# paulvantieghem/curla

Hardware: AMD Instinct MI355X
Metric: SAC+CURL gradient updates/sec, batch=512 84x84x9 (higher is better)
Workload: dtype f32

## Files before the change

curla_amd/_lib.py:

```python
import ctypes
import os

_HERE = os.path.dirname(os.path.abspath(__file__))
LIB_PATH = os.environ.get("CURLA_LIB_PATH") or os.path.join(_HERE, "libcurla_hip.so")

c_int, c_ll, c_float, c_size_t, vp = ctypes.c_int, ctypes.c_longlong, ctypes.c_float, ctypes.c_size_t, ctypes.c_void_p
c_u64 = ctypes.c_ulonglong
c_double = ctypes.c_double

ABI_VERSION = 8

SIGNATURES = {
    "curla_conv1_fwd": [vp, c_int, vp, vp, vp, vp, vp, vp, c_int, c_int, c_int, c_int, c_int, c_int, c_int, c_float, vp],
    "curla_conv3x3_s1_fwd": [vp, vp, vp, vp, c_int, c_int, c_int, c_int, vp],
    "curla_conv3x3_s1_fwd2": [vp, vp, vp, vp, c_int, vp, vp, vp, vp, c_int, c_int, c_int, c_int, vp],
    "curla_conv3x3_s1_fwd_stack": [c_int, vp, vp, vp, vp, c_int, vp, vp, vp, vp, c_int, c_int, c_int, c_int, vp],
    "curla_conv3x3_s1_stack_granule": [],
    "curla_conv1_fwd2": [vp, vp, vp, vp, vp, vp, vp, c_int, vp, vp, vp, vp, vp, vp, c_int, c_int, c_int, c_int, c_int, c_int,
                         c_int, c_float, vp],
    "curla_conv3x3_s1_dgrad": [vp, vp, vp, vp, c_int, c_int, c_int, c_int, vp],
    "curla_conv3x3_s1_wgrad": [vp, vp, vp, vp, vp, c_int, c_int, c_int, c_int, vp],
    "curla_conv1_wgrad": [vp, c_int, vp, vp, vp, vp, vp, vp, vp, c_int, c_int, c_int, c_int, c_int, c_int, c_int,
                          c_float, vp],
    "curla_conv3x3_s1_wgrad_slabs": [vp, vp, vp, c_int, c_int, c_int, c_int, vp, vp],
    "curla_conv1_wgrad_slabs": [vp, c_int, vp, vp, vp, vp, vp, c_int, c_int, c_int, c_int, c_int, c_int, c_int, c_float, vp,
                                vp],
    "curla_conv3x3_s1_bwd_slabs": [vp, vp, vp, vp, vp, c_int, c_int, c_int, c_int, vp, vp],
    "curla_conv1_dgrad": [vp, vp, vp, c_int, c_int, c_int, c_int, c_int, c_float, vp],
    "curla_wgrad_reduce_multi": [c_int, vp, vp, vp, vp, vp, vp, vp],
    "curla_conv_wgrad_workspace_floats": [c_int],
    "curla_gemm": [vp, c_int, c_int, c_ll, vp, c_int, c_int, c_ll, vp, c_int, c_ll, c_int, c_int, c_int, c_int, c_int,
                   c_ll, c_float, vp, c_ll, c_int, vp, c_int, c_ll, vp],
    "curla_fc_dx": [vp, vp, vp, vp, c_int, c_int, c_int, vp],
    "curla_fc_dw": [vp, vp, vp, c_int, c_int, c_int, vp],
    "curla_fc_bwd": [vp, vp, vp, vp, vp, c_int, c_int, c_int, vp],
    "curla_fc_bwd_ln": [vp, vp, vp, vp, vp, c_int, c_int, c_int, vp, c_int, vp, vp, vp, vp],
    "curla_fc_dw_ln": [vp, vp, vp, c_int, c_int, c_int, vp, c_int, vp, vp, vp, vp],
    "curla_fc_bwd_ln2": [vp, vp, vp, vp, vp, c_int, c_int, c_int, vp, c_int, vp, vp, vp, vp, c_int, c_int, vp, vp],
    "curla_curl_head": [vp, vp, vp, vp, vp, vp, c_int, c_int, vp, vp, vp, vp, vp, vp, vp, vp, vp, vp],
    "curla_gemm_nested": [vp, c_int, c_int, c_ll, c_ll, vp, c_int, c_int, c_ll, c_ll, vp, c_int, c_ll, c_ll, c_int, c_int, c_int,
                          c_int, c_int, c_float, vp, c_ll, c_ll, c_int, vp, c_int, c_ll, c_ll, vp],
    "curla_mlp_out_fwd_nested": [vp, c_ll, c_ll, vp, c_ll, c_ll, vp, c_ll, c_ll, vp, c_ll, c_ll, c_int, c_int, c_int, c_int, c_int,
                                 vp],
    "curla_gemm_multi": [c_int, vp, vp, vp, c_int, c_int, c_int, c_int, c_int, c_int, c_int, c_ll, vp],
    "curla_fc_fwd_multi": [c_int, vp, vp, vp, c_int, c_int, c_int, c_int, c_ll, c_int, vp],
    "curla_splitk_reduce": [vp, c_int, c_ll, c_int, c_int, c_int, vp, c_int, vp, c_int, vp],
    "curla_mlp_out_fwd": [vp, c_ll, vp, c_ll, vp, c_ll, vp, c_ll, c_int, c_int, c_int, c_int, vp],
    "curla_mlp_out_bwd": [vp, c_ll, vp, c_ll, vp, c_ll, vp, c_ll, vp, c_ll, c_int, c_int, c_int, c_int, vp],
    "curla_mlp_out_bwd_loss": [vp, vp, c_ll, vp, c_ll, vp, c_ll, vp, c_ll, c_int, c_int, vp, vp, c_ll, vp],
    "curla_mlp_out_bwd_bias": [vp, c_ll, vp, c_ll, vp, c_ll, vp, c_ll, vp, c_ll, c_int, c_int, c_int, c_int, vp, vp, c_ll,
                               vp],
    "curla_gemm_small_shape": [c_int, c_int, c_int, c_int],
    "curla_gemm_colsum": [vp, c_int, c_int, c_ll, vp, c_int, c_int, c_ll, vp, c_int, c_ll, c_int, c_int, c_int, c_int, vp,
                          c_ll, vp],
    "curla_linear_bwd": [vp, c_ll, vp, c_ll, vp, c_ll, vp, c_ll, vp, c_ll, vp, c_ll, vp, c_ll, c_int, c_int, c_int, c_int, vp],
    "curla_fc_ln_fwd": [vp, c_int, c_ll, c_int, vp, vp, vp, c_int, c_int, c_float, vp, vp, vp, vp, c_int, vp, vp, c_int,
                        vp],
    "curla_critic_td_loss": [vp, vp, c_ll, vp, vp, vp, vp, c_float, c_int, vp, vp, vp, vp],
    "curla_soft_update2": [vp, vp, c_size_t, c_size_t, c_float, c_float, c_float, c_float, vp],
    "curla_adam_step": [vp, vp, vp, vp, c_size_t, c_double, c_double, c_double, c_double, c_ll, vp, vp],
    "curla_adam_step_lerp": [vp, vp, vp, vp, c_size_t, c_double, c_double, c_double, c_double, c_ll, vp, vp, c_size_t,
                             c_float, c_float, c_float, c_float, vp],
    "curla_adam_step_scalar64": [vp, vp, vp, vp, c_size_t, c_double, c_double, c_double, c_double, c_ll, vp, vp, vp, vp, vp,
                                 c_double, c_double, c_double, c_double, c_ll, vp, vp],
    "curla_adam_step2": [vp, vp, vp, vp, vp, vp, c_size_t, c_size_t, c_double, c_double, c_double, c_double, c_ll, c_double,
                         c_double, c_double, c_double, c_ll, vp, vp],
    "curla_f64_pack": [vp, vp, vp],
    "curla_f64_unpack": [vp, c_double, c_double, vp, vp],
    "curla_gather_transition_scalars": [vp, vp, c_int, c_int, vp, vp, vp, vp],
    "curla_sample_stage": [vp, vp, c_ll, vp, c_int, c_int, vp, vp, vp, vp],
    "curla_nstep_compose": [vp, c_ll, vp, vp, c_ll, c_int, c_float, c_int, c_int, vp, vp, vp, vp],
    "curla_sample_stage_nstep": [vp, vp, c_ll, c_ll, vp, vp, c_ll, c_int, c_float, c_int, c_int, vp, vp, vp, vp],
    "curla_host_device_pointer": [vp, vp],
    "curla_ln_bwd": [vp, vp, vp, vp, c_int, c_int, vp, vp, vp, vp, vp],
    "curla_ln_bwd_twin": [vp, vp, c_int, vp, vp, vp, c_int, c_int, vp, vp, vp, vp, vp],
    "curla_ln_bwd_partial": [vp, vp, c_int, vp, vp, vp, c_int, c_int, vp, vp, vp, vp],
    "curla_colsum": [vp, c_int, c_int, c_int, c_ll, vp, c_ll, c_int, vp],
    "curla_colsum3": [vp, c_int, vp, c_int, vp, c_int, c_int, vp, vp, vp, c_ll, c_int, vp],
    "curla_actor_head_fwd": [vp, vp, c_int, c_int, c_float, c_float, vp, vp, vp, vp, vp, vp, c_int, vp],
    "curla_mlp_out_head_fwd": [vp, vp, vp, vp, c_int, c_int, c_int, vp, c_float, c_float, vp, vp, vp, vp, vp, vp, c_int, vp],
    "curla_actor_head_fwd_rng": [vp, vp, c_u64, c_u64, vp, c_int, c_int, c_float, c_float, vp, vp, vp, vp, vp, vp, c_int, vp],
    "curla_mlp_out_head_fwd_rng": [vp, vp, vp, vp, c_int, c_int, c_int, vp, c_u64, c_u64, vp, c_float, c_float, vp, vp, vp,
                                   vp, vp, vp, c_int, vp],
    "curla_fc_ln_fwd_multi": [c_int, vp, c_int, c_ll, c_int, c_int, c_int, c_float, c_int, vp],
    "curla_actor_head_bwd": [vp, vp, c_int, vp, vp, c_float, vp, vp, vp, vp, c_int, c_int, c_float, c_float, vp, vp],
    "curla_policy_head_bwd": [vp, vp, vp, vp, vp, vp, vp, vp, vp, c_int, c_int, c_float, c_float, vp, vp],
    "curla_concat": [vp, vp, c_int, c_int, c_int, vp, vp],
    "curla_split_sum": [vp, c_ll, c_int, c_int, c_int, vp, vp, vp],
    "curla_td_target": [vp, c_ll, vp, vp, vp, vp, c_float, c_int, vp, vp],
    "curla_critic_loss": [vp, c_ll, vp, c_int, vp, vp, vp],
    "curla_actor_loss": [vp, c_ll, vp, vp, c_int, vp, c_float, c_int, vp, vp, vp, vp],
    "curla_curl_ce": [vp, c_int, c_int, vp, vp, vp, vp],
    "curla_mean": [vp, c_int, vp, vp],
    "curla_soft_update": [vp, vp, c_size_t, c_float, c_float, vp],
    "curla_crop_nchw": [vp, vp, vp, vp, c_int, c_int, c_int, c_int, c_int, c_int, vp, vp, vp],
    "curla_store_frame": [vp, vp, c_ll, c_int, c_int, c_int, vp],
    "curla_stage_frames_u8": [vp, vp, c_ll, c_int, c_int, c_int, c_int, c_int, c_int, c_int, c_int, vp],
    "curla_gather_stacks": [vp, vp, c_int, vp, c_int, c_int, c_int, c_int, vp, vp],
    "curla_nhwc_to_nchw": [vp, vp, c_int, c_int, c_int, c_int, vp],
    "curla_color_jiggle": [vp, vp, vp, vp, c_int, c_int, c_int, c_int, vp, vp],
    "curla_noisy_cover": [vp, vp, vp, c_float, c_float, c_float, c_int, c_int, c_int, c_int, c_int, c_int, vp, vp],
    "curla_gather_nhwc": [vp, vp, c_int, c_int, c_int, c_int, vp, vp],
    "curla_noisy_cover_rng": [vp, vp, c_float, c_u64, c_u64, vp, c_float, c_float, c_float, vp, c_int, c_int, c_int, c_int,
                              c_int, c_int, vp, vp, vp],
    "curla_color_jiggle_nchw": [vp, vp, vp, c_int, c_int, c_int, c_int, vp, vp],
    "curla_noisy_cover_nchw": [vp, vp, c_float, c_float, c_float, c_int, c_int, c_int, c_int, c_int, c_int, vp, vp],
    "curla_random_shift_u8": [vp, vp, c_int, vp, vp, c_int, c_int, c_int, c_int, c_int, vp, vp],
    "curla_version": [],
    "curla_abi_version": [],
    "curla_set_option": [ctypes.c_char_p, ctypes.c_char_p],
    "curla_get_option": [ctypes.c_char_p],
}
_RESTYPES = {"curla_conv_wgrad_workspace_floats": c_size_t, "curla_version": ctypes.c_char_p,
             "curla_get_option": ctypes.c_char_p}
_ERRORS = {-1: "CURLA_ERR_ARG (bad pointer/size/alignment)", -2: "CURLA_ERR_LAUNCH (HIP launch failed)",
           -3: "CURLA_ERR_UNSUPPORTED (shape not supported by the gfx950 kernels)"}


class CurlaHipError(RuntimeError):
    pass


_lib = None


def load():
    global _lib
    if _lib is not None:
        return _lib
    if not os.path.exists(LIB_PATH):
        raise CurlaHipError(f"{LIB_PATH} is missing: build it with `python -m curla_amd.build` "
                            "(there is no CPU/PyTorch fallback for the learner path)")
    if LIB_PATH == os.path.join(_HERE, "libcurla_hip.so") and os.environ.get("CURLA_SKIP_SRCHASH", "0") != "1":
        from . import build
        try:
            want = build.source_hash()
        except OSError as e:
            raise CurlaHipError(f"cannot check {LIB_PATH} against its sources ({e}); set CURLA_SKIP_SRCHASH=1 to load "
                                "a library that was built elsewhere") from e
        if build.built_hash() != want:
            raise CurlaHipError(f"{LIB_PATH} was built from other sources than the ones in curla_amd/csrc "
                                f"(stamp {build.built_hash()} != {want}): rebuild it with "
                                "`python -m curla_amd.build` (or CURLA_SKIP_SRCHASH=1 for an externally built library)")
    lib = ctypes.CDLL(LIB_PATH)
    try:
        lib.curla_abi_version.restype = c_int
        got = int(lib.curla_abi_version())
    except AttributeError:
        got = None
    if got != ABI_VERSION:
        raise CurlaHipError(f"{LIB_PATH} has C-ABI version {got}, this binding was written for {ABI_VERSION} "
                            "(include/curla_hip.h CURLA_ABI_VERSION): rebuild the library or use the matching package")
    for name, args in SIGNATURES.items():
        fn = getattr(lib, name)
        fn.argtypes = args
        fn.restype = _RESTYPES.get(name, c_int)
    _lib = lib
    return lib


_trace_hook = None


def set_trace_hook(fn):
    global _trace_hook
    _trace_hook = fn


def call(name, *args):
    if _trace_hook is not None:
        _trace_hook(name, args)
        return
# ... 46 lines not shown
```

curla_amd/csrc/conv.hip:

```cpp
#include <algorithm>
#include <cstdlib>
#include <cstring>
#include <mutex>
#include <type_traits>

#include "common.h"
#include "options.h"

namespace {

constexpr int kLdsPix = 36;

enum { MODE_FWD = 0, MODE_DGRAD = 1 };

__device__ float g_zero_px[32];

#ifdef CURLA_ABLATE
int g_ablate = 0;
#define ABL(bit) (a.dbg & (bit))
#define ABL_HOST g_ablate
#else
#define ABL(bit) 0
#define ABL_HOST 0
#endif

#include "conv_rw.h"

__global__ __launch_bounds__(512, 2) void conv_rw_fwd_kernel(rw::Args A) {
  extern __shared__ __attribute__((aligned(16))) float lds[];
  for (int l = 0; l < A.nlayers; ++l) {
    rw::build_filter<MODE_FWD, 512>(lds, A.p[l][0].w, A.p[l][1].B > 0 ? A.p[l][1].w : nullptr, threadIdx.x);
    __syncthreads();
    rw::run_layer<MODE_FWD, 8>(A.g[l], A.p[l][0], A.p[l][1], lds, blockIdx.x, gridDim.x);
    if (l + 1 < A.nlayers) {
      __builtin_amdgcn_fence(__ATOMIC_RELEASE, "workgroup");
      __syncthreads();
      __builtin_amdgcn_fence(__ATOMIC_ACQUIRE, "workgroup");
    }
  }
}

#include "conv_rw43.h"

__global__ __launch_bounds__(256, 1) __attribute__((amdgpu_waves_per_eu(1, 1))) void conv_rw43_fwd_kernel(rw::Args A) {
  extern __shared__ __attribute__((aligned(16))) float lds[];
  for (int l = 0; l < A.nlayers; ++l) {
    rw43::build_filter<MODE_FWD, 256>(lds, A.p[l][0].w, A.p[l][1].B > 0 ? A.p[l][1].w : nullptr, threadIdx.x);
    __syncthreads();
    rw43::run_layer<MODE_FWD, 4>(A.g[l], A.p[l][0], A.p[l][1], lds, blockIdx.x, gridDim.x);
    if (l + 1 < A.nlayers) {
      __builtin_amdgcn_fence(__ATOMIC_RELEASE, "workgroup");
      __syncthreads();
      __builtin_amdgcn_fence(__ATOMIC_ACQUIRE, "workgroup");
    }
  }
}

__global__ __launch_bounds__(256, 1) __attribute__((amdgpu_waves_per_eu(1, 1))) void conv_rw43_dgrad_kernel(rw::Args A) {
  extern __shared__ __attribute__((aligned(16))) float lds[];
  rw43::build_filter<MODE_DGRAD, 256>(lds, A.p[0][0].w, nullptr, threadIdx.x);
  __syncthreads();
  rw43::run_layer<MODE_DGRAD, 4>(A.g[0], A.p[0][0], A.p[0][1], lds, blockIdx.x, gridDim.x);
}

#include "conv_rwb.h"

#ifdef RWB_CLOCK
__device__ unsigned long long g_rwb_clock[3 * 1024];
#endif

template <int NW>
__device__ __forceinline__ void rwb_fwd_body(const rw::Args& A) {
  extern __shared__ __attribute__((aligned(16))) unsigned short lds_h[];
#if defined(RWB_STAMP) || defined(RWB_CLOCK)
  const unsigned long long kt0 = __builtin_readcyclecounter(), kr0 = __builtin_amdgcn_s_memrealtime();
#endif
  for (int l = 0; l < A.nlayers; ++l) {
#ifdef RWB_STAMP
    const unsigned long long k0 = __builtin_readcyclecounter();
#endif
    rwb::build_filter<MODE_FWD, 64 * NW>(lds_h, A.p[l][0].w, A.p[l][1].B > 0 ? A.p[l][1].w : nullptr, threadIdx.x);
    __syncthreads();
#ifdef RWB_STAMP
    const unsigned long long k1 = __builtin_readcyclecounter();
#endif
    rwb::run_layer<MODE_FWD, NW>(A.g[l], A.p[l][0], A.p[l][1], lds_h, blockIdx.x, gridDim.x);
#ifdef RWB_STAMP
    const unsigned long long k2 = __builtin_readcyclecounter();
#endif
    if (l + 1 < A.nlayers) {
      __builtin_amdgcn_fence(__ATOMIC_RELEASE, "workgroup");
      __syncthreads();
      __builtin_amdgcn_fence(__ATOMIC_ACQUIRE, "workgroup");
    }
#ifdef RWB_STAMP
    const unsigned long long k3 = __builtin_readcyclecounter();
    if (threadIdx.x == 0 && blockIdx.x == 7) {
      rwb::g_rwb_stamp[4] += k1 - k0, rwb::g_rwb_stamp[5] += k2 - k1, rwb::g_rwb_stamp[6] += k3 - k2, rwb::g_rwb_stamp[7] += 1;
    }
#endif
  }
#ifdef RWB_STAMP
  if (threadIdx.x == 0 && blockIdx.x == 7) {
    rwb::g_rwb_stamp[15] += __builtin_readcyclecounter() - kt0;
    rwb::g_rwb_stamp[14] += __builtin_amdgcn_s_memrealtime() - kr0;
  }
#endif
#ifdef RWB_CLOCK
  if (threadIdx.x == 0 && blockIdx.x < 1024) {
    g_rwb_clock[3 * blockIdx.x + 0] += __builtin_readcyclecounter() - kt0;
    g_rwb_clock[3 * blockIdx.x + 1] += __builtin_amdgcn_s_memrealtime() - kr0;
    g_rwb_clock[3 * blockIdx.x + 2] += 1;
  }
#endif
}

__global__ __launch_bounds__(512, 1) void conv_rwb_fwd_kernel(rw::Args A) { rwb_fwd_body<8>(A); }

__global__ __launch_bounds__(512, 1) void conv_rwb_dgrad_kernel(rw::Args A) {
  extern __shared__ __attribute__((aligned(16))) unsigned short lds_h[];
  rwb::build_filter<MODE_DGRAD, 512>(lds_h, A.p[0][0].w, nullptr, threadIdx.x);
  __syncthreads();
  rwb::run_layer<MODE_DGRAD, 8>(A.g[0], A.p[0][0], A.p[0][1], lds_h, blockIdx.x, gridDim.x);
}

__global__ __launch_bounds__(256, 2) void conv_rw_dgrad_kernel(rw::Args A) {
  extern __shared__ __attribute__((aligned(16))) float lds[];
  rw::build_filter<MODE_DGRAD, 256>(lds, A.p[0][0].w, nullptr, threadIdx.x);
  __syncthreads();
  rw::run_layer<MODE_DGRAD, 4>(A.g[0], A.p[0][0], A.p[0][1], lds, blockIdx.x, gridDim.x);
}

#include "conv1_rw.h"

template <int C>
__global__ __launch_bounds__(512, 2) void conv1_rw_fwd_kernel(rw::Conv1Args a) {
  rw::conv1_body<C, 8>(a, blockIdx.x, gridDim.x);
}

template <int C>
__global__ __launch_bounds__(512, 2) void wgrad1_rw_kernel(rw::Wgrad1Args a) {
  rw::wgrad1_body<C, 8>(a, blockIdx.x, gridDim.x);
}

#include "conv1_u8_rw.h"

constexpr int kC1U8Threads = 512, kC1U8PerCU = 2;

template <int C>
__global__ __launch_bounds__(kC1U8Threads, kC1U8PerCU) void conv1_u8_rw_fwd_kernel(rw::Conv1U8Args a) {
  __shared__ __attribute__((aligned(16))) float lds_img[2 * rw::conv1_u8_image_floats<C>()];
  rw::conv1_u8_stage_weights<C, kC1U8Threads>(lds_img, a.p[0].w, a.p[0].bias, a.scale, threadIdx.x);
  if (a.p[1].B > 0)
    rw::conv1_u8_stage_weights<C, kC1U8Threads>(lds_img + rw::conv1_u8_image_floats<C>(), a.p[1].w, a.p[1].bias, a.scale,
                                                threadIdx.x);
  __syncthreads();
  if ((a.Ws * C) % 4 == 0)
    rw::conv1_u8_body<C, kC1U8Threads / 64, true>(a, lds_img, blockIdx.x, gridDim.x);
  else
    rw::conv1_u8_body<C, kC1U8Threads / 64, false>(a, lds_img, blockIdx.x, gridDim.x);
}

constexpr int kC1U8bThreads = 256, kC1U8bPerCU = 3;
template <int C>
__global__ __launch_bounds__(kC1U8bThreads, kC1U8bPerCU) void conv1_u8_rwb_fwd_kernel(rw::Conv1U8Args a) {
  __shared__ __attribute__((aligned(16))) unsigned char lds_imgb[2 * rw::kConv1U8B3ImageBytes];
  rw::conv1_u8b_stage_weights<C, kC1U8bThreads>(lds_imgb, a.p[0].w, a.p[0].bias, a.scale, threadIdx.x);
  if (a.p[1].B > 0)
    rw::conv1_u8b_stage_weights<C, kC1U8bThreads>(lds_imgb + rw::kConv1U8B3ImageBytes, a.p[1].w, a.p[1].bias, a.scale,
                                                  threadIdx.x);
  __syncthreads();
  if ((a.Ws * C) % 4 == 0)
    rw::conv1_u8b_body<C, kC1U8bThreads / 64, true>(a, lds_imgb, blockIdx.x, gridDim.x);
  else
    rw::conv1_u8b_body<C, kC1U8bThreads / 64, false>(a, lds_imgb, blockIdx.x, gridDim.x);
}

#include "conv1_band.h"

constexpr int kPartialS1 = 32 * 288 + 32;

#include "conv_rw_wgrad.h"
#include "conv_rw_wgrad2.h"

__device__ __forceinline__ void wgrad_any(const rw::WgradArgs& wa, const int bid, const int nblk) {
  if (wa.two_d)
    rw::wgrad2_body<4>(wa, bid, nblk);
  else
    rw::wgrad_body<4>(wa, bid, nblk);
}

__global__ __launch_bounds__(256, 2) void wgrad_rw_kernel(rw::WgradArgs wa) {
  wgrad_any(wa, blockIdx.x, gridDim.x);
}

__global__ __launch_bounds__(256, 2) void bwd_rw2_kernel(rw::WgradArgs wa, rw::Args da, int nw) {
  if ((int)blockIdx.x < nw) {
    wgrad_any(wa, blockIdx.x, nw);
  } else {
    extern __shared__ __attribute__((aligned(16))) float lds[];
    rw::build_filter<MODE_DGRAD, 256>(lds, da.p[0][0].w, nullptr, threadIdx.x);
    __syncthreads();
    rw::run_layer<MODE_DGRAD, 4>(da.g[0], da.p[0][0], da.p[0][1], lds, (int)blockIdx.x - nw, (int)gridDim.x - nw);
  }
}

__global__ __launch_bounds__(256, 2) void bwd_rwb2_kernel(rw::WgradArgs wa, rw::Args da, int nw) {
  if ((int)blockIdx.x < nw) {
    wgrad_any(wa, blockIdx.x, nw);
  } else {
    extern __shared__ __attribute__((aligned(16))) unsigned short lds_hb[];
    rwb::build_filter<MODE_DGRAD, 256>(lds_hb, da.p[0][0].w, nullptr, threadIdx.x);
    __syncthreads();
    rwb::run_layer<MODE_DGRAD, 4>(da.g[0], da.p[0][0], da.p[0][1], lds_hb, (int)blockIdx.x - nw, (int)gridDim.x - nw);
  }
}

#include "conv1_wgrad.h"

#include "conv_wgrad_reduce.h"

constexpr int kMaxLds = 160 * 1024;
static_assert(2 * rwb::kWBytes <= kMaxLds, "the two problems' split filters of conv_rwb_fwd_kernel must fit one CU's LDS");
template <typename K>
int set_lds(K kernel, size_t bytes) {
  if (bytes > (size_t)kMaxLds) return CURLA_ERR_UNSUPPORTED;
  return curla_set_dyn_lds(reinterpret_cast<const void*>(kernel), kMaxLds);
}

template <typename... Params, typename... Args>
int launch(void (*kernel)(Params...), int grid, int threads, size_t lds, hipStream_t st, const Args&... args) {
  if (lds) {
    const int rc = set_lds(kernel, lds);
    if (rc != CURLA_OK) return rc;
  }
  hipLaunchKernelGGL(kernel, dim3(grid), dim3(threads), lds, st, args...);
  return curla_launch_status();
}

template <int... Cs, typename F>
int dispatch_c(int C, F&& f) {
  int rc = CURLA_ERR_UNSUPPORTED;
  (void)(... || (C == Cs ? (rc = f(std::integral_constant<int, Cs>{}), true) : false));
  return rc;
}

enum { kSrcF32Nchw = 0, kSrcU8Ring = 1, kSrcF32Nhwc = 2 };
template <typename F>
int dispatch_src(int src_kind, F&& f) {
  if (src_kind == kSrcU8Ring) return f(std::integral_constant<int, SRC_U8>{});
  if (src_kind == kSrcF32Nhwc) return f(std::integral_constant<int, SRC_NHWC>{});
  return f(std::integral_constant<int, SRC_F32>{});
}


enum class S1Form { F23, F43, B3 };
S1Form select_s1_form() {
  const int opt = curla_opt(kOptS1Fwd);
  return opt == kS1FwdF23 ? S1Form::F23 : opt == kS1FwdF43 ? S1Form::F43 : S1Form::B3;
}

enum class BwdShape { SideBySide, TwoAndTwo };
BwdShape select_bwd_shape(S1Form dgrad, int B, int Ho, int Wo) {
  const int opt = curla_opt(kOptBwdSplit);
  const bool side = opt == kBwdSplitAuto ? dgrad == S1Form::B3 || (long long)B * Ho * Wo <= (1LL << 20) : opt == kBwdSplitOn;
  return side ? BwdShape::SideBySide : BwdShape::TwoAndTwo;
}

enum class S1WgradForm { X, XY };
S1WgradForm select_s1_wgrad_form() { return curla_opt(kOptS1Wgrad) == kS1WgradX ? S1WgradForm::X : S1WgradForm::XY; }

int u8_row_bytes(int Wc, int C) { return ((Wc * C + 15) & ~15) + 16; }
int f32_row_floats(int Wc, int C) { return ((Wc * C + 3) & ~3) + 4; }
int u8_band_rows(int Ho, int RSb, size_t budget) {
  int th = Ho;
  while (th > 1 && (size_t)(2 * th + 1) * RSb > budget) --th;
  return th;
}

enum class Conv1U8Form { Rwb, Rw, Hybrid, Band };
constexpr size_t kConv1U8BandBudget = 76 * 1024;
Conv1U8Form select_conv1_u8_form(int C, int Hs, int Ws, int Wc, int Btotal, int Ho, int Wo) {
  const int opt = curla_opt(kOptConv1U8);
  const bool walk_asked = opt == kConv1U8Auto || opt == kConv1U8Rw || opt == kConv1U8Rwb;
  const bool walk_fits =
      (long long)Hs * Ws * C < (1LL << 30) && (long long)Btotal * Ho * ((Wo + 15) / 16 + 1) < (1LL << 28);
  if (walk_asked && walk_fits) return opt != kConv1U8Rw && 3 * C <= 32 ? Conv1U8Form::Rwb : Conv1U8Form::Rw;
  const bool one_band = u8_band_rows(Ho, u8_row_bytes(Wc, C), kConv1U8BandBudget) == Ho;
  return one_band && Wc * C <= 64 * 16 && opt != kConv1U8Band ? Conv1U8Form::Hybrid : Conv1U8Form::Band;
}

enum class Conv1F32Form { Rw, Band };
Conv1F32Form select_conv1_f32_form(int src_kind, int C, int Hc, int Wc) {
  const bool rw = src_kind == kSrcF32Nhwc && curla_opt(kOptConv1F32) == kConv1F32Rw && (long long)Hc * Wc * C * 4 < (1LL << 30);
  return rw ? Conv1F32Form::Rw : Conv1F32Form::Band;
}

enum class Wgrad1U8Form { B16, F32, F32FourWave };
constexpr size_t kWgrad1U8BandBudget = 76 * 1024, kWgrad1U8BandBudget4 = 38 * 1024;
Wgrad1U8Form select_wgrad1_u8_form(int C, int Wc, int Wo) {
  if ((ABL_HOST & 1024) && (size_t)(2 * 4 + 1) * u8_row_bytes(Wc, C) <= kWgrad1U8BandBudget4) return Wgrad1U8Form::F32FourWave;
  return curla_opt(kOptWgrad1U8) != kWgrad1U8F32 && Wo >= 8 && 3 * C <= 32 ? Wgrad1U8Form::B16 : Wgrad1U8Form::F32;
}

bool rw_supported(int Hi, int Wi) { return (long long)(Hi + 2) * (Wi + 2) * 128 < (1LL << 30); }

rw::Geom s1_plan(S1Form f, int Hi, int Wi, int Ho, int Wo) {
  return f == S1Form::B3 ? rwb::plan(Hi, Wi, Ho, Wo) : f == S1Form::F43 ? rw43::plan(Hi, Wi, Ho, Wo) : rw::plan(Hi, Wi, Ho, Wo);
}
size_t s1_filter_bytes(S1Form f) {
  return f == S1Form::B3 ? rwb::kWBytes : (f == S1Form::F43 ? rw43::kWFloats : rw::kWFloats) * sizeof(float);
}

int launch_rw_fwd(int nlayers, const float* in, const float* const* w, const float* const* bias, float* const* out, int B,
                  const float* in2, const float* const* w2, const float* const* bias2, float* const* out2, int B2, int Hi,
                  int Wi, bool owned, hipStream_t st) {
  const S1Form form = select_s1_form();
  rw::Args A;
  A.nlayers = nlayers;
  for (int l = 0; l < rw::kMaxLayers; ++l) {
    const bool on = l < nlayers;
    const int hi = Hi - 2 * l, wi = Wi - 2 * l;
    A.g[l] = on ? s1_plan(form, hi, wi, hi - 2, wi - 2) : rw::Geom{};
    A.p[l][0] = on ? rw::Problem{l == 0 ? in : out[l - 1], w[l], bias[l], out[l], B} : rw::Problem{};
    A.p[l][1] = (on && B2 > 0) ? rw::Problem{l == 0 ? in2 : out2[l - 1], w2[l], bias2[l], out2[l], B2} : rw::Problem{};
    if (on && (hi < 3 || wi < 3)) return CURLA_ERR_UNSUPPORTED;
  }
  if (!rw_supported(Hi, Wi)) return CURLA_ERR_UNSUPPORTED;
  const int cus = curla_cu_count();
  const int grid = owned ? cus : std::min(B > B2 ? B : B2, cus);
  const size_t lds = (size_t)(B2 > 0 ? 2 : 1) * s1_filter_bytes(form);
  switch (form) {
    case S1Form::B3: return launch(conv_rwb_fwd_kernel, grid, 512, lds, st, A);
    case S1Form::F43: return launch(conv_rw43_fwd_kernel, grid, 256, lds, st, A);
    default: return launch(conv_rw_fwd_kernel, grid, 512, lds, st, A);
  }
}

rw::Args rw_dgrad_args(S1Form form, const float* g, const float* w, const float* act_below, float* gin, int B, int Ho,
                       int Wo) {
  rw::Args A;
  A.nlayers = 1;
  for (int l = 0; l < rw::kMaxLayers; ++l) A.g[l] = rw::Geom{}, A.p[l][0] = rw::Problem{}, A.p[l][1] = rw::Problem{};
  A.g[0] = s1_plan(form, Ho, Wo, Ho + 2, Wo + 2);
  A.p[0][0] = rw::Problem{g, w, act_below, gin, B};
  return A;
}

int launch_dgrad(S1Form form, const float* g, const float* w, const float* act_below, float* gin, int B, int Ho, int Wo,
                 hipStream_t st) {
  const rw::Args A = rw_dgrad_args(form, g, w, act_below, gin, B, Ho, Wo);
  const int cus = curla_cu_count();
  const size_t lds = s1_filter_bytes(form);
  switch (form) {
    case S1Form::B3: return launch(conv_rwb_dgrad_kernel, std::min(B, cus), 512, lds, st, A);
    case S1Form::F43: return launch(conv_rw43_dgrad_kernel, std::min(B, cus), 256, lds, st, A);
    default: return launch(conv_rw_dgrad_kernel, std::min(B, 2 * cus), 256, lds, st, A);
  }
}

int launch_conv_s1(int mode, const float* in, const float* w, const float* aux, float* out, int B, int Hs, int Ws,
                   hipStream_t st, const float* in2 = nullptr, const float* w2 = nullptr, const float* aux2 = nullptr,
                   float* out2 = nullptr, int B2 = 0) {
  if (!rw_supported(Hs, Ws)) return CURLA_ERR_UNSUPPORTED;
  if (mode == MODE_FWD) return launch_rw_fwd(1, in, &w, &aux, &out, B, in2, &w2, &aux2, &out2, B2, Hs, Ws, false, st);
  return launch_dgrad(select_s1_form(), in, w, aux, out, B, Hs, Ws, st);
}

rw::WgradArgs wgrad_args(const float* in, const float* g, float* workspace, int B, int Hi, int Wi, int Ho, int Wo) {
  const bool two_d = select_s1_wgrad_form() == S1WgradForm::XY;
  return rw::WgradArgs{in, g, workspace, B, Hi, Wi, Ho, Wo, two_d ? rw::plan4p(Hi, Wi, Ho, Wo) : rw::plan4(Hi, Wi, Ho, Wo),
                       two_d ? 1 : 0};
}

int plan_band_conv1(int Ho, int Wo, int Wc, int C, int g_px_per_row, size_t lds_budget) {
  const int RS = f32_row_floats(Wc, C);
// ... 151 lines not shown
                               float* const* out, int B, const float* in2, const float* const* w2,
                               const float* const* bias2, float* const* out2, int B2, int Hi, int Wi, int channels,
                               void* stream) {
  CURLA_REQUIRE(nlayers > 0 && nlayers <= rw::kMaxLayers && in && w && bias && out && B > 0 && Hi >= 3 && Wi >= 3);
  CURLA_REQUIRE(B2 == 0 || (in2 && w2 && bias2 && out2));
  if (channels != 32) return CURLA_ERR_UNSUPPORTED;
  const int G1 = curla_cu_count();
  if (B % G1 != 0 || B2 % G1 != 0) return CURLA_ERR_UNSUPPORTED;
  CURLA_REQUIRE(aligned16(in) && (!B2 || aligned16(in2)));
  for (int l = 0; l < nlayers; ++l) {
    CURLA_REQUIRE(w[l] && bias[l] && out[l] && aligned16(w[l]) && aligned16(bias[l]) && aligned16(out[l]));
    CURLA_REQUIRE(!B2 || (w2[l] && bias2[l] && out2[l] && aligned16(w2[l]) && aligned16(bias2[l]) && aligned16(out2[l])));
  }
  if (Hi - 2 * nlayers < 1 || Wi - 2 * nlayers < 1) return CURLA_ERR_UNSUPPORTED;
  return launch_rw_fwd(nlayers, in, w, bias, out, B, in2, w2, bias2, out2, B2, Hi, Wi, true,
                       static_cast<hipStream_t>(stream));
}

int curla_conv3x3_s1_stack_granule(void) { return curla_cu_count(); }

int curla_conv3x3_s1_dgrad(const float* g, const float* w, const float* act_below, float* gin, int B, int Ho, int Wo,
                           int channels, void* stream) {
  CURLA_REQUIRE(g && w && act_below && gin && B > 0 && Ho >= 1 && Wo >= 1);
  if (channels != 32) return gen_dgrad(g, w, act_below, gin, B, Ho, Wo, channels, static_cast<hipStream_t>(stream));
  CURLA_REQUIRE(aligned16(g) && aligned16(gin) && aligned16(act_below) && aligned16(w));
  return launch_conv_s1(MODE_DGRAD, g, w, act_below, gin, B, Ho, Wo, static_cast<hipStream_t>(stream));
}

static int conv1_common_check(const void* src, int src_kind, int B, int C, int Hs, int Ws, int Hc, int Wc) {
  CURLA_REQUIRE(src && B > 0 && Hc >= 3 && Wc >= 3 && src_kind >= 0 && src_kind <= 2);
  if (C != 9 && C != 12 && C != 6 && C != 3) return CURLA_ERR_UNSUPPORTED;
  if (src_kind == kSrcU8Ring) {
    CURLA_REQUIRE(Hs >= Hc && Ws >= Wc);
    CURLA_REQUIRE((reinterpret_cast<uintptr_t>(src) & 3) == 0);
  }
  return CURLA_OK;
}

struct Conv1Second {
  const int64_t* idx;
  const int32_t* h1;
  const int32_t* w1;
  const float* w;
  const float* bias;
  float* out;
  int B;
};

static int launch_conv1_u8_rw(Conv1U8Form form, const Conv1Args& a, hipStream_t st) {
  rw::Conv1U8Args ra;
  ra.src = static_cast<const uint8_t*>(a.src);
  ra.p[0] = rw::Conv1U8Problem{a.idx, a.h1, a.w1, a.w, a.bias, a.out, a.B};
  ra.p[1] = rw::Conv1U8Problem{a.idx2, a.h1_2, a.w1_2, a.w2, a.bias2, a.out2, a.B2};
  ra.Hs = a.Hs, ra.Ws = a.Ws, ra.Ho = a.Ho, ra.Wo = a.Wo, ra.scale = a.scale;
  ra.g.Hi = a.Hc, ra.g.Wi = a.Wc, ra.g.Ho = a.Ho, ra.g.Wo = a.Wo;
  rw::plan_units(ra.g, a.Ho, a.Wo, 16);
  const long long pool = (long long)(a.B + a.B2) * ra.g.steps;
  const bool b16 = form == Conv1U8Form::Rwb;
  const int threads = b16 ? kC1U8bThreads : kC1U8Threads;
  const int cap = (b16 ? kC1U8bPerCU : kC1U8PerCU) * curla_cu_count();
  const int share = 8 * (threads / 64);
  const int want = (int)((pool + share - 1) / share);
  const int grid = want < cap ? (want < 1 ? 1 : want) : cap;
  if (b16)
    return dispatch_c<9, 6, 3>(a.C, [&](auto cc) { return launch(conv1_u8_rwb_fwd_kernel<cc()>, grid, threads, 0, st, ra); });
  return dispatch_c<9, 12, 6, 3>(a.C, [&](auto cc) { return launch(conv1_u8_rw_fwd_kernel<cc()>, grid, threads, 0, st, ra); });
}

static int launch_conv1_u8_band(Conv1U8Form form, Conv1Args& a, hipStream_t st) {
  const size_t lds = plan_conv1_u8_band(a);
  const int grid = (a.B + a.B2) * a.nbands;
  if (form == Conv1U8Form::Hybrid) {
    rw::Geom G;
    G.Hi = a.Hc, G.Wi = a.Wc, G.Ho = a.Ho, G.Wo = a.Wo;
    rw::plan_units(G, a.Ho, a.Wo, 16);
    return dispatch_c<9, 12, 6, 3>(a.C, [&](auto cc) { return launch(conv1_u8_walk_kernel<cc()>, grid, 512, lds, st, a, G); });
  }
  return dispatch_c<9, 12, 6, 3>(a.C, [&](auto cc) { return launch(conv1_fwd_u8_kernel<cc()>, grid, 512, lds, st, a); });
}

static int launch_conv1_rw(const Conv1Args& a, hipStream_t st) {
  rw::Conv1Args ra;
  ra.src = static_cast<const float*>(a.src), ra.w = a.w, ra.bias = a.bias, ra.out = a.out;
  ra.B = a.B, ra.Hc = a.Hc, ra.Wc = a.Wc, ra.Ho = a.Ho, ra.Wo = a.Wo, ra.scale = a.scale;
  ra.g.Hi = a.Hc, ra.g.Wi = a.Wc, ra.g.Ho = a.Ho, ra.g.Wo = a.Wo;
  rw::plan_units(ra.g, a.Ho, a.Wo, 16);
  const int grid = std::min(a.B, curla_cu_count());
  return dispatch_c<12, 9, 6, 3>(a.C, [&](auto cc) { return launch(conv1_rw_fwd_kernel<cc()>, grid, 512, 0, st, ra); });
}

static int launch_conv1_band(int src_kind, Conv1Args& a, hipStream_t st) {
  a.th = plan_band_conv1(a.Ho, a.Wo, a.Wc, a.C, 0, 76 * 1024);
  a.nbands = (a.Ho + a.th - 1) / a.th;
  const size_t lds = std::max<size_t>(((size_t)(2 * a.th + 1) * f32_row_floats(a.Wc, a.C) + 8) * sizeof(float),
                              (size_t)32 * a.C * 9 * sizeof(float));
  const int grid = std::min(a.B * a.nbands, 2 * curla_cu_count());
  return dispatch_c<9, 12, 6, 3>(a.C, [&](auto cc) {
    return dispatch_src(src_kind, [&](auto src) { return launch(conv1_fwd_kernel<src(), cc()>, grid, 512, lds, st, a); });
  });
}

static int conv1_fwd_impl(const void* src, int src_kind, const int64_t* idx, const int32_t* h1, const int32_t* w1,
                          const float* w, const float* bias, float* out, int B, int C, int Hs, int Ws, int Hc, int Wc,
                          int channels, float scale, void* stream, const Conv1Second* second) {
  CURLA_REQUIRE(w && bias && out);
  int rc = conv1_common_check(src, src_kind, B, C, Hs, Ws, Hc, Wc);
  if (rc != CURLA_OK) return rc;
  hipStream_t st = static_cast<hipStream_t>(stream);
  if (second && src_kind != kSrcU8Ring) return CURLA_ERR_UNSUPPORTED;
  if (channels != 32) {
    rc = gen_fwd1(gen_src(src, src_kind, idx, h1, w1, C, Hs, Ws, Hc, Wc, scale), w, bias, out, B, channels, st);
    if (rc == CURLA_OK && second)
      rc = gen_fwd1(gen_src(src, src_kind, second->idx, second->h1, second->w1, C, Hs, Ws, Hc, Wc, scale), second->w,
                    second->bias, second->out, second->B, channels, st);
    return rc;
  }
  Conv1Args a;
  a.src = src, a.idx = idx, a.h1 = h1, a.w1 = w1, a.w = w, a.bias = bias, a.out = out;
  a.B = B, a.C = C, a.Hs = Hs, a.Ws = Ws, a.Hc = Hc, a.Wc = Wc;
  a.Ho = (Hc - 3) / 2 + 1, a.Wo = (Wc - 3) / 2 + 1;
  a.scale = scale;
  a.dbg = ABL_HOST;
  a.idx2 = second ? second->idx : nullptr, a.h1_2 = second ? second->h1 : nullptr, a.w1_2 = second ? second->w1 : nullptr;
  a.w2 = second ? second->w : nullptr, a.bias2 = second ? second->bias : nullptr, a.out2 = second ? second->out : nullptr;
  a.B2 = second ? second->B : 0;
  if (src_kind == kSrcU8Ring) {
    switch (const Conv1U8Form form = select_conv1_u8_form(C, Hs, Ws, Wc, B + a.B2, a.Ho, a.Wo)) {
      case Conv1U8Form::Rwb:
      case Conv1U8Form::Rw: return launch_conv1_u8_rw(form, a, st);
      case Conv1U8Form::Hybrid:
      case Conv1U8Form::Band:
        if (!(ABL_HOST & 128)) return launch_conv1_u8_band(form, a, st);
        break;
    }
  } else if (select_conv1_f32_form(src_kind, C, Hc, Wc) == Conv1F32Form::Rw) {
    return launch_conv1_rw(a, st);
  }
  return launch_conv1_band(src_kind, a, st);
}

int curla_conv1_fwd(const void* src, int src_kind, const int64_t* idx, const int32_t* h1, const int32_t* w1,
                    const float* w, const float* bias, float* out, int B, int C, int Hs, int Ws, int Hc, int Wc,
                    int channels, float scale, void* stream) {
  return conv1_fwd_impl(src, src_kind, idx, h1, w1, w, bias, out, B, C, Hs, Ws, Hc, Wc, channels, scale, stream, nullptr);
}

int curla_conv1_fwd2(const uint8_t* ring, const int64_t* idx, const int32_t* h1, const int32_t* w1, const float* w,
                     const float* bias, float* out, int B, const int64_t* idx2, const int32_t* h1_2,
                     const int32_t* w1_2, const float* w2, const float* bias2, float* out2, int B2, int C, int Hs, int Ws,
                     int Hc, int Wc, int channels, float scale, void* stream) {
  CURLA_REQUIRE(w2 && bias2 && out2 && B2 > 0);
  Conv1Second sec{idx2, h1_2, w1_2, w2, bias2, out2, B2};
  return conv1_fwd_impl(ring, kSrcU8Ring, idx, h1, w1, w, bias, out, B, C, Hs, Ws, Hc, Wc, channels, scale, stream, &sec);
}

size_t curla_conv_wgrad_workspace_floats(int cin) {
  return (size_t)4 * curla_cu_count() * ((size_t)32 * cin * 9 + 32);
}

static int launch_wgrad_s1(const float* in, const float* g, float* workspace, int B, int Hi, int Wi, int channels,
                           hipStream_t st, int* nslabs) {
  CURLA_REQUIRE(in && g && workspace && B > 0 && Hi >= 3 && Wi >= 3);
  if (channels != 32) return gen_wgrad_s1(in, g, workspace, B, Hi, Wi, channels, st, nslabs);
  if (!rw_supported(Hi, Wi)) return CURLA_ERR_UNSUPPORTED;
  CURLA_REQUIRE(aligned16(in) && aligned16(g));
  const rw::WgradArgs ra = wgrad_args(in, g, workspace, B, Hi, Wi, Hi - 2, Wi - 2);
  *nslabs = std::min(B, 2 * curla_cu_count());
  return launch(wgrad_rw_kernel, *nslabs, 256, kPartialS1 * sizeof(float), st, ra);
}

static int launch_wgrad_reduce(const float* workspace, int nslabs, int nw, int channels, float* dw, float* db, hipStream_t st) {
  return launch(wgrad_reduce_kernel, (nw + channels + 31) / 32, 1024, 0, st, workspace, nslabs, nw, channels, dw, db);
}

int curla_conv3x3_s1_wgrad(const float* in, const float* g, float* dw, float* db, float* workspace, int B, int Hi,
                           int Wi, int channels, void* stream) {
  CURLA_REQUIRE(dw && db);
  hipStream_t st = static_cast<hipStream_t>(stream);
  int nslabs = 0;
  const int rc = launch_wgrad_s1(in, g, workspace, B, Hi, Wi, channels, st, &nslabs);
  if (rc != CURLA_OK) return rc;
  return launch_wgrad_reduce(workspace, nslabs, channels * channels * 9, channels, dw, db, st);
}

int curla_conv3x3_s1_wgrad_slabs(const float* in, const float* g, float* workspace, int B, int Hi, int Wi, int channels,
                                 int* nslabs, void* stream) {
  CURLA_REQUIRE(nslabs);
  return launch_wgrad_s1(in, g, workspace, B, Hi, Wi, channels, static_cast<hipStream_t>(stream), nslabs);
}

int curla_conv3x3_s1_bwd_slabs(const float* in, const float* g, const float* w, float* gin, float* workspace, int B, int Hi,
                               int Wi, int channels, int* nslabs, void* stream) {
  CURLA_REQUIRE(in && g && w && gin && workspace && nslabs && B > 0 && Hi >= 3 && Wi >= 3);
  hipStream_t st = static_cast<hipStream_t>(stream);
  if (channels != 32) {
    const int rc = gen_wgrad_s1(in, g, workspace, B, Hi, Wi, channels, st, nslabs);
    return rc != CURLA_OK ? rc : gen_dgrad(g, w, in, gin, B, Hi - 2, Wi - 2, channels, st);
  }
  CURLA_REQUIRE(aligned16(in) && aligned16(g) && aligned16(w) && aligned16(gin));
  const int Ho = Hi - 2, Wo = Wi - 2;
  if (!rw_supported(Hi, Wi)) return CURLA_ERR_UNSUPPORTED;
  const S1Form form = select_s1_form();
  if (form == S1Form::F43) {
    const int rc = launch_wgrad_s1(in, g, workspace, B, Hi, Wi, channels, st, nslabs);
    return rc != CURLA_OK ? rc : launch_dgrad(form, g, w, in, gin, B, Ho, Wo, st);
  }
  const int per_cu = select_bwd_shape(form, B, Ho, Wo) == BwdShape::SideBySide ? 1 : 2;
  const int n = std::min(B, per_cu * curla_cu_count());
  const rw::WgradArgs wr = wgrad_args(in, g, workspace, B, Hi, Wi, Ho, Wo);
  const rw::Args dr = rw_dgrad_args(form, g, w, in, gin, B, Ho, Wo);
  const size_t lds = std::max<size_t>(s1_filter_bytes(form), kPartialS1 * sizeof(float));
  *nslabs = n;
  return launch(form == S1Form::B3 ? bwd_rwb2_kernel : bwd_rw2_kernel, 2 * n, 256, lds, st, wr, dr, n);
}

int curla_wgrad_reduce_multi(int njobs, const float* const* slabs, const int* nslabs, const int* nw, const int* nb,
                             float* const* dw, float* const* db, void* stream) {
  CURLA_REQUIRE(njobs > 0 && njobs <= kMaxReduceJobs && slabs && nslabs && nw && dw && db);
  ReduceJobs J;
  int blocks = 0;
  for (int j = 0; j < njobs; ++j) {
    CURLA_REQUIRE(slabs[j] && dw[j] && db[j] && nslabs[j] > 0 && nw[j] > 0);
    J.partial[j] = slabs[j], J.dw[j] = dw[j], J.db[j] = db[j], J.nslabs[j] = nslabs[j], J.nw[j] = nw[j];
    J.nb[j] = nb ? nb[j] : 32;
    CURLA_REQUIRE(J.nb[j] > 0);
    J.first_block[j] = blocks;
    blocks += (nw[j] + J.nb[j] + 31) / 32;
  }
  J.first_block[njobs] = blocks;
  J.njobs = njobs;
  return launch(wgrad_reduce_multi_kernel, blocks, 1024, 0, static_cast<hipStream_t>(stream), J);
}

static int launch_wgrad1(const void* src, int src_kind, const int64_t* idx, const int32_t* h1, const int32_t* w1,
                         const float* g, float* workspace, int B, int C, int Hs, int Ws, int Hc, int Wc, int channels,
                         float scale, void* stream, int* nslabs) {
  CURLA_REQUIRE(g && workspace);
  const int rc = conv1_common_check(src, src_kind, B, C, Hs, Ws, Hc, Wc);
  if (rc != CURLA_OK) return rc;
  hipStream_t st = static_cast<hipStream_t>(stream);
  if (channels != 32)
    return gen_wgrad1(gen_src(src, src_kind, idx, h1, w1, C, Hs, Ws, Hc, Wc, scale), g, workspace, B, channels, st, nslabs);
  CURLA_REQUIRE(aligned16(g));
  Wgrad1Args a;
  a.src = src, a.idx = idx, a.h1 = h1, a.w1 = w1, a.g = g, a.partial = workspace;
  a.B = B, a.C = C, a.Hs = Hs, a.Ws = Ws, a.Hc = Hc, a.Wc = Wc;
  a.Ho = (Hc - 3) / 2 + 1, a.Wo = (Wc - 3) / 2 + 1;
  a.scale = scale;
  a.lds_bytes = 0;
  a.dbg = ABL_HOST;
  const size_t slab_bytes = (size_t)(32 * C * 9 + 32) * sizeof(float);
  int& grid = *nslabs;
  if (src_kind == kSrcU8Ring && !(ABL_HOST & 256)) {
    const Wgrad1U8Form form = select_wgrad1_u8_form(C, Wc, a.Wo);
    const size_t lds = plan_wgrad1_u8(a, form);
    grid = std::min(B * a.nbands, (form == Wgrad1U8Form::F32FourWave ? 4 : 2) * curla_cu_count());
    switch (form) {
      case Wgrad1U8Form::B16:
        return dispatch_c<9, 6, 3>(C, [&](auto cc) { return launch(wgrad1_u8b_kernel<cc(), 8>, grid, 512, lds, st, a); });
      case Wgrad1U8Form::F32FourWave:
        return dispatch_c<9, 12, 6, 3>(C, [&](auto cc) { return launch(wgrad1_u8_kernel<cc(), 4>, grid, 256, lds, st, a); });
      default:
        return dispatch_c<9, 12, 6, 3>(C, [&](auto cc) { return launch(wgrad1_u8_kernel<cc(), 8>, grid, 512, lds, st, a); });
    }
  }
  if (src_kind != kSrcU8Ring && select_conv1_f32_form(src_kind, C, Hc, Wc) == Conv1F32Form::Rw) {
    rw::Wgrad1Args ra;
    ra.src = static_cast<const float*>(src), ra.g = g, ra.partial = workspace;
    ra.B = B, ra.Hc = Hc, ra.Wc = Wc, ra.Ho = a.Ho, ra.Wo = a.Wo, ra.scale = scale;
    ra.gg.Hi = Hc, ra.gg.Wi = Wc, ra.gg.Ho = a.Ho, ra.gg.Wo = a.Wo;
    rw::plan_units(ra.gg, a.Ho, a.Wo, 4);
    grid = std::min(B, curla_cu_count());
    return dispatch_c<12, 9, 6, 3>(C, [&](auto cc) { return launch(wgrad1_rw_kernel<cc()>, grid, 512, slab_bytes, st, ra); });
  }
  a.th = plan_band_conv1(a.Ho, a.Wo, Wc, C, 0, 150 * 1024);
  a.nbands = (a.Ho + a.th - 1) / a.th;
  const size_t lds = std::max<size_t>(((size_t)(2 * a.th + 1) * f32_row_floats(Wc, C) + 8) * sizeof(float), slab_bytes);
  grid = std::min(B * a.nbands, curla_cu_count());
  return dispatch_c<9, 12, 6, 3>(C, [&](auto cc) {
    return dispatch_src(src_kind, [&](auto s) { return launch(wgrad1_kernel<s(), cc()>, grid, 512, lds, st, a); });
  });
}

int curla_conv1_wgrad(const void* src, int src_kind, const int64_t* idx, const int32_t* h1, const int32_t* w1,
                      const float* g, float* dw, float* db, float* workspace, int B, int C, int Hs, int Ws, int Hc,
                      int Wc, int channels, float scale, void* stream) {
  CURLA_REQUIRE(dw && db);
  int nslabs = 0;
  const int rc = launch_wgrad1(src, src_kind, idx, h1, w1, g, workspace, B, C, Hs, Ws, Hc, Wc, channels, scale, stream, &nslabs);
  if (rc != CURLA_OK) return rc;
  return launch_wgrad_reduce(workspace, nslabs, channels * C * 9, channels, dw, db, static_cast<hipStream_t>(stream));
}

int curla_conv1_wgrad_slabs(const void* src, int src_kind, const int64_t* idx, const int32_t* h1, const int32_t* w1,
                            const float* g, float* workspace, int B, int C, int Hs, int Ws, int Hc, int Wc, int channels,
                            float scale, int* nslabs, void* stream) {
  CURLA_REQUIRE(nslabs);
  return launch_wgrad1(src, src_kind, idx, h1, w1, g, workspace, B, C, Hs, Ws, Hc, Wc, channels, scale, stream, nslabs);
}

}

#include "conv1_dgrad.h"
```

curla_amd/csrc/conv1_u8_rw.h:

```cpp
#pragma once

namespace rw {

struct Conv1U8Problem {
  const int64_t* idx;
  const int32_t* h1;
  const int32_t* w1;
  const float* w;
  const float* bias;
  float* out;
  int B;
};

struct Conv1U8Args {
  const uint8_t* src;
  Conv1U8Problem p[2];
  int Hs, Ws, Ho, Wo;
  float scale;
  Geom g;
};

template <class T>
__device__ __forceinline__ T const_load(const T* p, int i) {
  return ((const T __attribute__((address_space(4)))*)(unsigned long long)p)[i];
// ... 100 lines not shown
    const long long slot = P.idx ? const_load(P.idx, b) : b;
    const int origin = ((P.h1 ? const_load(P.h1, b) : 0) * a.Ws + (P.w1 ? const_load(P.w1, b) : 0)) * C;
    const uint8_t* crop = a.src + (size_t)slot * frame + origin;
    const int mis = AL ? (int)(reinterpret_cast<uintptr_t>(crop) & 3) : 0;
    const __amdgpu_buffer_rsrc_t rin = uniform_rsrc(crop - mis, frame - origin + 8 + mis);
    const __amdgpu_buffer_rsrc_t rout = uniform_rsrc(P.out + (size_t)b * a.Ho * a.Wo * 32, a.Ho * out_row);
    {
      int x, y0;
      bool lane_on;
      if (k < G.nfull) {
        x = 16 * k + li, y0 = 0, lane_on = true;
      } else {
        const int u = (k - G.nfull) * 16 + li;
        const int col = u / G.nseg, sg = u - col * G.nseg;
        lane_on = col < G.brem;
        x = 16 * G.nfull + col, y0 = sg * G.nr;
      }
      const int Y = y0 + sb;
      const unsigned run = (unsigned)((2 * Y * a.Ws + 2 * x) * C + E * kq + mis);
      const unsigned vin = lane_on ? (AL ? run & ~3u : run) : 0x80000000u;
      const unsigned sh = run & 3u;
      unsigned vo = lane_on ? (unsigned)((Y * a.Wo + x) * 128 + kq * 16) : 0x80000000u;

      struct Row {
        float v[E];
      };
      using Raw = RawBytes<NL>;
      auto load_row = [&](Raw& R, int r) {
        load_raw<NL>(R, rin, vin, __builtin_amdgcn_readfirstlane((unsigned)(r * in_row)));
      };
      auto convert = [&](Row& F, const Raw& R) {
        RawBytes<NW_> Wd;
#pragma unroll
        for (int j = 0; j < NW_; ++j)
          Wd.d[j] = AL ? __builtin_amdgcn_alignbyte(j + 1 < NL ? R.d[j + 1 < NL ? j + 1 : j] : 0u, R.d[j], sh) : R.d[j];
#pragma unroll
        for (int e = 0; e < E; ++e) F.v[e] = byte_f32<NW_>(Wd, e);
      };
      auto mma_row = [&](f32x4 (&acc)[2], const Row& F, const int dy) {
#pragma unroll
        for (int e = 0; e < E; ++e)
#pragma unroll
          for (int mt = 0; mt < 2; ++mt) acc[mt] = mfma16(wr[dy][e][mt], F.v[e], acc[mt]);
      };
      struct Pair {
        Raw a, b;
      };
      auto step = [&](const Row& r0, Row& r1, Row& r2, const Pair& cur, Pair& nxt, const int t) {
        load_row(nxt.a, 2 * t + 2 * kDepth + 1);
        load_row(nxt.b, 2 * t + 2 * kDepth + 2);
        __builtin_amdgcn_sched_barrier(0);
        f32x4 acc[2] = {bias4[0], bias4[1]};
        mma_row(acc, r0, 0);
        __builtin_amdgcn_sched_barrier(0);
        convert(r1, cur.a);
        convert(r2, cur.b);
        __builtin_amdgcn_sched_barrier(0);
        mma_row(acc, r1, 1);
        mma_row(acc, r2, 2);
#pragma unroll
        for (int mt = 0; mt < 2; ++mt) {
          f32x4 v = acc[mt];
#pragma unroll
          for (int r = 0; r < 4; ++r) v[r] = relu_bits(v[r]);
          __builtin_amdgcn_raw_buffer_store_b128(__builtin_bit_cast(__attribute__((ext_vector_type(4))) unsigned, v), rout,
                                                 vo + mt * 64u, 0, CURLA_ACT_STORE_POLICY);
        }
        vo += out_row;
      };

      Row S0, S1, S2, S3, S4;
      Pair P0, P1, P2;
      {
        Raw R0;
        load_row(R0, 0), load_row(P0.a, 1), load_row(P0.b, 2), load_row(P1.a, 3), load_row(P1.b, 4);
        convert(S0, R0);
      }
      for (int t = 0;;) {
        step(S0, S1, S2, P0, P2, t);
        if (++t >= n) break;
        step(S2, S3, S4, P1, P0, t);
        if (++t >= n) break;
        step(S4, S0, S1, P2, P1, t);
        if (++t >= n) break;
        step(S1, S2, S3, P0, P2, t);
        if (++t >= n) break;
        step(S3, S4, S0, P1, P0, t);
        if (++t >= n) break;
        step(S0, S1, S2, P2, P1, t);
        if (++t >= n) break;
        step(S2, S3, S4, P0, P2, t);
        if (++t >= n) break;
        step(S4, S0, S1, P1, P0, t);
        if (++t >= n) break;
        step(S1, S2, S3, P2, P1, t);
        if (++t >= n) break;
        step(S3, S4, S0, P0, P2, t);
        if (++t >= n) break;
        step(S0, S1, S2, P1, P0, t);
        if (++t >= n) break;
        step(S2, S3, S4, P2, P1, t);
        if (++t >= n) break;
        step(S4, S0, S1, P0, P2, t);
        if (++t >= n) break;
        step(S1, S2, S3, P1, P0, t);
        if (++t >= n) break;
        step(S3, S4, S0, P2, P1, t);
        if (++t >= n) break;
      }
    }
  }
}

struct U8Frag {
  unsigned d[4];
};

constexpr int kConv1U8B3ImageBytes = 3 * 2 * 3 * 64 * 16 + 32 * 4;

template <int C, int NT>
__device__ __forceinline__ void conv1_u8b_stage_weights(unsigned char* img, const float* __restrict__ w,
                                                        const float* __restrict__ bias, float scale, int tid) {
  static_assert(3 * C <= 32, "one k-step per input row");
  typedef __bf16 bf2 __attribute__((ext_vector_type(2)));
  auto pk = [](float x0, float x1) {
    const f32x2 v = {x0, x1};
    return __builtin_bit_cast(unsigned, __builtin_convertvector(v, bf2));
  };
  for (int item = tid; item < 3 * 2 * 64; item += NT) {
    const int slot = item & 63, dm = item >> 6, dy = dm >> 1, mt = dm & 1;
    const int li = slot & 15, kq = slot >> 4, co = 16 * mt + li;
    unsigned h[4], m[4], l[4];
#pragma unroll
    for (int q = 0; q < 4; ++q) {
      float x[2];
#pragma unroll
      for (int e = 0; e < 2; ++e) {
        const int rr = 8 * kq + 2 * q + e, dx = rr / C, c = rr - dx * C;
        x[e] = rr < 3 * C ? w[(co * C + c) * 9 + dy * 3 + dx] * scale : 0.f;
      }
      h[q] = pk(x[0], x[1]);
      const float r0 = x[0] - __builtin_bit_cast(float, h[q] << 16), r1 = x[1] - __builtin_bit_cast(float, h[q] & 0xFFFF0000u);
      m[q] = pk(r0, r1);
      const float s0 = r0 - __builtin_bit_cast(float, m[q] << 16), s1 = r1 - __builtin_bit_cast(float, m[q] & 0xFFFF0000u);
      l[q] = pk(s0, s1);
    }
    typedef unsigned u4 __attribute__((ext_vector_type(4)));
    u4* p = reinterpret_cast<u4*>(img) + (dm * 3) * 64 + slot;
    p[0] = u4{h[0], h[1], h[2], h[3]}, p[64] = u4{m[0], m[1], m[2], m[3]}, p[128] = u4{l[0], l[1], l[2], l[3]};
  }
  if (tid < 32) reinterpret_cast<float*>(img + 3 * 2 * 3 * 64 * 16)[tid] = bias[tid];
}

template <int C, int NW, bool AL>
__device__ __forceinline__ void conv1_u8b_body(const Conv1U8Args& a, const unsigned char* lds_img, const int bid,
                                               const int nblk) {
  constexpr int E = 8;
  constexpr int NW_ = 2;
  constexpr int NL = AL ? 3 : NW_;
  typedef short bf16x8 __attribute__((ext_vector_type(8)));
  typedef unsigned u4 __attribute__((ext_vector_type(4)));
  const int lane = threadIdx.x & 63;
  const int wave = __builtin_amdgcn_readfirstlane(threadIdx.x >> 6);
  const int li = lane & 15, kq = lane >> 4;
  const Geom& G = a.g;

  const int B0 = a.p[0].B;
  const int pool = (B0 + a.p[1].B) * G.steps;
  const int per = pool / nblk, rem = pool - per * nblk;
  const int g0 = bid * per + (bid < rem ? bid : rem), len = per + (bid < rem ? 1 : 0);
  const int lo = g0 + len * wave / NW, hi = g0 + len * (wave + 1) / NW;
  const int in_row = a.Ws * C, out_row = a.Wo * 128;
  const int frame = a.Hs * in_row;

  u4 wf[3][2][3];
  f32x4 bias4[2];
  int have = -1;

  for (int g = lo; g < hi;) {
    const int u = g / G.steps;
    const int r = g - u * G.steps;
    int k, sb, n_strip;
    if (r < G.nfull * G.Ho) {
      k = r / G.Ho, sb = r - k * G.Ho, n_strip = G.Ho;
    } else {
      const int q = (r - G.nfull * G.Ho) / G.nr;
      k = G.nfull + q, sb = r - G.nfull * G.Ho - q * G.nr, n_strip = G.nr;
    }
    const int n = hi - g < n_strip - sb ? hi - g : n_strip - sb;
    g += n;
    const int prob = u >= B0 ? 1 : 0;
    const int b = u - (prob ? B0 : 0);
    const Conv1U8Problem& P = a.p[prob];
    if (prob != have) {
      have = prob;
      const unsigned char* im = lds_img + prob * kConv1U8B3ImageBytes;
      const u4* wl = reinterpret_cast<const u4*>(im) + lane;
#pragma unroll
      for (int dy = 0; dy < 3; ++dy)
#pragma unroll
        for (int mt = 0; mt < 2; ++mt)
#pragma unroll
          for (int p = 0; p < 3; ++p) wf[dy][mt][p] = wl[((dy * 2 + mt) * 3 + p) * 64];
      const float* bl = reinterpret_cast<const float*>(im + 3 * 2 * 3 * 64 * 16);
#pragma unroll
      for (int mt = 0; mt < 2; ++mt) bias4[mt] = *reinterpret_cast<const f32x4*>(bl + mt * 16 + 4 * kq);
    }
    const long long slot = P.idx ? const_load(P.idx, b) : b;
    const int origin = ((P.h1 ? const_load(P.h1, b) : 0) * a.Ws + (P.w1 ? const_load(P.w1, b) : 0)) * C;
    const uint8_t* crop = a.src + (size_t)slot * frame + origin;
    const int mis = AL ? (int)(reinterpret_cast<uintptr_t>(crop) & 3) : 0;
    const __amdgpu_buffer_rsrc_t rin = uniform_rsrc(crop - mis, frame - origin + 16 + mis);
    const __amdgpu_buffer_rsrc_t rout = uniform_rsrc(P.out + (size_t)b * a.Ho * a.Wo * 32, a.Ho * out_row);
    {
      int x, y0;
      bool lane_on;
      if (k < G.nfull) {
        x = 16 * k + li, y0 = 0, lane_on = true;
      } else {
        const int uu = (k - G.nfull) * 16 + li;
        const int col = uu / G.nseg, sg = uu - col * G.nseg;
        lane_on = col < G.brem;
        x = 16 * G.nfull + col, y0 = sg * G.nr;
      }
      const int Y = y0 + sb;
      const unsigned run = (unsigned)((2 * Y * a.Ws + 2 * x) * C + E * kq + mis);
      const unsigned vin = lane_on ? (AL ? run & ~3u : run) : 0x80000000u;
      const unsigned sh = run & 3u;
      unsigned vo = lane_on ? (unsigned)((Y * a.Wo + x) * 128 + kq * 16) : 0x80000000u;

      using Raw = RawBytes<NL>;
      auto load_row = [&](Raw& R, int rr) {
        load_raw<NL>(R, rin, vin, __builtin_amdgcn_readfirstlane((unsigned)(rr * in_row)));
      };
      auto convert = [&](u4& F, const Raw& R) {
        RawBytes<NW_> Wd;
#pragma unroll
        for (int j = 0; j < NW_; ++j)
          Wd.d[j] = AL ? __builtin_amdgcn_alignbyte(R.d[j + 1], R.d[j], sh) : R.d[j];
#pragma unroll
        for (int q = 0; q < 4; ++q) {
          const float f0 = byte_f32<NW_>(Wd, 2 * q), f1 = byte_f32<NW_>(Wd, 2 * q + 1);
          F[q] = (__builtin_bit_cast(unsigned, f0) >> 16) | (__builtin_bit_cast(unsigned, f1) & 0xFFFF0000u);
        }
      };
      auto mma_row = [&](f32x4 (&acc)[2], const u4& F, const int dy) {
        const bf16x8 xb = __builtin_bit_cast(bf16x8, F);
#pragma unroll
        for (int p = 2; p >= 0; --p)
#pragma unroll
          for (int mt = 0; mt < 2; ++mt)
            acc[mt] = __builtin_amdgcn_mfma_f32_16x16x32_bf16(__builtin_bit_cast(bf16x8, wf[dy][mt][p]), xb, acc[mt], 0, 0, 0);
      };
      struct Pair {
        Raw a, b;
      };
      auto step = [&](const u4& r0, u4& r1, u4& r2, const Pair& cur, Pair& nxt, const int t) {
        load_row(nxt.a, 2 * t + 2 * kDepth + 1);
        load_row(nxt.b, 2 * t + 2 * kDepth + 2);
        __builtin_amdgcn_sched_barrier(0);
        f32x4 acc[2] = {bias4[0], bias4[1]};
        mma_row(acc, r0, 0);
        convert(r1, cur.a);
        convert(r2, cur.b);
        mma_row(acc, r1, 1);
        mma_row(acc, r2, 2);
#pragma unroll
        for (int mt = 0; mt < 2; ++mt) {
          f32x4 v = acc[mt];
#pragma unroll
          for (int rr = 0; rr < 4; ++rr) v[rr] = relu_bits(v[rr]);
          __builtin_amdgcn_raw_buffer_store_b128(__builtin_bit_cast(u4, v), rout, vo + mt * 64u, 0, CURLA_ACT_STORE_POLICY);
        }
        vo += out_row;
      };

      u4 S0, S1, S2, S3, S4;
      Pair P0, P1, P2;
      {
        Raw R0;
        load_row(R0, 0), load_row(P0.a, 1), load_row(P0.b, 2), load_row(P1.a, 3), load_row(P1.b, 4);
        convert(S0, R0);
      }
      for (int t = 0;;) {
        step(S0, S1, S2, P0, P2, t);
        if (++t >= n) break;
        step(S2, S3, S4, P1, P0, t);
        if (++t >= n) break;
        step(S4, S0, S1, P2, P1, t);
        if (++t >= n) break;
        step(S1, S2, S3, P0, P2, t);
        if (++t >= n) break;
        step(S3, S4, S0, P1, P0, t);
        if (++t >= n) break;
        step(S0, S1, S2, P2, P1, t);
        if (++t >= n) break;
        step(S2, S3, S4, P0, P2, t);
        if (++t >= n) break;
        step(S4, S0, S1, P1, P0, t);
        if (++t >= n) break;
        step(S1, S2, S3, P2, P1, t);
        if (++t >= n) break;
        step(S3, S4, S0, P0, P2, t);
        if (++t >= n) break;
        step(S0, S1, S2, P1, P0, t);
        if (++t >= n) break;
        step(S2, S3, S4, P2, P1, t);
        if (++t >= n) break;
        step(S4, S0, S1, P0, P2, t);
        if (++t >= n) break;
        step(S1, S2, S3, P1, P0, t);
        if (++t >= n) break;
        step(S3, S4, S0, P2, P1, t);
        if (++t >= n) break;
      }
    }
  }
}

}
```

curla_amd/csrc/conv_rwb.h:

```cpp
#pragma once

namespace rwb {

using rw::Args;
using rw::Geom;
using rw::Problem;
using rw::uniform_rsrc;

typedef short bf16x8 __attribute__((ext_vector_type(8)));
typedef unsigned u32x4 __attribute__((ext_vector_type(4)));
typedef __bf16 bf16x2_t __attribute__((ext_vector_type(2)));

constexpr int kWBytes = 3 * 4 * 2 * 3 * 64 * 16;

inline Geom plan(int Hi, int Wi, int Ho, int Wo) { return rw::plan(Hi, Wi, Ho, Wo); }

struct B3 {
  u32x4 h, m, l;
};

__device__ __forceinline__ unsigned cvt_pk_bf16(float x0, float x1) {
  const f32x2 v = {x0, x1};
  return __builtin_bit_cast(unsigned, __builtin_convertvector(v, bf16x2_t));
}

__device__ __forceinline__ B3 split8(const float (&v)[8]) {
  B3 o;
#if defined(RWB_ABL) && (RWB_ABL & 1)
#pragma unroll
  for (int p = 0; p < 4; ++p) o.h[p] = __builtin_bit_cast(unsigned, v[2 * p]), o.m[p] = __builtin_bit_cast(unsigned, v[2 * p + 1]);
  o.l = o.h;
  return o;
#endif
#pragma unroll
  for (int p = 0; p < 4; ++p) {
    const float x0 = v[2 * p], x1 = v[2 * p + 1];
    const unsigned h = cvt_pk_bf16(x0, x1);
    const float r0 = x0 - __builtin_bit_cast(float, h << 16), r1 = x1 - __builtin_bit_cast(float, h & 0xFFFF0000u);
    const unsigned m = cvt_pk_bf16(r0, r1);
    const float s0 = r0 - __builtin_bit_cast(float, m << 16), s1 = r1 - __builtin_bit_cast(float, m & 0xFFFF0000u);
    o.h[p] = h, o.m[p] = m, o.l[p] = cvt_pk_bf16(s0, s1);
  }
  return o;
}

__device__ __forceinline__ f32x4 mfma_bf16(const u32x4 a, const u32x4 b, const f32x4 c) {
  return __builtin_amdgcn_mfma_f32_16x16x32_bf16(__builtin_bit_cast(bf16x8, a), __builtin_bit_cast(bf16x8, b), c, 0, 0, 0);
}

template <int MODE, int NT>
__device__ __forceinline__ void build_filter(unsigned short* lds_w, const float* __restrict__ w0,
                                             const float* __restrict__ w1, int tid) {
  const int nitems = (w1 ? 2 : 1) * 6 * 64;
  for (int item = tid; item < nitems; item += NT) {
    const int slot = item & 63, dm = (item >> 6) % 6, prob = item / 384;
    const int li = slot & 15, kq = slot >> 4, dy = dm >> 1, mt = dm & 1;
    const float* __restrict__ w = prob ? w1 : w0;
    const int co = 16 * mt + li;
    float u[8][4];
#pragma unroll
    for (int j = 0; j < 8; ++j) {
      const int ci = 8 * kq + j;
      const float* t = MODE == MODE_FWD ? w + (co * 32 + ci) * 9 + dy * 3 : w + (ci * 32 + co) * 9 + (2 - dy) * 3;
      if (MODE == MODE_FWD)
        rw::filter_transform(t[0], t[1], t[2], u[j]);
      else
        rw::filter_transform(t[2], t[1], t[0], u[j]);
    }
    u32x4* img = reinterpret_cast<u32x4*>(lds_w + prob * (kWBytes / 2));
#pragma unroll
    for (int pos = 0; pos < 4; ++pos) {
      float v[8];
#pragma unroll
      for (int j = 0; j < 8; ++j) v[j] = u[j][pos];
      const B3 x = split8(v);
      u32x4* p = img + ((((dy * 4 + pos) * 2 + mt) * 3)) * 64 + slot;
      p[0] = x.h, p[64] = x.m, p[128] = x.l;
    }
  }
}

#ifdef RWB_STAMP
__device__ unsigned long long g_rwb_stamp[16];
#endif

struct Acc {
  f32x4 m[2][4];
};

template <int MODE, int NW>
__device__ __forceinline__ void run_layer(const Geom& G, const Problem& P0, const Problem& P1, const unsigned short* lds_w,
                                          int bid, int nblk) {
  const int lane = threadIdx.x & 63;
  const int wave = __builtin_amdgcn_readfirstlane(threadIdx.x >> 6);
  const int li = lane & 15, kq = lane >> 4;
  const int pad = MODE == MODE_FWD ? 0 : 2;
  const int cnt0 = bid < P0.B ? (P0.B - bid + nblk - 1) / nblk : 0;
  const int cnt1 = bid < P1.B ? (P1.B - bid + nblk - 1) / nblk : 0;
  const int nstrips = G.nfull + G.ntr;
  const int T = (cnt0 + cnt1) * G.steps;
  const int lo = (int)((long)wave * T / NW), hi = (int)((long)(wave + 1) * T / NW);
  const int in_row = G.Wi * 128, out_row = G.Wo * 128;

  int before = 0;
  for (int si = 0; si < cnt0 + cnt1; ++si) {
    const bool second = si >= cnt0;
    const Problem& P = second ? P1 : P0;
    const int b = bid + (second ? si - cnt0 : si) * nblk;
    const u32x4* lw = reinterpret_cast<const u32x4*>(lds_w + (second ? kWBytes / 2 : 0)) + lane;
    for (int k = 0; k < nstrips; ++k) {
      const int n_strip = k < G.nfull ? G.Ho : G.nr;
      const int a0 = lo > before ? lo : before;
      const int a1 = hi < before + n_strip ? hi : before + n_strip;
      const int sb = a0 - before, n = a1 - a0;
      before += n_strip;
      if (n <= 0) continue;

      int j, y0;
      bool lane_on;
      if (k < G.nfull) {
        j = 16 * k + li, y0 = 0, lane_on = true;
      } else {
        const int u = (k - G.nfull) * 16 + li;
        const int col = u / G.nseg, sg = u - col * G.nseg;
        lane_on = col < G.brem;
        j = 16 * G.nfull + col, y0 = sg * G.nr;
      }
      const int Y = y0 + sb;
      const int x0 = 2 * j;
      const __amdgpu_buffer_rsrc_t rin = uniform_rsrc(P.in + (size_t)b * G.Hi * G.Wi * 32, G.Hi * in_row);
      const __amdgpu_buffer_rsrc_t rout = uniform_rsrc(P.out + (size_t)b * G.Ho * G.Wo * 32, G.Ho * out_row);
      const __amdgpu_buffer_rsrc_t raux = uniform_rsrc(MODE == MODE_DGRAD ? P.aux + (size_t)b * G.Ho * G.Wo * 32 : P.aux,
                                                       MODE == MODE_DGRAD ? G.Ho * out_row : 128);
      unsigned voff[4];
#pragma unroll
      for (int c = 0; c < 4; ++c) {
        const int col = x0 + c - pad;
        const bool ok = lane_on && (unsigned)col < (unsigned)G.Wi;
        voff[c] = ok ? (unsigned)(((Y - pad) * G.Wi + col) * 128 + kq * 32) : 0x80000000u;
      }
      unsigned oa = lane_on ? (unsigned)((Y * G.Wo + x0) * 128 + kq * 16) : 0x80000000u;
      unsigned ob = (lane_on && x0 + 1 < G.Wo) ? oa + 128u : 0x80000000u;

      f32x4 bias[2] = {{0, 0, 0, 0}, {0, 0, 0, 0}};
      if (MODE == MODE_FWD) {
        bias[0] = *reinterpret_cast<const f32x4*>(P.aux + 4 * kq);
        bias[1] = *reinterpret_cast<const f32x4*>(P.aux + 16 + 4 * kq);
      }

      f32x4 raw[4][2];
      auto load_row = [&]() {
#pragma unroll
        for (int c = 0; c < 4; ++c) {
          raw[c][0] = __builtin_bit_cast(f32x4, __builtin_amdgcn_raw_buffer_load_b128(rin, voff[c], 0, 0));
          raw[c][1] = __builtin_bit_cast(f32x4, __builtin_amdgcn_raw_buffer_load_b128(rin, voff[c] + 16u, 0, 0));
        }
      };
      struct W3 {
        u32x4 h, m, l;
      };
      auto wread = [&](const int g) {
        const int pos = g / 6, dy = 2 - (g / 2) % 3, mt = g & 1;
        const u32x4* p = lw + ((((dy * 4 + pos) * 2 + mt) * 3)) * 64;
        W3 w;
#if defined(RWB_ABL) && (RWB_ABL & 2)
        w.h = p[0], w.m = w.h, w.l = w.h;
        return w;
#endif
        w.h = p[0], w.m = p[64], w.l = p[128];
        return w;
      };

      Acc S0, S1, S2;
      f32x4 mk[2][2];

      auto mul6 = [&](f32x4 acc, const W3& w, const B3& x) {
#if !(defined(RWB_ABL) && (RWB_ABL & 4))
        acc = mfma_bf16(w.l, x.h, acc);
        acc = mfma_bf16(w.h, x.l, acc);
        acc = mfma_bf16(w.m, x.m, acc);
#endif
        acc = mfma_bf16(w.m, x.h, acc);
        acc = mfma_bf16(w.h, x.m, acc);
        acc = mfma_bf16(w.h, x.h, acc);
        return acc;
      };
      auto finish = [&](const Acc& S) {
#pragma unroll
        for (int mt = 0; mt < 2; ++mt) {
          f32x4 ya = S.m[mt][0] + S.m[mt][1] + S.m[mt][2];
          f32x4 yb = S.m[mt][1] - S.m[mt][2] - S.m[mt][3];
          if (MODE == MODE_FWD) {
#pragma unroll
            for (int r = 0; r < 4; ++r) ya[r] = fmaxf(ya[r], 0.f), yb[r] = fmaxf(yb[r], 0.f);
          } else {
#pragma unroll
            for (int r = 0; r < 4; ++r) ya[r] = mk[0][mt][r] > 0.f ? ya[r] : 0.f, yb[r] = mk[1][mt][r] > 0.f ? yb[r] : 0.f;
          }
          __builtin_amdgcn_raw_buffer_store_b128(__builtin_bit_cast(u32x4, ya), rout, oa + mt * 64u, 0, CURLA_ACT_STORE_POLICY);
          __builtin_amdgcn_raw_buffer_store_b128(__builtin_bit_cast(u32x4, yb), rout, ob + mt * 64u, 0, CURLA_ACT_STORE_POLICY);
        }
        oa += out_row, ob += out_row;
      };

      W3 Wa, Wb;
      auto step = [&](Acc& Sdy2, Acc& Sdy1, Acc& Sdy0, const int t) {
#ifdef RWB_STAMP
        const unsigned long long c0 = __builtin_readcyclecounter();
#endif
        B3 X[4];
        {
          float v[4][8];
#pragma unroll
          for (int c8 = 0; c8 < 8; ++c8) {
            const float d0 = raw[0][c8 >> 2][c8 & 3], d1 = raw[1][c8 >> 2][c8 & 3], d2 = raw[2][c8 >> 2][c8 & 3],
                        d3 = raw[3][c8 >> 2][c8 & 3];
            v[0][c8] = d0 - d2, v[1][c8] = d1 + d2, v[2][c8] = d2 - d1, v[3][c8] = d1 - d3;
          }
#pragma unroll
          for (int pos = 0; pos < 4; ++pos) X[pos] = split8(v[pos]);
        }
        if (t < n + 1) {
#pragma unroll
          for (int c = 0; c < 4; ++c) voff[c] += in_row;
          load_row();
        }
        const bool do2 = t >= 2, do1 = t >= 1 && t <= n, do0 = t < n;
        if (MODE == MODE_DGRAD && do2) {
#pragma unroll
          for (int mt = 0; mt < 2; ++mt) {
            mk[0][mt] = __builtin_bit_cast(f32x4, __builtin_amdgcn_raw_buffer_load_b128(raux, oa + mt * 64u, 0, 0));
            mk[1][mt] = __builtin_bit_cast(f32x4, __builtin_amdgcn_raw_buffer_load_b128(raux, ob + mt * 64u, 0, 0));
          }
        }
#ifdef RWB_STAMP
        const unsigned long long c1 = __builtin_readcyclecounter();
#endif
#pragma unroll
        for (int g = 0; g < 24; ++g) {
          const int pos = g / 6, which = (g / 2) % 3, mt = g & 1;
          W3& cur = (g & 1) ? Wb : Wa;
          W3& nxt = (g & 1) ? Wa : Wb;
          nxt = wread(g == 23 ? 0 : g + 1);
          __builtin_amdgcn_sched_barrier(0);
          if (which == 0) {
            if (do2) Sdy2.m[mt][pos] = mul6(Sdy2.m[mt][pos], cur, X[pos]);
          } else if (which == 1) {
            if (do1) Sdy1.m[mt][pos] = mul6(Sdy1.m[mt][pos], cur, X[pos]);
          } else {
            const f32x4 z = {0, 0, 0, 0};
            if (do0) Sdy0.m[mt][pos] = mul6(pos == 1 ? bias[mt] : z, cur, X[pos]);
          }
          __builtin_amdgcn_sched_barrier(0);
        }
#ifdef RWB_STAMP
        const unsigned long long c2 = __builtin_readcyclecounter();
#endif
        if (do2) finish(Sdy2);
#ifdef RWB_STAMP
        const unsigned long long c3 = __builtin_readcyclecounter();
        if (threadIdx.x == 0 && blockIdx.x == 7 && t >= 2 && t < n) {
          g_rwb_stamp[0] += c1 - c0, g_rwb_stamp[1] += c2 - c1, g_rwb_stamp[2] += c3 - c2, g_rwb_stamp[3] += 1;
        }
        if (threadIdx.x == 0 && blockIdx.x == 7 && !(t >= 2 && t < n)) {
          const int e = t < 2 ? t : (t == n ? 2 : 3);
          g_rwb_stamp[11 + e] += c3 - c0;
        }
#endif
      };

#ifdef RWB_STAMP
      const unsigned long long p1 = __builtin_readcyclecounter();
#endif
      load_row();
      Wa = wread(0);
      for (int t = 0;;) {
        step(S1, S2, S0, t);
        if (++t > n + 1) break;
        step(S2, S0, S1, t);
        if (++t > n + 1) break;
        step(S0, S1, S2, t);
        if (++t > n + 1) break;
      }
#ifdef RWB_STAMP
      if (threadIdx.x == 0 && blockIdx.x == 7) {
        g_rwb_stamp[8] += __builtin_readcyclecounter() - p1, g_rwb_stamp[9] += 1, g_rwb_stamp[10] += n;
      }
#endif

    }
  }
}

}
```

curla_amd/csrc/options.h:

```cpp
#pragma once

enum CurlaOpt {
  kOptConv1U8 = 0,
  kOptConv1F32,
  kOptS1Fwd,
  kOptBwdSplit,
  kOptGemmTile,
  kOptLinearBwd,
  kOptGemmMfma,
  kOptS1Wgrad,
  kOptWgrad1U8,
  kOptCount
};

enum Conv1U8Opt { kConv1U8Auto, kConv1U8Hybrid, kConv1U8Band, kConv1U8Rw, kConv1U8Rwb, kConv1U8Values };
enum Conv1F32Opt { kConv1F32Rw, kConv1F32Band, kConv1F32Values };
enum S1FwdOpt { kS1FwdAuto, kS1FwdF23, kS1FwdF43, kS1FwdB3, kS1FwdValues };
enum BwdSplitOpt { kBwdSplitAuto, kBwdSplitOff, kBwdSplitOn, kBwdSplitValues };
enum GemmTileOpt { kGemmTileAuto, kGemmTile6464, kGemmTile6432, kGemmTile3232, kGemmTile12864, kGemmTileValues };
enum LinearBwdOpt { kLinearBwdPair, kLinearBwdSplit, kLinearBwdValues };
enum GemmMfmaOpt { kGemmMfmaAuto, kGemmMfmaF32, kGemmMfmaB3, kGemmMfmaValues };
enum S1WgradOpt { kS1WgradAuto, kS1WgradX, kS1WgradXY, kS1WgradValues };
enum Wgrad1U8Opt { kWgrad1U8Auto, kWgrad1U8F32, kWgrad1U8B16, kWgrad1U8Values };

int curla_opt(int id);
```

curla_amd/csrc/options.hip:

```cpp
#include "options.h"

#include <atomic>
#include <cctype>
#include <cstdlib>
#include <cstring>
#include <mutex>

#include "../../include/curla_hip.h"

namespace {

struct OptDef {
  const char* name;
  const char* values[6];
  const char* alias[6];
};

constexpr OptDef kDefs[kOptCount] = {
    {"conv1_u8", {"auto", "hybrid", "band", "rw", "rwb", nullptr}, {nullptr, nullptr, nullptr, nullptr, nullptr, nullptr}},
    {"conv1_f32", {"rw", "band", nullptr}, {nullptr, nullptr, nullptr}},
    {"s1_fwd", {"auto", "f23", "f43", "b3", nullptr}, {nullptr, nullptr, nullptr, "bf16x3", nullptr}},
    {"bwd_split", {"auto", "0", "1", nullptr}, {nullptr, "off", "on", nullptr}},
    {"gemm_tile", {"auto", "6464", "6432", "3232", "12864", nullptr}, {nullptr, "64x64", "64x32", "32x32", "128x64", nullptr}},
    {"linear_bwd", {"pair", "split", nullptr}, {nullptr, nullptr, nullptr}},
    {"gemm_mfma", {"auto", "f32", "b3", nullptr}, {nullptr, nullptr, "bf16x3", nullptr}},
    {"s1_wgrad", {"auto", "x", "xy", nullptr}, {nullptr, "1d", "2d", nullptr}},
    {"wgrad1_u8", {"auto", "f32", "b16", nullptr}, {nullptr, nullptr, "bf16", nullptr}},
};

constexpr int kValueCount[kOptCount] = {kConv1U8Values, kConv1F32Values, kS1FwdValues, kBwdSplitValues, kGemmTileValues,
                                        kLinearBwdValues, kGemmMfmaValues, kS1WgradValues, kWgrad1U8Values};
constexpr bool value_counts_match() {
  for (int id = 0; id < kOptCount; ++id)
    if (!kDefs[id].values[kValueCount[id] - 1] || kDefs[id].values[kValueCount[id]]) return false;
  return true;
}
static_assert(value_counts_match(), "options.h names a different number of values than kDefs lists for some option");

std::atomic<int> g_value[kOptCount];
std::once_flag g_once;

int parse(const OptDef& d, const char* text) {
  for (int i = 0; i < 6 && d.values[i]; ++i)
    if (!strcmp(text, d.values[i]) || (d.alias[i] && !strcmp(text, d.alias[i]))) return i;
  return -1;
}

void init_from_env() {
  for (int id = 0; id < kOptCount; ++id) {
    char env[64] = "CURLA_";
    size_t n = strlen(env);
    for (const char* p = kDefs[id].name; *p && n + 1 < sizeof(env); ++p) env[n++] = (char)toupper((unsigned char)*p);
    env[n] = 0;
    const char* e = getenv(env);
    const int v = e ? parse(kDefs[id], e) : 0;
    g_value[id].store(v < 0 ? 0 : v, std::memory_order_relaxed);
  }
}

int find(const char* name) {
  if (!name) return -1;
  for (int id = 0; id < kOptCount; ++id)
    if (!strcmp(name, kDefs[id].name)) return id;
  return -1;
}

}

int curla_opt(int id) {
  std::call_once(g_once, init_from_env);
  return g_value[id].load(std::memory_order_relaxed);
}

extern "C" {

int curla_set_option(const char* name, const char* value) {
  std::call_once(g_once, init_from_env);
  const int id = find(name);
  if (id < 0 || !value) return CURLA_ERR_ARG;
  const int v = parse(kDefs[id], value);
  if (v < 0) return CURLA_ERR_ARG;
  g_value[id].store(v, std::memory_order_relaxed);
  return CURLA_OK;
}

const char* curla_get_option(const char* name) {
  std::call_once(g_once, init_from_env);
  const int id = find(name);
  return id < 0 ? nullptr : kDefs[id].values[g_value[id].load(std::memory_order_relaxed)];
}

}
```

curla_amd/curl_sac.py:

```python
import os
import warnings

import numpy as np
import torch
import torch.nn as nn

from . import autograd, ops
from .augmentations import RandomCrop
from .encoder import CNNEncoder
from .ops import ObsRef
from .optim import FlatAdam

LOG_FREQ = 25_000


def weight_init(m):
    if isinstance(m, nn.Linear):
        nn.init.orthogonal_(m.weight.data)
        if m.bias is not None:
            m.bias.data.zero_()
        return
    if isinstance(m, (nn.Conv2d, nn.ConvTranspose2d)):
        kh, kw = m.weight.shape[2:]
        assert kh == kw, "square kernels only"
# ... 623 lines not shown
                raise ValueError("empty batch of observations: " + want)
            shape = (len(x),) + tuple(np.shape(x[0]))
            if any(tuple(np.shape(f)) != shape[1:] for f in x):
                raise ValueError("observations of different shapes in one batch: " + want)
            if not all(isinstance(f, np.ndarray) and f.dtype == np.uint8 for f in x):
                x = np.stack([np.asarray(f.cpu() if torch.is_tensor(f) else f) for f in x])
        if len(shape) != 4 or shape[0] < 1 or shape[1] != C or shape[2:] not in windows:
            raise ValueError("observation batch of shape %s: %s" % (shape, want))
        if noise is not None and not (torch.is_tensor(noise) and tuple(noise.shape) == (shape[0], A)):
            raise ValueError("noise of shape %s: expected an (N, A) = (%d, %d) tensor"
                             % (tuple(getattr(noise, "shape", ())), shape[0], A))
        from . import _lib
        if self.device.type != "cuda" and _lib._trace_hook is None:
            raise RuntimeError("CurlSacAgent.select_actions / sample_actions need a CUDA/HIP device: the acting path "
                               "has no CPU fallback")
        return x, shape, windows[shape[2:]]

    def _stage_obs_batch(self, x, shape, window):
        N, C, H, W = shape
        top, left = window
        h, w = self.image_shape
        if torch.is_tensor(x) and x.dtype == torch.uint8 and not x.is_cuda:
            x = x.numpy()
        on_device = torch.is_tensor(x) and x.dtype == torch.uint8
        if not (on_device or isinstance(x, list) or (isinstance(x, np.ndarray) and x.dtype == np.uint8)):
            if torch.is_tensor(x):
                return x[:, :, top:top + h, left:left + w].to(self.device, torch.float32).contiguous()
            return torch.FloatTensor(np.ascontiguousarray(x[:, :, top:top + h, left:left + w])).to(self.device)
        cuda = self.device.type == "cuda"
        st = self._act_batch_stage.get((C, H, W))
        if st is None or st["cap"] < N:
            ring = torch.zeros(N * h * w * C + 32, dtype=torch.uint8, device=self.device)
            st = self._act_batch_stage[(C, H, W)] = dict(cap=N, ring=ring, src=None, pins=None, turn=0)
        n_src = N * C * H * W
        if on_device:
            src = x.to(self.device).contiguous()
        else:
            if st["src"] is None:
                cap = st["cap"] * C * H * W
                st["src"] = torch.empty(cap, dtype=torch.uint8, device=self.device)
                pins = [torch.empty(cap, dtype=torch.uint8, pin_memory=cuda) for _ in range(self._ACT_PINS)]
                st["pins"] = [(p, p.numpy(), torch.cuda.Event() if cuda else None) for p in pins]
            k = st["turn"]
            st["turn"] = (k + 1) % len(st["pins"])
            pin, pin_np, event = st["pins"][k]
            if cuda:
                event.synchronize()
            host = pin_np[:n_src].reshape(N, C, H, W)
            if isinstance(x, list):
                np.stack(x, out=host)
            else:
                np.copyto(host, x)
            src = st["src"][:n_src].view(N, C, H, W)
            src.copy_(pin[:n_src].view(N, C, H, W), non_blocking=True)
            if cuda:
                event.record()
        frames = st["ring"][:N * h * w * C].view(N, h, w, C)
        ops.stage_frames(src, frames, 0, top, left)
        return ops.ObsRef.from_ring(frames, None, None, None, N, (h, w))

    def select_actions(self, obs, as_tensor=False):
        x, shape, window = self._act_batch_args(obs, None)
        with torch.no_grad():
            mu, _, _, _ = self.actor(self._stage_obs_batch(x, shape, window), compute_pi=False, compute_log_pi=False)
        return mu if as_tensor else mu.cpu().numpy()

    def sample_actions(self, obs, noise=None, as_tensor=False):
        x, shape, window = self._act_batch_args(obs, noise)
        if noise is not None:
            noise = noise.detach().to(self.device, torch.float32).contiguous()
        with torch.no_grad():
            _, pi, _, _ = self.actor(self._stage_obs_batch(x, shape, window), compute_log_pi=False, noise=noise)
        return pi if as_tensor else pi.cpu().numpy()

    def _encoder_backward(self, ws, obs_ref, dz, xhat, rstd, enc, conv_grads=True, dense_done=None, twin_ld=None,
                          ln_token=None):
        B, F, K, L = obs_ref.B, enc.feature_dim, enc.flat_dim, enc.num_layers
        acts = ws.acts_main
        dy, dy2 = (dz, None) if twin_ld is None else (dz[0], dz[1])
        streams = ops.fc_bwd_streams(F, K)
        ln = ln_token if ln_token is not None else ops.ln_bwd(
            dy, xhat, rstd, enc.ln.weight, B, F, ws.dfc, dgamma=enc.ln.weight.grad, dbeta=enc.ln.bias.grad,
            dbias_in=enc.fc.bias.grad, dy2=dy2, ld=twin_ld, defer=ws.ln_partial if streams else None)
        h = acts[-1]
        cur = L % 2
        g = ws.gviews[cur][L - 1]
        if streams and conv_grads:
            ops.fc_bwd(ws.dfc, enc.fc.weight, h, g, enc.fc.weight.grad, B, F, K, ln=ln)
        elif streams:
            ops.fc_dw(ws.dfc, h, enc.fc.weight.grad, B, F, K, ln=ln)
        else:
            ops.linear_dw(ws.dfc, 0, h, 0, enc.fc.weight.grad, 0, B, F, K)
        if dense_done is not None:
            dense_done()
        if not conv_grads:
            return
        if not streams:
            ops.linear_dx(ws.dfc, 0, enc.fc.weight, 0, g, 0, B, F, K, mask=h)
        jobs = []
        for layer in range(L, 1, -1):
            conv = enc.convs[layer - 1]
            cur ^= 1
            gin = ws.gviews[cur][layer - 2]
            n = ops.conv_s1_bwd_slabs(acts[layer - 2], g, conv.weight, gin, ws.wg_ws[layer - 1])
            jobs.append((ws.wg_ws[layer - 1], n, conv.weight.grad, conv.bias.grad))
            g = gin
        n = ops.conv1_wgrad_slabs(obs_ref, g, ws.wg_ws[0], enc.num_filters)
        jobs.append((ws.wg_ws[0], n, enc.convs[0].weight.grad, enc.convs[0].bias.grad))
        for i in range(0, len(jobs), 8):
            ops.wgrad_reduce_multi(jobs[i:i + 8])

    def _records(self, step):
        return self.log_param_hist_imgs and step % LOG_FREQ == 0

    def _noise(self, ws, noise):
        if noise is not None:
            ws.noise.copy_(noise)
            return ws.noise, None
        if self._graph_cap is not None:
            cap = self._graph_cap
            addr = cap["rng"][cap["n_noise"]]
            cap["n_noise"] += 1
            return ws.noise, (0, 0, addr)
        if ws.noise.is_cuda and not self._noise_launch:
            try:
                gen = torch.cuda.default_generators[ws.noise.device.index if ws.noise.device.index is not None
                                                    else torch.cuda.current_device()]
                off = gen.get_offset()
                gen.set_offset(off + 4 * ((ws.noise.numel() + 3) // 4))
                return ws.noise, (gen.initial_seed(), off // 4)
            except (AttributeError, RuntimeError) as e:
                self._noise_launch = True
                warnings.warn(f"curla_amd: the torch generator exposes no Philox offset ({e!r}); policy noise falls "
                              "back to a separate normal_() launch per phase", RuntimeWarning, stacklevel=2)
        ws.noise.normal_()
        return ws.noise, None

    _noise_launch = False

    def update_critic(self, obs, action, reward, next_obs, not_done, L, step, noise=None):
        self._restore_grad_views()
        o, no = _as_ref(obs), _as_ref(next_obs)
        B, A, H = o.B, self.action_dim, self.hidden_dim
        enc, F = self.critic.encoder, self.critic.encoder.feature_dim
        ws = self._ws(B)
        self._anchor_cache = self._pos_cache = None
        self._pos_fc_done = False
        action, reward, not_done = action.contiguous(), reward.contiguous(), not_done.contiguous()

        pair = getattr(o, "pair", None)
        merged = pair is not None and pair[1] is no and pair[0].B == 2 * B
        tenc = self.critic_target.encoder
        if merged:
            enc.conv_forward2(pair[0], ws.acts_pair, tenc, no, ws.acts_tmp)
            h_next = ws.acts_pair[-1][B:]
        else:
            enc.conv_forward(no, ws.acts_tmp)
            h_next = ws.acts_tmp[-1]
        if merged:
            CNNEncoder.fc_partial_multi([(self.actor.encoder, h_next), (tenc, ws.acts_tmp[-1]), (enc, ws.acts_main[-1])])
        else:
            self.actor.encoder.fc_partial(h_next)
        four = merged and self._twin_outer is not None
        rec = self._records(step)
        if four:
            CNNEncoder.ln_from_partial_multi(B, [
                (self.actor.encoder, ws.z_a, {}), (tenc, ws.z_t, dict(xa=ws.xa2[0])),
                (enc, ws.z_c, dict(xhat=ws.xhat_c, rstd=ws.rstd_c, fc_out=ws.fc_out if rec else None, xa=ws.xa,
                                   act=action))], A)
        else:
            self.actor.encoder.ln_from_partial(B, ws.z_a)
        nz, rng = self._noise(ws, noise)
        _mlp_fwd(ws.z_a, 0, _Mlp(self.actor.trunk), 1, B, F, H, 2 * A, ws.a_h1, ws.a_h2, ws.a_out,
                 head=(nz, self.actor.log_std_min, self.actor.log_std_max,
                       dict(pi=None if four else ws.pi, log_pi=ws.log_pi, xa=ws.xa2[0] if four else None, rng=rng)))
        if four:
            _mlp_fwd(ws.xa2, 0, self.critic_target.twin(), 2, B, F + A, H, 1, ws.q_h1_2, ws.q_h2_2, ws.q2,
                     outer=(2, self._twin_outer))
        else:
            if not merged:
                tenc.conv_forward(no, ws.acts_tmp)
                tenc.fc_partial(ws.acts_tmp[-1])
            tenc.ln_from_partial(B, ws.z_t, xa=ws.xa, act=ws.pi)
            _mlp_fwd(ws.xa, 0, self.critic_target.twin(), 2, B, F + A, H, 1, ws.q_h1, ws.q_h2, ws.tq)
            if not merged:
                enc.conv_forward(o, ws.acts_main)
                enc.fc_partial(ws.acts_main[-1])
            enc.ln_from_partial(B, ws.z_c, xhat=ws.xhat_c, rstd=ws.rstd_c, fc_out=ws.fc_out if rec else None,
                                xa=ws.xa, act=action)
            _mlp_fwd(ws.xa, 0, self.critic.twin(), 2, B, F + A, H, 1, ws.q_h1, ws.q_h2, ws.q)
        if rec:
            self.critic.outputs['q1'], self.critic.outputs['q2'] = ws.q[0].clone(), ws.q[1].clone()
            enc.record_from(o, ws.acts_main, ws.fc_out, ws.z_c)
        td = (dict(kind=1, twin_stride=B, q=ws.q, target_q_twin=ws.tq, log_pi=ws.log_pi, reward=reward,
                   not_done=not_done, log_alpha=self.log_alpha, discount=self.discount, target_q=ws.target_q,
                   scalars=ws.scalars[0:1], dq=ws.dq),
              lambda: ops.critic_td_loss(ws.q, ws.tq, B, ws.log_pi, reward, not_done, self.log_alpha, self.discount, B,
                                         ws.target_q, ws.scalars[0:1], ws.dq))
        _mlp_bwd(ws.xa, 0, self.critic.twin(), self.critic.twin(grads=True), 2, B, F + A, H, 1, ws.q_h1, ws.q_h2, ws.dq,
                 ws.q_dh2, ws.q_dh1, ws.dxa, loss=td)
        if step % self.log_interval == 0:
            L.log('train_critic/loss', ws.scalars[0], step)
        lay = self._lay
        e0, total = lay["enc"][0], lay["total"]
        if self._dp_active and self._dp_overlap:
            cut = self._grad_offset(enc.fc.weight, self._critic_gflat)
            self._encoder_backward(ws, o, ws.dxa, ws.xhat_c, ws.rstd_c, enc, conv_grads=not self.detach_encoder,
                                   dense_done=lambda: self._allreduce(self._critic_gflat[cut:total], async_op=True),
                                   twin_ld=F + A)
            self._allreduce(self._critic_gflat[e0:cut], async_op=True)
            self._allreduce_wait()
        else:
            self._encoder_backward(ws, o, ws.dxa, ws.xhat_c, ws.rstd_c, enc, conv_grads=not self.detach_encoder,
                                   twin_ld=F + A)
            self._allreduce(self._critic_gflat[e0:total])
        if self.detach_encoder:
            saved = [(p, p.grad) for m in enc.convs for p in (m.weight, m.bias)]
            for p, _ in saved:
                p.grad = None
            self.critic_optimizer.step()
            for p, g in saved:
                p.grad = g
        else:
            fused = False
            if self._soft_update_hint:
                (e0, e1), (_, q1) = lay["enc"], lay["q"]
                fused = FlatAdam.step_with_lerp(self.critic_optimizer, self._target_flat, e0, q1, e1 - e0,
                                                self.encoder_tau, self.critic_tau)
                self._soft_update_done = fused
            if not fused:
                self.critic_optimizer.step()
        if self.log_param_hist_imgs:
            self.critic.log(L, step)

    def update_actor_and_alpha(self, obs, L, step, noise=None):
        self._restore_grad_views()
        o = _as_ref(obs)
        B, A, H = o.B, self.action_dim, self.hidden_dim
        enc, aenc, F = self.critic.encoder, self.actor.encoder, self.critic.encoder.feature_dim
        ws = self._ws(B)

        pos = self._pos_hint
        self._pos_hint = None
        if pos is not None:
            enc.conv_forward2(o, ws.acts_main, self.critic_target.encoder, pos, ws.acts_tmp)
            self._pos_cache = pos
        else:
            enc.conv_forward(o, ws.acts_main)
        h = ws.acts_main[-1]
        fcs = [(aenc, h), (enc, h)]
        if pos is not None:
            fcs.append((self.critic_target.encoder, ws.acts_tmp[-1]))
            self._pos_fc_done = True
        CNNEncoder.fc_partial_multi(fcs)
        lns = [(aenc, ws.z_a, dict(xhat=ws.xhat_a, rstd=ws.rstd_a)),
               (enc, ws.z_c, dict(xhat=ws.xhat_c, rstd=ws.rstd_c, xa=ws.xa))]
        if pos is not None:
            lns.append((self.critic_target.encoder, ws.z_pos, {}))
        CNNEncoder.ln_from_partial_multi(B, lns, A)
        self._anchor_cache = obs

        trunk = _Mlp(self.actor.trunk)
        nz, rng = self._noise(ws, noise)
        lo, hi = self.actor.log_std_min, self.actor.log_std_max
        _mlp_fwd(ws.z_a, 0, trunk, 1, B, F, H, 2 * A, ws.a_h1, ws.a_h2, ws.a_out,
                 head=(nz, lo, hi, dict(mu=ws.mu, pi=ws.pi, log_pi=ws.log_pi, log_std=ws.log_std, tanh_ls=ws.tanh_ls,
                                        xa=ws.xa, rng=rng)))
        if self._records(step):
            self.actor.outputs['mu'], self.actor.outputs['std'] = ws.a_out[:, :A].clone(), ws.log_std.exp()
        _mlp_fwd(ws.xa, 0, self.critic.twin(), 2, B, F + A, H, 1, ws.q_h1, ws.q_h2, ws.q)
        al = (dict(kind=2, A=A, twin_stride=B, q=ws.q, log_pi=ws.log_pi, log_std=ws.log_std, log_alpha=self.log_alpha,
                   target_entropy=float(self.target_entropy), scalars=ws.scalars[1:5], dq=ws.dq,
                   dlog_alpha=self.log_alpha.grad),
              lambda: ops.actor_loss(ws.q, B, ws.log_pi, ws.log_std, A, self.log_alpha, float(self.target_entropy), B,
                                     ws.scalars[1:5], ws.dq, self.log_alpha.grad))
        _mlp_bwd(ws.xa, 0, self.critic.twin(), None, 2, B, F + A, H, 1, ws.q_h1, ws.q_h2, ws.dq, ws.q_dh2, ws.q_dh1,
                 ws.dxa, loss=al)
        if step % self.log_interval == 0:
            L.log('train_actor/loss', ws.scalars[1], step)
            L.log('train_actor/target_entropy', self.target_entropy, step)
            L.log('train_actor/entropy', ws.scalars[3], step)
        ops.actor_head_bwd(None, self.log_alpha, 1.0 / B, nz, ws.pi, ws.log_std, ws.tanh_ls, B, A, lo, hi, ws.a_dout,
                           twin_dxa=ws.dxa, F=F)
        _mlp_bwd(ws.z_a, 0, trunk, _Mlp(self.actor.trunk, grads=True), 1, B, F, H, 2 * A, ws.a_h1, ws.a_h2, ws.a_dout,
                 ws.a_dh2, ws.a_dh1, ws.dz)
        streams = ops.fc_bwd_streams(F, enc.flat_dim)
        ln = ops.ln_bwd(ws.dz, ws.xhat_a, ws.rstd_a, aenc.ln.weight, B, F, ws.dfc, dgamma=aenc.ln.weight.grad,
                        dbeta=aenc.ln.bias.grad, dbias_in=aenc.fc.bias.grad, defer=ws.ln_partial if streams else None)
        if streams:
            ops.fc_dw(ws.dfc, h, aenc.fc.weight.grad, B, F, enc.flat_dim, ln=ln)
        else:
            ops.linear_dw(ws.dfc, 0, h, 0, aenc.fc.weight.grad, 0, B, F, enc.flat_dim)

        rider = (self.log_alpha.grad, self._la_words)
        if self._dp_active and self._dp_overlap:
            self._allreduce(self._actor_gbucket, async_op=True, f64_rider=rider)
            if self._defer_actor_step and not self.log_param_hist_imgs:
                self._actor_step_pending = True
            else:
                self._allreduce_wait()
        else:
            self._allreduce(self._actor_gbucket, f64_rider=rider)
        if not self._actor_step_pending:
            self._actor_steps()
        if self.log_param_hist_imgs:
            self.actor.log(L, step)
        if step % self.log_interval == 0:
            L.log('train_alpha/loss', ws.scalars[2], step)
            L.log('train_alpha/value', ws.scalars[4], step)

    _defer_actor_step = False
    _actor_step_pending = False

    def _actor_steps(self):
        if isinstance(self.actor_optimizer, FlatAdam):
            FlatAdam.step_with_scalar(self.actor_optimizer, self.log_alpha_optimizer)
        else:
            self.actor_optimizer.step()
            self.log_alpha_optimizer.step()

    def _finish_actor_step(self):
        if self._actor_step_pending:
            self._actor_step_pending = False
            self._allreduce_wait()
            self._actor_steps()

    def update_cpc(self, obs_anchor, obs_pos, cpc_kwargs, L, step):
        self._restore_grad_views()
        oa, op_ = _as_ref(obs_anchor), _as_ref(obs_pos)
        B = oa.B
        enc, tenc, F = self.critic.encoder, self.critic_target.encoder, self.critic.encoder.feature_dim
        ws = self._ws(B)
        need_anchor = self._anchor_cache is None or self._anchor_cache is not obs_anchor
        need_pos = self._pos_cache is None or self._pos_cache is not obs_pos
        pos_fc_done = self._pos_fc_done and not need_pos
        self._anchor_cache = self._pos_cache = None
        self._pos_fc_done = False
        if need_anchor and need_pos:
            enc.conv_forward2(oa, ws.acts_main, tenc, op_, ws.acts_tmp)
        elif need_anchor:
            enc.conv_forward(oa, ws.acts_main)
        elif need_pos:
            tenc.conv_forward(op_, ws.acts_tmp)
        if need_anchor:
            CNNEncoder.fc_partial_multi([(enc, ws.acts_main[-1]), (tenc, ws.acts_tmp[-1])])
            CNNEncoder.ln_from_partial_multi(B, [(enc, ws.z_c, dict(xhat=ws.xhat_c, rstd=ws.rstd_c)),
                                                 (tenc, ws.z_pos, {})])
        elif not pos_fc_done:
            tenc.fc_partial(ws.acts_tmp[-1])
            tenc.ln_from_partial(B, ws.z_pos)

        W = self.CURL.W
        ops.linear_fwd(ws.z_pos, 0, W, 0, None, 0, ws.WzT, 0, B, F, F)
        logged = step % self.log_interval == 0
        token = None
        if ops.curl_head_supported(B, F) and ops.fc_bwd_streams(F, enc.flat_dim) and not self._curl_unfused:
            token = ops.curl_head(ws.z_c, ws.z_pos, ws.WzT, ws.xhat_c, ws.rstd_c, enc.ln.weight, B, F, ws.row_loss, ws.dfc,
                                  ws.ln_partial, ws.w_partial, enc.ln.weight.grad, enc.ln.bias.grad, enc.fc.bias.grad,
                                  W.grad, loss=ws.scalars[5:6] if logged else None, logits=ws.logits, dz=ws.dz)
        else:
            ops.linear_fwd(ws.z_c, 0, ws.WzT, 0, None, 0, ws.logits, 0, B, B, F)
            ops.curl_ce(ws.logits, B, B, ws.row_loss, ws.scalars[5:6] if logged else None, ws.dlogits)
            ops.linear_dx(ws.dlogits, 0, ws.WzT, 0, ws.dz, 0, B, B, F)
            ops.linear_dw(ws.dlogits, 0, ws.z_c, 0, ws.dWzT, 0, B, B, F)
            ops.linear_dw(ws.dWzT, 0, ws.z_pos, 0, W.grad, 0, B, F, F)
        e1 = self._lay["enc"][1]
        if self._dp_active and self._dp_overlap:
            cut = self._grad_offset(enc.fc.weight, self._critic_gflat)
            self._encoder_backward(ws, oa, ws.dz, ws.xhat_c, ws.rstd_c, enc, ln_token=token,
                                   dense_done=lambda: self._allreduce(self._critic_gflat[cut:e1], async_op=True))
            self._allreduce(self._critic_gflat[0:cut], async_op=True)
            self._allreduce_wait()
        else:
            self._encoder_backward(ws, oa, ws.dz, ws.xhat_c, ws.rstd_c, enc, ln_token=token)
            self._allreduce(self._critic_gflat[0:e1])
        if isinstance(self.encoder_optimizer, FlatAdam):
            FlatAdam.step_pair(self.encoder_optimizer, self.cpc_optimizer)
        else:
            self.encoder_optimizer.step()
            self.cpc_optimizer.step()
        if step % self.log_interval == 0:
            L.log('train/curl_loss', ws.scalars[5], step)

    def soft_update_targets(self):
        lay = self._lay
        (e0, e1), (q0, q1) = lay["enc"], lay["q"]
        assert e1 == q0
        ops.soft_update2(self._critic_flat[e0:q1], self._target_flat[e0:q1], e1 - e0, self.encoder_tau, self.critic_tau)

    def update(self, replay_buffer, L, step, only_cpc=False, noise=None):
        self._restore_grad_views()
        self._check_n_step(replay_buffer)
        if noise is None and self._graphs is not None and self._graph_usable(replay_buffer, step, only_cpc):
            return self._update_graphed(replay_buffer, L, step)
        self._update_eager(replay_buffer, L, step, only_cpc, noise)

    def _check_n_step(self, replay_buffer):
        if getattr(replay_buffer, "n_step", 1) > 1 and replay_buffer.discount != self.discount:
            raise ValueError("replay_buffer.discount = %r (n_step = %d) differs from the agent's discount = %r"
                             % (replay_buffer.discount, replay_buffer.n_step, self.discount))

    def _update_eager(self, replay_buffer, L, step, only_cpc=False, noise=None):
        if hasattr(replay_buffer, "sample_cpc_refs"):
            sample = replay_buffer.sample_cpc_refs()
        else:
            sample = replay_buffer.sample_cpc()

        if self._dp_active and self._dp_check_every > 0 and step % self._dp_check_every == 0:
            self.check_replicas()
        self._update_phases(sample, L, step, only_cpc, noise)

    def _update_phases(self, sample, L, step, only_cpc=False, noise=None):
        obs, action, reward, next_obs, not_done, cpc_kwargs = sample
        noise_c, noise_a = noise if noise is not None else (None, None)
        if step % self.log_interval == 0:
            ws = self._ws(action.shape[0])
            ops.mean(reward.contiguous(), reward.numel(), ws.scalars[6:7])
            L.log('train/batch_reward', ws.scalars[6], step)

        do_cpc = (not self.pixel_sac) and step % self.cpc_update_freq == 0
        if not only_cpc:
            soft = step % self.critic_target_update_freq == 0
            self._soft_update_hint, self._soft_update_done = soft, False
            try:
                self.update_critic(obs, action, reward, next_obs, not_done, L, step, noise=noise_c)
            finally:
                self._soft_update_hint = False
            if soft and not self._soft_update_done:
                self.soft_update_targets()
            if step % self.actor_update_freq == 0:
                if do_cpc and isinstance(cpc_kwargs.get("obs_pos"), ObsRef):
                    self._pos_hint = cpc_kwargs["obs_pos"]
                self._defer_actor_step = do_cpc
                try:
                    self.update_actor_and_alpha(obs, L, step, noise=noise_a)
                finally:
                    self._pos_hint = None
                    self._defer_actor_step = False

        if do_cpc:
            obs_anchor, obs_pos = cpc_kwargs["obs_anchor"], cpc_kwargs["obs_pos"]
            self.update_cpc(obs_anchor, obs_pos, cpc_kwargs, L, step)
        self._finish_actor_step()

    def enable_update_graphs(self, replay_buffer, warm=1, depth=2):
        if self.device.type != "cuda":
            raise RuntimeError("update graphs need the HIP device")
        if not getattr(replay_buffer, "graph_supported", lambda: False)():
            raise ValueError("enable_update_graphs: this replay buffer / augmentation is not graph-replayable "
                             "(covered: RandomCrop, RandomShift or identity, plain storage with both rings in one "
                             "allocation or dedup_frames storage; ColorJiggle / NoisyCover "
                             "only on a ReplayBuffer constructed with staged_aug=True; pinned index slots, i.e. not "
                             "CURLA_STAGE_COPY=1)")
        opts = (self.critic_optimizer, self.actor_optimizer, self.encoder_optimizer, self.cpc_optimizer)
        if not all(isinstance(o, FlatAdam) and "step" not in vars(o) for o in opts) or \
                type(self.log_alpha_optimizer) is not torch.optim.Adam or self._noise_launch:
            raise ValueError("enable_update_graphs needs the FlatAdam optimizers and the in-kernel policy noise")
        self._graphs = {}
        self._graph_rb = replay_buffer
        self._graph_warm = int(warm)
        self._graph_depth = max(1, int(depth))
        self._graph_seen = {}
        self._graph_key_at_capture = None

    def disable_update_graphs(self):
        self._graphs = None

    def _graph_kind(self, step):
        return (step % self.actor_update_freq == 0, step % self.critic_target_update_freq == 0,
                (not self.pixel_sac) and step % self.cpc_update_freq == 0)

    def _graph_usable(self, replay_buffer, step, only_cpc):
        return (replay_buffer is self._graph_rb and not only_cpc and not (self._dp_active and not self._dp_avg)
                and not self._records(step) and step % self.log_interval != 0 and self.training)

    def _graph_live(self, opt):
        if opt is self.critic_optimizer and self.detach_encoder:
            convs = {id(p) for m in self.critic.encoder.convs for p in (m.weight, m.bias)}
            return [p for p in opt._plist if id(p) not in convs]
        return None

    def _graph_key(self):
        opts = (self.critic_optimizer, self.actor_optimizer, self.encoder_optimizer, self.cpc_optimizer,
                self.log_alpha_optimizer)
        hyper = tuple((float(g["betas"][0]), float(g["betas"][1]), float(g["eps"]), float(g.get("weight_decay", 0)))
                      for o in opts for g in o.param_groups)
        return (float(self.discount), float(self.critic_tau), float(self.encoder_tau), bool(self.detach_encoder),
                bool(self.pixel_sac), float(self.target_entropy), float(self.actor.log_std_min),
                float(self.actor.log_std_max), self.actor_update_freq, self.critic_target_update_freq,
                self.cpc_update_freq, self._dp_active, self._dp_overlap, id(self._dp_group) if self._dp_active else 0,
                hyper, self._graph_rb_key())

    def _graph_rb_key(self):
        rb = getattr(self, "_graph_rb", None)
        n = getattr(rb, "n_step", 1)
        return (n, float(rb.discount)) if n > 1 else (1, None)
# ... 190 lines not shown
```

curla_amd/encoder.py:

```python
import os

import torch
import torch.nn as nn

from . import autograd, ops


def tie_weights(src, trg):
    if type(src) is not type(trg):
        raise AssertionError("tie_weights needs two layers of the same type")
    trg.weight, trg.bias = src.weight, src.bias


def conv_out_hw(h, w, num_layers):
    h, w = (h - 3) // 2 + 1, (w - 3) // 2 + 1
    for _ in range(num_layers - 1):
        h, w = h - 2, w - 2
    return h, w


class _FcLinear(nn.Linear):

    nhwc = None

    def to_reference_layout(self, w):
        if self.nhwc is None:
            return w
        c, h, ww = self.nhwc
        return w.reshape(-1, h, ww, c).permute(0, 3, 1, 2).reshape(w.shape[0], -1)

    def from_reference_layout(self, w):
        if self.nhwc is None:
            return w
        c, h, ww = self.nhwc
        return w.reshape(-1, c, h, ww).permute(0, 2, 3, 1).reshape(w.shape[0], -1)

    def _save_to_state_dict(self, destination, prefix, keep_vars):
        super()._save_to_state_dict(destination, prefix, keep_vars)
        if self.nhwc is not None:
            destination[prefix + "weight"] = self.to_reference_layout(destination[prefix + "weight"].detach()).contiguous()

    def _load_from_state_dict(self, state_dict, prefix, *args, **kwargs):
        key = prefix + "weight"
        if self.nhwc is not None and key in state_dict:
            state_dict = dict(state_dict)
            state_dict[key] = self.from_reference_layout(state_dict[key]).contiguous()
        super()._load_from_state_dict(state_dict, prefix, *args, **kwargs)


class EncoderWorkspace:

    def __init__(self, enc, B, device):
        self.B = B
        self.acts = [torch.empty((B, h, w, enc.num_filters), device=device, dtype=torch.float32)
                     for (h, w) in enc.layer_hw[1:]]


class CNNEncoder(nn.Module):

    def __init__(self, obs_shape, feature_dim, num_layers=4, num_filters=32, output_logits=False):
        super().__init__()
        assert len(obs_shape) == 3
        c, h, w = obs_shape
        oh, ow = conv_out_hw(h, w, num_layers)
        if h < 3 or w < 3 or oh < 1 or ow < 1:
            raise NotImplementedError("Encoder does not support input shape")
        self.obs_shape = tuple(obs_shape)
        self.feature_dim = feature_dim
        self.num_layers = num_layers
        self.num_filters = num_filters
        self.convs = nn.ModuleList([nn.Conv2d(c, num_filters, 3, stride=2)])
        for _ in range(num_layers - 1):
            self.convs.append(nn.Conv2d(num_filters, num_filters, 3, stride=1))
        hw = [(h, w), ((h - 3) // 2 + 1, (w - 3) // 2 + 1)]
        for _ in range(num_layers - 1):
            hw.append((hw[-1][0] - 2, hw[-1][1] - 2))
        self.layer_hw = hw
        self.out_dim = hw[-1]
        self.flat_dim = num_filters * hw[-1][0] * hw[-1][1]
        self.fc = _FcLinear(self.flat_dim, feature_dim)
        self.ln = nn.LayerNorm(feature_dim)
        self.outputs = dict()
        self.output_logits = output_logits
        self.record_outputs = False
        self._ws = {}
        self._partial = {}
        self._nsplit = {}

    def workspace(self, B, tag="infer"):
        key = (B, tag)
        if key not in self._ws:
            self._ws[key] = EncoderWorkspace(self, B, self.fc.weight.device)
        return self._ws[key]

    def conv_params(self):
        return [(m.weight, m.bias) for m in self.convs]

    def ksplit(self, B):
        mt = (B + 63) // 64
        ks = max(1, min(32, 512 // mt))
        return min(ks, max(1, self.flat_dim // 256))

    def partial(self, B):
        if B not in self._partial:
            ns = max(self.ksplit(B), ops.FC_FWD_MAX_SPLIT if self._streams(B) else 1)
            self._partial[B] = torch.empty((ns, B, self.feature_dim), device=self.fc.weight.device, dtype=torch.float32)
        return self._partial[B]

    def _streams(self, B):
        return os.environ.get("CURLA_FC_FWD") != "gemm" and ops.fc_fwd_supported(B, self.feature_dim, self.flat_dim)

    def nsplit(self, B):
        return self._nsplit.get(B, self.ksplit(B))

    def conv_forward(self, obs_ref, acts, conv_params=None):
        cp = conv_params or self.conv_params()
        L = self.num_layers
        ops.conv1_fwd(obs_ref, cp[0][0], cp[0][1], acts[0])
        if L > 2 and ops.conv_s1_fwd_stack(acts[0], [cp[i][0] for i in range(1, L)], [cp[i][1] for i in range(1, L)],
                                           acts[1:L]):
            return acts[-1]
        for i in range(1, L):
            ops.conv_s1_fwd(acts[i - 1], cp[i][0], cp[i][1], acts[i])
        return acts[-1]

    def conv_forward2(self, obs_ref, acts, other, other_ref, other_acts):
        cp, cp2 = self.conv_params(), other.conv_params()
        if self.num_layers != other.num_layers or acts[0].shape[1:] != other_acts[0].shape[1:]:
            self.conv_forward(obs_ref, acts)
            other.conv_forward(other_ref, other_acts)
            return
        if ops.conv1_pairable(obs_ref, other_ref):
            ops.conv1_fwd2(obs_ref, cp[0][0], cp[0][1], acts[0], other_ref, cp2[0][0], cp2[0][1], other_acts[0])
        else:
            ops.conv1_fwd(obs_ref, cp[0][0], cp[0][1], acts[0])
            ops.conv1_fwd(other_ref, cp2[0][0], cp2[0][1], other_acts[0])
        L = self.num_layers
        if L > 1 and ops.conv_s1_fwd_stack(acts[0], [cp[i][0] for i in range(1, L)], [cp[i][1] for i in range(1, L)],
                                           acts[1:L], other_acts[0], [cp2[i][0] for i in range(1, L)],
                                           [cp2[i][1] for i in range(1, L)], other_acts[1:L]):
            return
        for i in range(1, L):
            ops.conv_s1_fwd2(acts[i - 1], cp[i][0], cp[i][1], acts[i], other_acts[i - 1], cp2[i][0], cp2[i][1],
                             other_acts[i])

    def head_forward(self, h, z, fc_out=None, xhat=None, rstd=None, xa=None, act=None):
        self.fc_partial(h)
        return self.ln_from_partial(h.shape[0], z, fc_out=fc_out, xhat=xhat, rstd=rstd, xa=xa, act=act)

    def fc_partial(self, h):
        B = h.shape[0]
        if self.fc.nhwc is None:
            raise RuntimeError("encoder weights are not in kernel layout; call CNNEncoder.to_kernel_layout() "
                               "(CurlSacAgent does) before running the HIP path")
        F, K = self.feature_dim, self.flat_dim
        if self._streams(B):
            ns = self._nsplit[B] = ops.fc_fwd_nsplit(1, B, K)
            ops.fc_fwd_multi([h], [self.fc.weight], [self.partial(B)], B, F, K, ns, B * F)
            return
        self._nsplit[B] = self.ksplit(B)
        ops.gemm(h, 0, K, 0, self.fc.weight, 0, K, 0, self.partial(B), F, 0, B, F, K, 1, ksplit=self.ksplit(B),
                 split_stride=B * F)

    @staticmethod
    def fc_partial_multi(pairs):
        enc0, h0 = pairs[0]
        B, F, K = h0.shape[0], enc0.feature_dim, enc0.flat_dim
        same = all(e.feature_dim == F and e.flat_dim == K and h.shape[0] == B and e.fc.nhwc is not None for e, h in pairs)
        if not same or len(pairs) > 4 or len(pairs) < 2:
            for e, h in pairs:
                e.fc_partial(h)
            return
        if enc0._streams(B):
            ns = ops.fc_fwd_nsplit(len(pairs), B, K)
            for e, _ in pairs:
                e._nsplit[B] = ns
            ops.fc_fwd_multi([h for _, h in pairs], [e.fc.weight for e, _ in pairs], [e.partial(B) for e, _ in pairs], B, F,
                             K, ns, B * F)
            return
        for e, _ in pairs:
            e._nsplit[B] = enc0.ksplit(B)
        ops.gemm_multi([h for _, h in pairs], [e.fc.weight for e, _ in pairs], [e.partial(B) for e, _ in pairs], B, F, K,
                       ksplit=enc0.ksplit(B), split_stride=B * F)

    def ln_from_partial(self, B, z, fc_out=None, xhat=None, rstd=None, xa=None, act=None):
        F = self.feature_dim
        ops.fc_ln_fwd(self.partial(B), self.nsplit(B), B * F, F, self.fc.bias, self.ln.weight, self.ln.bias, B, F, z,
                      fc_out=fc_out, xhat=xhat, rstd=rstd, eps=self.ln.eps, tanh_out=0 if self.output_logits else 1,
                      xa=xa, act=act)
        return z

    @staticmethod
    def ln_from_partial_multi(B, jobs, A=0):
        enc0 = jobs[0][0]
        F = enc0.feature_dim
        assert all(e.feature_dim == F and e.nsplit(B) == enc0.nsplit(B) and e.ln.eps == enc0.ln.eps for e, _, _ in jobs)
        ops.fc_ln_fwd_multi([dict(partial=e.partial(B), bias=e.fc.bias, gamma=e.ln.weight, beta=e.ln.bias, y=z,
                                  tanh_out=0 if e.output_logits else 1, **kw) for e, z, kw in jobs],
                            enc0.nsplit(B), B * F, F, B, F, enc0.ln.eps, A)

    def to_kernel_layout(self):
        if self.fc.nhwc is None:
            nhwc = (self.num_filters,) + tuple(self.out_dim)
            with torch.no_grad():
                self.fc.nhwc = nhwc
                self.fc.weight.data.copy_(self.fc.from_reference_layout(self.fc.weight.data.clone()))
        return self

    def _forward_conv_nhwc(self, obs):
        ref = obs if isinstance(obs, ops.ObsRef) else ops.ObsRef.from_tensor(obs.contiguous().float())
        ws = self.workspace(ref.B)
        self.conv_forward(ref, ws.acts)
        if self.record_outputs:
            self._record(ws.acts)
        return ref, ws.acts[-1]

    def _record(self, acts):
        for i, a in enumerate(acts):
            out = torch.empty((a.shape[0], a.shape[3], a.shape[1], a.shape[2]), device=a.device, dtype=a.dtype)
            ops.nhwc_to_nchw(a, out)
            self.outputs["conv%s" % (i + 1)] = out

    def _wants_graph(self, obs, convs=True):
        ps = self.parameters() if convs else (self.fc.weight, self.fc.bias, self.ln.weight, self.ln.bias)
        return autograd.wants_graph(obs, *ps)

    def forward_conv(self, obs):
        if autograd.wants_graph(obs, *[t for m in self.convs for t in (m.weight, m.bias)]):
            return autograd.forward_conv(self, obs)
        ref, h = self._forward_conv_nhwc(obs)
        out = torch.empty((h.shape[0], h.shape[3], h.shape[1], h.shape[2]), device=h.device, dtype=h.dtype)
        ops.nhwc_to_nchw(h, out)
        return out.view(ref.B, -1)

    def forward(self, obs, detach=False):
        if self._wants_graph(obs, convs=not detach):
            return autograd.encoder_forward(self, obs, detach)
        ref, h = self._forward_conv_nhwc(obs)
        h = h.view(ref.B, -1)
        z = torch.empty((h.shape[0], self.feature_dim), device=h.device, dtype=torch.float32)
        fc_out = torch.empty_like(z) if self.record_outputs else None
        self.head_forward(h, z, fc_out=fc_out)
        if self.record_outputs:
            self.outputs["fc"] = fc_out
            self.outputs["ln" if self.output_logits else "tanh"] = z
        return z

    def copy_conv_weights_from(self, source):
        for mine, theirs in zip(self.convs, source.convs):
            tie_weights(src=theirs, trg=mine)

    def record_from(self, obs_ref, acts, fc_out, z):
        if obs_ref.is_u8 == 1:
            x = torch.empty((obs_ref.B, obs_ref.C, obs_ref.Hc, obs_ref.Wc), device=z.device, dtype=torch.float32)
            ops.crop_nchw(obs_ref.src, obs_ref.idx, obs_ref.h1, obs_ref.w1, obs_ref.B, (obs_ref.Hc, obs_ref.Wc), out_f32=x)
        elif obs_ref.is_u8 == 2:
            x = torch.empty((obs_ref.B, obs_ref.C, obs_ref.Hc, obs_ref.Wc), device=z.device, dtype=torch.float32)
            ops.nhwc_to_nchw(obs_ref.src, x)
        else:
            x = obs_ref.src.clone()
        self.outputs['obs'] = x.div_(255.0)
        for i, a in enumerate(acts):
            out = torch.empty((a.shape[0], a.shape[3], a.shape[1], a.shape[2]), device=a.device, dtype=a.dtype)
            ops.nhwc_to_nchw(a, out)
            self.outputs['conv%s' % (i + 1)] = out
        self.outputs['fc'] = fc_out.clone()
        self.outputs['ln' if self.output_logits else 'tanh'] = z.clone()

    def log(self, L, step, log_freq):
        if step % log_freq:
            return
        for name, value in self.outputs.items():
            L.log_histogram('train_encoder/%s_hist' % name, value, step)
            if value.dim() > 2:
                L.log_image('train_encoder/%s_img' % name, value[0], step)
        for n, conv in enumerate(self.convs, start=1):
            L.log_param('train_encoder/conv%s' % n, conv, step)
        L.log_param('train_encoder/fc', self.fc, step)
        L.log_param('train_encoder/ln', self.ln, step)


PixelEncoder = CNNEncoder
```

curla_amd/ops.py:

```python
import ctypes

import torch

from . import _lib
from ._lib import call, ptr, stream

F32 = torch.float32


def _dev(t, dtype=F32):
    if not ((t.is_cuda or _lib._trace_hook is not None) and t.dtype == dtype and t.is_contiguous()):
        raise _lib.CurlaHipError(f"expected a contiguous {dtype} CUDA tensor, got {t.dtype} {t.device} "
                                 f"contiguous={t.is_contiguous()}")
    return t


class ObsRef:

    __slots__ = ("src", "is_u8", "idx", "h1", "w1", "B", "C", "Hs", "Ws", "Hc", "Wc", "guard", "pair")

    def __init__(self):
        self.guard = None
        self.pair = None

    @staticmethod
    def from_ring(frames, idx, h1, w1, B, crop_hw, guard=None):
        o = ObsRef()
        _dev(frames, torch.uint8)
        o.src, o.is_u8, o.idx, o.h1, o.w1, o.B = frames, 1, idx, h1, w1, B
        _, o.Hs, o.Ws, o.C = frames.shape
        o.Hc, o.Wc = crop_hw
        o.guard = guard
        return o

    def check(self):
        g = self.guard
        if g is not None and g[0][g[1]] != g[2]:
            raise _lib.CurlaHipError("stale minibatch handle: the replay buffer has drawn further samples since and "
                                     "recycled this one's device index block (ReplayBuffer.N_SAMPLE_SLOTS handles "
                                     "are valid at a time)")
        return self

    @staticmethod
    def from_nhwc(x):
        o = ObsRef()
        _dev(x)
        o.src, o.is_u8, o.idx, o.h1, o.w1 = x, 2, None, None, None
        o.B, o.Hc, o.Wc, o.C = x.shape
        o.Hs, o.Ws = o.Hc, o.Wc
        return o

    @staticmethod
    def from_tensor(x):
        o = ObsRef()
        _dev(x)
        o.src, o.is_u8, o.idx, o.h1, o.w1 = x, 0, None, None, None
        o.B, o.C, o.Hc, o.Wc = x.shape
        o.Hs, o.Ws = o.Hc, o.Wc
        return o


def conv1_fwd(obs: ObsRef, w, b, out, scale=1.0 / 255.0):
    obs.check()
    call("curla_conv1_fwd", ptr(obs.src), obs.is_u8, ptr(obs.idx), ptr(obs.h1), ptr(obs.w1), ptr(w), ptr(b), ptr(out),
         obs.B, obs.C, obs.Hs, obs.Ws, obs.Hc, obs.Wc, w.shape[0], scale, stream())


def conv1_wgrad(obs: ObsRef, g, dw, db, ws, scale=1.0 / 255.0):
    obs.check()
    call("curla_conv1_wgrad", ptr(obs.src), obs.is_u8, ptr(obs.idx), ptr(obs.h1), ptr(obs.w1), ptr(g), ptr(dw), ptr(db),
         ptr(ws), obs.B, obs.C, obs.Hs, obs.Ws, obs.Hc, obs.Wc, dw.shape[0], scale, stream())


def conv_s1_fwd(x, w, b, out):
    B, H, W, C = x.shape
    call("curla_conv3x3_s1_fwd", ptr(x), ptr(w), ptr(b), ptr(out), B, H, W, C, stream())


def conv_s1_fwd2(x, w, b, out, x2, w2, b2, out2):
    B, H, W, C = x.shape
    assert x2.shape[1:] == x.shape[1:]
    call("curla_conv3x3_s1_fwd2", ptr(x), ptr(w), ptr(b), ptr(out), B, ptr(x2), ptr(w2), ptr(b2), ptr(out2), x2.shape[0],
         H, W, C, stream())


def conv_s1_fwd_stack(x, ws, bs, outs, x2=None, ws2=None, bs2=None, outs2=None):
    import ctypes
    B, H, W, C = x.shape
    n = len(ws)
    B2 = 0 if x2 is None else x2.shape[0]
    G = stack_granule()
    if n > 6 or B % G or B2 % G or C != 32:
        return False
    P = ctypes.c_void_p * n
    arr = lambda ts: P(*[ptr(t) for t in ts])
    a_w, a_b, a_o = arr(ws), arr(bs), arr(outs)
    if B2:
        assert x2.shape[1:] == x.shape[1:]
        a_w2, a_b2, a_o2 = arr(ws2), arr(bs2), arr(outs2)
        p2 = (ptr(x2), ctypes.addressof(a_w2), ctypes.addressof(a_b2), ctypes.addressof(a_o2))
    else:
        p2 = (None, None, None, None)
    call("curla_conv3x3_s1_fwd_stack", n, ptr(x), ctypes.addressof(a_w), ctypes.addressof(a_b), ctypes.addressof(a_o), B,
         p2[0], p2[1], p2[2], p2[3], B2, H, W, C, stream())
    return True


_PER_DEVICE = {}


def _device_cached(what, compute):
    key = (what, torch.cuda.current_device())
    if key not in _PER_DEVICE:
        _PER_DEVICE[key] = compute()
    return _PER_DEVICE[key]


def stack_granule():
    if _lib._trace_hook is not None:
        return 256
    return _device_cached("stack_granule", lambda: int(_lib.load().curla_conv3x3_s1_stack_granule()))


def cu_count():
    if _lib._trace_hook is not None:
        return 256
    return _device_cached("cus", lambda: torch.cuda.get_device_properties(torch.cuda.current_device()).multi_processor_count)


def conv1_pairable(o1: "ObsRef", o2: "ObsRef"):
    return (o1.is_u8 == 1 and o2.is_u8 == 1 and o1.src.data_ptr() == o2.src.data_ptr() and o1.src.shape == o2.src.shape
            and (o1.Hc, o1.Wc) == (o2.Hc, o2.Wc))


def conv1_fwd2(o1: "ObsRef", w, b, out, o2: "ObsRef", w2, b2, out2, scale=1.0 / 255.0):
    o1.check(), o2.check()
    call("curla_conv1_fwd2", ptr(o1.src), ptr(o1.idx), ptr(o1.h1), ptr(o1.w1), ptr(w), ptr(b), ptr(out), o1.B, ptr(o2.idx),
         ptr(o2.h1), ptr(o2.w1), ptr(w2), ptr(b2), ptr(out2), o2.B, o1.C, o1.Hs, o1.Ws, o1.Hc, o1.Wc, w.shape[0], scale,
         stream())


def conv_s1_dgrad(g, w, act_below, gin):
    B, H, W, C = g.shape
    call("curla_conv3x3_s1_dgrad", ptr(g), ptr(w), ptr(act_below), ptr(gin), B, H, W, C, stream())


def conv_s1_wgrad(x, g, dw, db, ws):
    B, H, W, C = x.shape
    call("curla_conv3x3_s1_wgrad", ptr(x), ptr(g), ptr(dw), ptr(db), ptr(ws), B, H, W, C, stream())


def conv_s1_wgrad_slabs(x, g, ws):
    import ctypes
    B, H, W, C = x.shape
    n = ctypes.c_int(1)
    call("curla_conv3x3_s1_wgrad_slabs", ptr(x), ptr(g), ptr(ws), B, H, W, C, ctypes.addressof(n), stream())
    return n.value


def conv_s1_bwd_slabs(x, g, w, gin, ws):
    import ctypes
    B, H, W, C = x.shape
    n = ctypes.c_int(1)
    call("curla_conv3x3_s1_bwd_slabs", ptr(x), ptr(g), ptr(w), ptr(gin), ptr(ws), B, H, W, C, ctypes.addressof(n),
         stream())
    return n.value


def conv1_wgrad_slabs(obs: ObsRef, g, ws, channels, scale=1.0 / 255.0):
    import ctypes
    obs.check()
    n = ctypes.c_int(1)
    call("curla_conv1_wgrad_slabs", ptr(obs.src), obs.is_u8, ptr(obs.idx), ptr(obs.h1), ptr(obs.w1), ptr(g), ptr(ws),
         obs.B, obs.C, obs.Hs, obs.Ws, obs.Hc, obs.Wc, channels, scale, ctypes.addressof(n), stream())
    return n.value


def conv1_dgrad(g, w, dobs, scale=1.0 / 255.0):
    B, C, H, W = dobs.shape
    _dev(g), _dev(dobs)
    call("curla_conv1_dgrad", ptr(g), ptr(w), ptr(dobs), B, C, H, W, w.shape[0], scale, stream())


def wgrad_reduce_multi(jobs):
    import ctypes
    n = len(jobs)
    P, I = ctypes.c_void_p * n, ctypes.c_int * n
    slabs = P(*[ptr(j[0]) for j in jobs])
    ns = I(*[int(j[1]) for j in jobs])
    nw = I(*[int(j[2].numel()) for j in jobs])
    nb = I(*[int(j[3].numel()) for j in jobs])
    dw = P(*[ptr(j[2]) for j in jobs])
    db = P(*[ptr(j[3]) for j in jobs])
    call("curla_wgrad_reduce_multi", n, ctypes.addressof(slabs), ctypes.addressof(ns), ctypes.addressof(nw),
         ctypes.addressof(nb), ctypes.addressof(dw), ctypes.addressof(db), stream())


def wgrad_workspace_floats(cin):
    if _lib._trace_hook is not None:
        return 512 * (32 * cin * 9 + 32)
    return int(_lib.load().curla_conv_wgrad_workspace_floats(cin))


def gemm(A, a_kmajor, lda, sA, Bm, b_kmajor, ldb, sB, C, ldc, sC, M, N, K, nbatch=1, ksplit=1, split_stride=0,
         alpha=1.0, bias=None, sBias=0, relu=0, mask=None, ldmask=0, sMask=0):
    call("curla_gemm", ptr(A), a_kmajor, lda, sA, ptr(Bm), b_kmajor, ldb, sB, ptr(C), ldc, sC, M, N, K, nbatch, ksplit,
         split_stride, alpha, ptr(bias), sBias, relu, ptr(mask), ldmask, sMask, stream())


def gemm_multi(As, Bs, Cs, M, N, K, ksplit=1, split_stride=0):
    import ctypes
    n = len(As)
    P = ctypes.c_void_p * n
    a, b, c = P(*[ptr(t) for t in As]), P(*[ptr(t) for t in Bs]), P(*[ptr(t) for t in Cs])
    call("curla_gemm_multi", n, ctypes.addressof(a), ctypes.addressof(b), ctypes.addressof(c), K, K, N, M, N, K, ksplit,
         split_stride, stream())


FC_FWD_MAX_SPLIT = 64


def fc_fwd_supported(B, F_, K):
    return 50 <= F_ <= 64 and F_ % 2 == 0 and B % 128 == 0 and K % 32 == 0 and B * K * 4 < 2 ** 31 and F_ * K * 4 < 2 ** 31

# ... 431 lines not shown
```

include/curla_hip.h:

```cpp
#ifndef CURLA_HIP_H
#define CURLA_HIP_H

#include <stddef.h>
#include <stdint.h>

#ifdef __cplusplus
extern "C" {
#endif

#define CURLA_OK 0
#define CURLA_ERR_ARG (-1)
#define CURLA_ERR_LAUNCH (-2)
#define CURLA_ERR_UNSUPPORTED (-3)

const char* curla_version(void);

#define CURLA_ABI_VERSION 8
int curla_abi_version(void);

int curla_set_option(const char* name, const char* value);
const char* curla_get_option(const char* name);


int curla_conv1_fwd(const void* src, int src_kind, const int64_t* idx, const int32_t* h1, const int32_t* w1,
                    const float* w, const float* bias, float* out, int B, int C, int Hs, int Ws, int Hc, int Wc,
                    int channels, float scale, void* stream);
int curla_conv1_fwd2(const uint8_t* ring, const int64_t* idx, const int32_t* h1, const int32_t* w1, const float* w,
                     const float* bias, float* out, int B, const int64_t* idx2, const int32_t* h1_2,
                     const int32_t* w1_2, const float* w2, const float* bias2, float* out2, int B2, int C, int Hs, int Ws,
                     int Hc, int Wc, int channels, float scale, void* stream);

int curla_conv3x3_s1_fwd(const float* in, const float* w, const float* bias, float* out, int B, int Hi, int Wi,
                         int channels, void* stream);
int curla_conv3x3_s1_fwd2(const float* in, const float* w, const float* bias, float* out, int B, const float* in2,
                          const float* w2, const float* bias2, float* out2, int B2, int Hi, int Wi, int channels,
                          void* stream);
int curla_conv3x3_s1_fwd_stack(int nlayers, const float* in, const float* const* w, const float* const* bias,
                               float* const* out, int B, const float* in2, const float* const* w2,
                               const float* const* bias2, float* const* out2, int B2, int Hi, int Wi, int channels,
                               void* stream);
int curla_conv3x3_s1_stack_granule(void);

int curla_conv3x3_s1_dgrad(const float* g, const float* w, const float* act_below, float* gin, int B, int Ho, int Wo,
                           int channels, void* stream);
int curla_conv3x3_s1_wgrad(const float* in, const float* g, float* dw, float* db, float* workspace, int B, int Hi,
                           int Wi, int channels, void* stream);
int curla_conv1_wgrad(const void* src, int src_kind, const int64_t* idx, const int32_t* h1, const int32_t* w1,
                      const float* g, float* dw, float* db, float* workspace, int B, int C, int Hs, int Ws, int Hc,
                      int Wc, int channels, float scale, void* stream);
int curla_conv3x3_s1_wgrad_slabs(const float* in, const float* g, float* workspace, int B, int Hi, int Wi, int channels,
                                 int* nslabs, void* stream);
int curla_conv1_wgrad_slabs(const void* src, int src_kind, const int64_t* idx, const int32_t* h1, const int32_t* w1,
                            const float* g, float* workspace, int B, int C, int Hs, int Ws, int Hc, int Wc, int channels,
                            float scale, int* nslabs, void* stream);
int curla_conv3x3_s1_bwd_slabs(const float* in, const float* g, const float* w, float* gin, float* workspace, int B, int Hi,
                               int Wi, int channels, int* nslabs, void* stream);
int curla_conv1_dgrad(const float* g, const float* w, float* dobs, int B, int C, int H, int W, int channels,
                      float scale, void* stream);
int curla_wgrad_reduce_multi(int njobs, const float* const* slabs, const int* nslabs, const int* nw, const int* nb,
                             float* const* dw, float* const* db, void* stream);
size_t curla_conv_wgrad_workspace_floats(int cin);

int curla_gemm(const float* A, int a_kmajor, int lda, long long strideA, const float* B, int b_kmajor, int ldb,
               long long strideB, float* C, int ldc, long long strideC, int M, int N, int K, int nbatch, int ksplit,
               long long split_stride, float alpha, const float* bias, long long strideBias, int relu,
               const float* mask, int ldmask, long long strideMask, void* stream);
int curla_gemm_small_shape(int M, int N, int K, int nbatch);
int curla_gemm_colsum(const float* A, int a_kmajor, int lda, long long strideA, const float* B, int b_kmajor, int ldb,
                      long long strideB, float* C, int ldc, long long strideC, int M, int N, int K, int nbatch,
                      float* colsum, long long strideColsum, void* stream);
int curla_linear_bwd(const float* dy, long long stride_dy, const float* x, long long stride_x, const float* W,
                     long long stride_W, const float* mask, long long stride_mask, float* dW, long long stride_dW,
                     float* db, long long stride_db, float* dx, long long stride_dx, int B, int N, int K, int nbatch,
                     void* stream);
int curla_gemm_nested(const float* A, int a_kmajor, int lda, long long strideA, long long strideA2, const float* B,
                      int b_kmajor, int ldb, long long strideB, long long strideB2, float* C, int ldc, long long strideC,
                      long long strideC2, int M, int N, int K, int nbatch, int nbatch2, float alpha, const float* bias,
                      long long strideBias, long long strideBias2, int relu, const float* mask, int ldmask,
                      long long strideMask, long long strideMask2, void* stream);
int curla_gemm_multi(int nprob, const float* const* A, const float* const* B, float* const* C, int lda, int ldb, int ldc,
                     int M, int N, int K, int ksplit, long long split_stride, void* stream);
int curla_fc_fwd_multi(int nprob, const float* const* x, const float* const* W, float* const* partial, int B, int F, int K,
                       int nsplit, long long split_stride, int x_blocked, void* stream);
int curla_splitk_reduce(const float* partial, int nsplit, long long split_stride, int M, int N, int ldp, float* C,
                        int ldc, const float* bias, int relu, void* stream);
int curla_fc_dx(const float* dz, const float* W, const float* mask, float* dx, int B, int F, int K, void* stream);
int curla_fc_dw(const float* dz, const float* x, float* dW, int B, int F, int K, void* stream);
int curla_fc_bwd(const float* dz, const float* W, const float* x, float* dx, float* dW, int B, int F, int K,
                 void* stream);
int curla_fc_bwd_ln(const float* dz, const float* W, const float* x, float* dx, float* dW, int B, int F, int K,
                    const float* ln_partial, int nparts, float* dgamma, float* dbeta, float* dbias_in, void* stream);
int curla_fc_dw_ln(const float* dz, const float* x, float* dW, int B, int F, int K, const float* ln_partial, int nparts,
                   float* dgamma, float* dbeta, float* dbias_in, void* stream);
int curla_fc_bwd_ln2(const float* dz, const float* W, const float* x, float* dx, float* dW, int B, int F, int K,
                     const float* ln_partial, int nparts, float* dgamma, float* dbeta, float* dbias_in,
                     const float* extra_partial, int extra_parts, int extra_len, float* extra_out, void* stream);

int curla_mlp_out_fwd(const float* h, long long strideH, const float* W, long long strideW, const float* bias,
                      long long strideBias, float* out, long long strideOut, int M, int N, int K, int nbatch,
                      void* stream);
int curla_mlp_out_fwd_nested(const float* h, long long strideH, long long strideH2, const float* W, long long strideW,
                             long long strideW2, const float* bias, long long strideBias, long long strideBias2,
                             float* out, long long strideOut, long long strideOut2, int M, int N, int K, int nbatch,
                             int nbatch2, void* stream);
int curla_mlp_out_bwd(const float* dy, long long strideDy, const float* h, long long strideH, const float* W,
                      long long strideW, float* dh, long long strideDh, float* dW, long long strideDW, int M, int N,
                      int K, int nbatch, void* stream);
int curla_mlp_out_bwd_bias(const float* dy, long long strideDy, const float* h, long long strideH, const float* W,
                           long long strideW, float* dh, long long strideDh, float* dW, long long strideDW, int M, int N,
                           int K, int nbatch, float* db_out, float* db_hidden, long long strideDb, void* stream);

typedef struct CurlaFcLnJob {
  const float *partial, *bias, *gamma, *beta;
  float *fc_out, *y, *xhat, *rstd, *xa;
  const float* act;
  int tanh_out;
} CurlaFcLnJob;
typedef struct CurlaLossArgs {
  int kind, A;
  long long twin_stride;
  const float *q, *target_q_twin, *log_pi, *reward, *not_done, *log_std;
  const double* log_alpha;
  double* dlog_alpha;
  float *target_q, *scalars, *dq;
  float discount, target_entropy;
} CurlaLossArgs;
int curla_mlp_out_bwd_loss(const CurlaLossArgs* loss, const float* h, long long strideH, const float* W,
                           long long strideW, float* dh, long long strideDh, float* dW, long long strideDW, int B, int K,
                           float* db_out, float* db_hidden, long long strideDb, void* stream);
int curla_fc_ln_fwd(const float* partial, int nsplit, long long split_stride, int ldp, const float* bias,
                    const float* gamma, const float* beta, int B, int F, float eps, float* fc_out, float* y,
                    float* xhat, float* rstd, int tanh_out, float* xa, const float* act, int A, void* stream);
int curla_fc_ln_fwd_multi(int njobs, const CurlaFcLnJob* jobs, int nsplit, long long split_stride, int ldp, int B,
                          int F, float eps, int A, void* stream);
int curla_ln_bwd(const float* dy, const float* xhat, const float* rstd, const float* gamma, int B, int F, float* dx,
                 float* dgamma, float* dbeta, float* dbias_in, void* stream);
int curla_ln_bwd_twin(const float* dy, const float* dy2, int ld_dy, const float* xhat, const float* rstd,
                      const float* gamma, int B, int F, float* dx, float* dgamma, float* dbeta, float* dbias_in,
                      void* stream);
int curla_ln_bwd_partial(const float* dy, const float* dy2, int ld_dy, const float* xhat, const float* rstd,
                         const float* gamma, int B, int F, float* dx, float* partial, int* nparts, void* stream);
int curla_colsum(const float* X, int M, int N, int ldx, long long strideX, float* out, long long strideOut, int nbatch,
                 void* stream);

int curla_colsum3(const float* X0, int N0, const float* X1, int N1, const float* X2, int N2, int M, float* out0,
                  float* out1, float* out2, long long strideOut, int nbatch, void* stream);

int curla_actor_head_fwd(const float* trunk_out, const float* noise, int B, int A, float log_std_min,
                         float log_std_max, float* mu, float* pi, float* log_pi, float* log_std, float* tanh_ls,
                         float* pi_xa, int xa_ld, void* stream);
int curla_mlp_out_head_fwd(const float* h, const float* W, const float* bias, float* trunk_out, int B, int A, int K,
                           const float* noise, float log_std_min, float log_std_max, float* mu, float* pi,
                           float* log_pi, float* log_std, float* tanh_ls, float* pi_xa, int xa_ld, void* stream);
int curla_actor_head_fwd_rng(const float* trunk_out, float* noise_out, unsigned long long seed,
                             unsigned long long offset, const unsigned long long* rng_dev, int B, int A,
                             float log_std_min, float log_std_max, float* mu, float* pi, float* log_pi, float* log_std,
                             float* tanh_ls, float* pi_xa, int xa_ld, void* stream);
int curla_mlp_out_head_fwd_rng(const float* h, const float* W, const float* bias, float* trunk_out, int B, int A, int K,
                               float* noise_out, unsigned long long seed, unsigned long long offset,
                               const unsigned long long* rng_dev, float log_std_min, float log_std_max, float* mu,
                               float* pi, float* log_pi, float* log_std, float* tanh_ls, float* pi_xa, int xa_ld,
                               void* stream);
int curla_actor_head_bwd(const float* gpi, const float* gpi2, int gpi_ld, const float* glp_rows, const double* log_alpha,
                         float glp_scale, const float* noise, const float* pi, const float* log_std,
                         const float* tanh_ls, int B, int A, float log_std_min, float log_std_max, float* dtrunk_out,
                         void* stream);
int curla_policy_head_bwd(const float* dmu, const float* dpi, const float* dlog_pi, const float* dlog_std,
                          const float* noise, const float* mu, const float* pi, const float* log_std,
                          const float* tanh_ls, int B, int A, float log_std_min, float log_std_max, float* dtrunk_out,
                          void* stream);

int curla_concat(const float* z, const float* act, int B, int F, int A, float* xa, void* stream);
int curla_split_sum(const float* dxa, long long twin_stride, int B, int F, int A, float* dz, float* dact,
                    void* stream);

int curla_td_target(const float* tq, long long twin_stride, const float* log_pi, const float* reward,
                    const float* not_done, const double* log_alpha, float discount, int B, float* target_q,
                    void* stream);
int curla_critic_loss(const float* q, long long twin_stride, const float* target_q, int B, float* loss, float* dq,
                      void* stream);
int curla_critic_td_loss(const float* q, const float* tq, long long twin_stride, const float* log_pi,
                         const float* reward, const float* not_done, const double* log_alpha, float discount, int B,
                         float* target_q, float* loss, float* dq, void* stream);
// ... 72 lines not shown
```

Before: 511.7.

## Fuse conv1 and conv2 forward in LDS for no-grad target encoder passes

Adds a kernel that computes the stride-2 uint8 first conv layer into row bands held in LDS and runs the second 3x3 conv straight from those bands. It is used only for target-encoder forwards that need no gradient. This avoids writing the first layer's activations to global memory and reading them back, and saves one launch. The cost is the 1-wave-per-CU LDS footprint, a barrier between band production and consumption, and bands that must be recomputed per image. The no-grad path also has to fall back to the unpaired conv1 launch instead of the paired fwd2 kernel.

```diff
diff --git a/curla_amd/_lib.py b/curla_amd/_lib.py
--- a/curla_amd/_lib.py
+++ b/curla_amd/_lib.py
@@ -18,6 +18,8 @@
     "curla_conv3x3_s1_stack_granule": [],
     "curla_conv1_fwd2": [vp, vp, vp, vp, vp, vp, vp, c_int, vp, vp, vp, vp, vp, vp, c_int, c_int, c_int, c_int, c_int, c_int,
                          c_int, c_float, vp],
+    "curla_conv12_nograd_fwd": [vp, vp, vp, vp, vp, vp, vp, vp, vp, c_int, c_int, c_int, c_int, c_int, c_int, c_int, c_float,
+                                vp],
     "curla_conv3x3_s1_dgrad": [vp, vp, vp, vp, c_int, c_int, c_int, c_int, vp],
     "curla_conv3x3_s1_wgrad": [vp, vp, vp, vp, vp, c_int, c_int, c_int, c_int, vp],
     "curla_conv1_wgrad": [vp, c_int, vp, vp, vp, vp, vp, vp, vp, c_int, c_int, c_int, c_int, c_int, c_int, c_int,
diff --git a/curla_amd/csrc/conv.hip b/curla_amd/csrc/conv.hip
--- a/curla_amd/csrc/conv.hip
+++ b/curla_amd/csrc/conv.hip
@@ -176,6 +176,22 @@
     rw::conv1_u8b_body<C, kC1U8bThreads / 64, false>(a, lds_imgb, blockIdx.x, gridDim.x);
 }
 
+#include "conv12_nograd.h"
+
+template <int C>
+__global__ __launch_bounds__(512, 1) void conv12_nograd_kernel(ngf::Args a) {
+  extern __shared__ __attribute__((aligned(16))) unsigned short lds_h[];
+  unsigned char* lds = reinterpret_cast<unsigned char*>(lds_h);
+  rwb::build_filter<MODE_FWD, 512>(lds_h, a.wb, nullptr, threadIdx.x);
+  rw::conv1_u8b_stage_weights<C, 512>(lds + ngf::kImgOff, a.wa, a.ba, a.scale, threadIdx.x);
+  if (threadIdx.x < 64) reinterpret_cast<unsigned*>(lds + ngf::kZeroOff)[threadIdx.x] = 0u;
+  __syncthreads();
+  if ((a.Ws * C) % 4 == 0)
+    ngf::body<C, true>(a, lds, blockIdx.x, gridDim.x);
+  else
+    ngf::body<C, false>(a, lds, blockIdx.x, gridDim.x);
+}
+
 #include "conv1_band.h"
 
 constexpr int kPartialS1 = 32 * 288 + 32;
@@ -222,6 +238,8 @@
 
 constexpr int kMaxLds = 160 * 1024;
 static_assert(2 * rwb::kWBytes <= kMaxLds, "the two problems' split filters of conv_rwb_fwd_kernel must fit one CU's LDS");
+static_assert(ngf::kLdsBytes == kMaxLds && ngf::kBandOff == rwb::kWBytes + rw::kConv1U8B3ImageBytes + 256 && ngf::kBandBytes > 0,
+              "conv12_nograd_kernel: layer 2's filter, the first layer's image and the bands share one CU's LDS");
 template <typename K>
 int set_lds(K kernel, size_t bytes) {
   if (bytes > (size_t)kMaxLds) return CURLA_ERR_UNSUPPORTED;
@@ -679,6 +697,31 @@
   CURLA_REQUIRE(w2 && bias2 && out2 && B2 > 0);
   Conv1Second sec{idx2, h1_2, w1_2, w2, bias2, out2, B2};
   return conv1_fwd_impl(ring, kSrcU8Ring, idx, h1, w1, w, bias, out, B, C, Hs, Ws, Hc, Wc, channels, scale, stream, &sec);
+}
+
+int curla_conv12_nograd_fwd(const uint8_t* ring, const int64_t* idx, const int32_t* h1, const int32_t* w1, const float* wa,
+                            const float* ba, const float* wb, const float* bb, float* out2, int B, int C, int Hs, int Ws,
+                            int Hc, int Wc, int channels, float scale, void* stream) {
+  CURLA_REQUIRE(wa && ba && wb && bb && out2);
+  const int rc = conv1_common_check(ring, kSrcU8Ring, B, C, Hs, Ws, Hc, Wc);
+  if (rc != CURLA_OK) return rc;
+  if (curla_opt(kOptNogradFuse) == kNogradFuseOff || channels != 32 || C != 9) return CURLA_ERR_UNSUPPORTED;
+  CURLA_REQUIRE(aligned16(wb) && aligned16(bb) && aligned16(out2));
+  ngf::Args a;
+  a.src = ring, a.idx = idx, a.h1 = h1, a.w1 = w1, a.wa = wa, a.ba = ba, a.wb = wb, a.bb = bb, a.out = out2;
+  a.B = B, a.Hs = Hs, a.Ws = Ws, a.scale = scale;
+  a.Ho1 = (Hc - 3) / 2 + 1, a.Wo1 = (Wc - 3) / 2 + 1, a.Ho2 = a.Ho1 - 2, a.Wo2 = a.Wo1 - 2;
+  if (a.Ho2 < 1 || a.Wo2 < 1 || !rw_supported(a.Ho1, a.Wo1) || (long long)Hs * Ws * C >= (1LL << 30)) return CURLA_ERR_UNSUPPORTED;
+  a.ns1 = (a.Wo1 + 15) / 16, a.ns2 = ((a.Wo2 + 1) / 2 + 15) / 16;
+  const int row_bytes = a.Wo1 * ngf::kPixBytes;
+  a.S = 2 * a.ns2 <= ngf::kWaves && ngf::kBandBytes / (2 * row_bytes) >= 3 ? 2 : 1;
+  a.band = ngf::kBandBytes / (a.S * row_bytes) / 3 * 3;
+  if (a.ns2 > ngf::kWaves || a.band < 3) return CURLA_ERR_UNSUPPORTED;
+  a.band = std::min(a.band, (a.Ho1 + 2) / 3 * 3);
+  const int grid = std::min((B + a.S - 1) / a.S, curla_cu_count());
+  return dispatch_c<9>(C, [&](auto cc) {
+    return launch(conv12_nograd_kernel<cc()>, grid, 512, ngf::kLdsBytes, static_cast<hipStream_t>(stream), a);
+  });
 }
 
 size_t curla_conv_wgrad_workspace_floats(int cin) {
diff --git a/curla_amd/csrc/conv12_nograd.h b/curla_amd/csrc/conv12_nograd.h
--- /dev/null
+++ b/curla_amd/csrc/conv12_nograd.h
@@ -0,0 +1,193 @@
+#pragma once
+
+namespace ngf {
+
+using rwb::u32x4;
+
+struct Args {
+  const uint8_t* src;
+  const int64_t* idx;
+  const int32_t* h1;
+  const int32_t* w1;
+  const float* wa;
+  const float* ba;
+  const float* wb;
+  const float* bb;
+  float* out;
+  int B, Hs, Ws;
+  int Ho1, Wo1, Ho2, Wo2;
+  float scale;
+  int S;
+  int band;
+  int ns1, ns2;
+};
+
+constexpr int kPixBytes = 144;
+constexpr int kImgOff = rwb::kWBytes;
+constexpr int kZeroOff = kImgOff + rw::kConv1U8B3ImageBytes;
+constexpr int kBandOff = kZeroOff + 256;
+constexpr int kLdsBytes = 160 * 1024;
+constexpr int kBandBytes = kLdsBytes - kBandOff;
+constexpr int kWaves = 8;
+static_assert(kZeroOff % 16 == 0 && kBandOff % 16 == 0, "16-byte LDS accesses");
+static_assert(kBandBytes >= 2 * 3 * 64 * kPixBytes, "two units' bands of three rows of 64 pixels must fit");
+
+__device__ __forceinline__ unsigned chan4_off(const int i) {
+  const int q = i >> 1, h = i & 1;
+  return (unsigned)(q * 32 + ((h ^ (q & 1)) * 16));
+}
+
+struct LdsRows {
+  const unsigned char* lds;
+  unsigned a[4];
+  unsigned st[4];
+  int half;
+  __device__ __forceinline__ void load(f32x4 (&raw)[4][2]) const {
+#pragma unroll
+    for (int c = 0; c < 4; ++c) {
+      raw[c][0] = *reinterpret_cast<const f32x4*>(lds + a[c]);
+      raw[c][1] = *reinterpret_cast<const f32x4*>(lds + (a[c] + half));
+    }
+  }
+  __device__ __forceinline__ void advance() {
+#pragma unroll
+    for (int c = 0; c < 4; ++c) a[c] += st[c];
+  }
+};
+
+struct Crop {
+  const uint8_t* base;
+  int range;
+  int mis;
+};
+
+template <int C, bool AL>
+__device__ __forceinline__ void body(const Args& a, unsigned char* lds, const int bid, const int nblk) {
+  constexpr int NL = AL ? 3 : 2;
+  constexpr int CH = 4;
+  using Raw = rw::RawBytes<NL>;
+  const int lane = threadIdx.x & 63;
+  const int wave = __builtin_amdgcn_readfirstlane(threadIdx.x >> 6);
+  const int li = lane & 15, kq = lane >> 4;
+  const int in_row = a.Ws * C, frame = a.Hs * in_row;
+  const int row_bytes = a.Wo1 * kPixBytes, unit_bytes = a.band * row_bytes;
+  const int out_row = a.Wo2 * 128;
+  const int cnt = bid < a.B ? (a.B - bid + nblk - 1) / nblk : 0;
+
+  for (int i0 = 0; i0 < cnt; i0 += a.S) {
+    const int nu = cnt - i0 < a.S ? cnt - i0 : a.S;
+    Crop crop[2];
+#pragma unroll
+    for (int s = 0; s < 2; ++s) {
+      const int b = bid + (i0 + (s < nu ? s : 0)) * nblk;
+      const long long slot = a.idx ? rw::const_load(a.idx, b) : b;
+      const int origin = ((a.h1 ? rw::const_load(a.h1, b) : 0) * a.Ws + (a.w1 ? rw::const_load(a.w1, b) : 0)) * C;
+      const uint8_t* p = a.src + (size_t)slot * frame + origin;
+      crop[s].mis = AL ? (int)(reinterpret_cast<uintptr_t>(p) & 3) : 0;
+      crop[s].base = p - crop[s].mis;
+      crop[s].range = frame - origin + 16 + crop[s].mis;
+    }
+
+    const bool walks = wave < nu * a.ns2;
+    const int ws = walks ? wave / a.ns2 : 0, wk = walks ? wave - ws * a.ns2 : 0;
+    const int j = 16 * wk + li, x0 = 2 * j;
+    const bool lane_on = walks && j < (a.Wo2 + 1) / 2;
+    rwb::Walk<MODE_FWD, LdsRows> W;
+    rwb::Acc S0, S1, S2;
+    W.lw = reinterpret_cast<const u32x4*>(lds) + lane;
+    W.n = a.Ho2, W.out_row = out_row;
+    W.rout = rw::uniform_rsrc(a.out + (size_t)(bid + (i0 + ws) * nblk) * a.Ho2 * a.Wo2 * 32, a.Ho2 * out_row);
+    W.raux = W.rout;
+    W.oa = lane_on ? (unsigned)(x0 * 128 + kq * 16) : 0x80000000u;
+    W.ob = (lane_on && x0 + 1 < a.Wo2) ? W.oa + 128u : 0x80000000u;
+    W.bias[0] = *reinterpret_cast<const f32x4*>(a.bb + 4 * kq);
+    W.bias[1] = *reinterpret_cast<const f32x4*>(a.bb + 16 + 4 * kq);
+    W.src.lds = lds;
+    W.src.half = (kq & 1) ? -16 : 16;
+    unsigned row0[4];
+#pragma unroll
+    for (int c = 0; c < 4; ++c) {
+      const bool ok = lane_on && x0 + c < a.Wo1;
+      row0[c] = ok ? (unsigned)(kBandOff + ws * unit_bytes + (x0 + c) * kPixBytes) + chan4_off(2 * kq)
+                   : (unsigned)kZeroOff + chan4_off(2 * kq);
+      W.src.st[c] = ok ? (unsigned)row_bytes : 0u;
+    }
+
+    for (int r0 = 0; r0 < a.Ho1; r0 += a.band) {
+      const int r1 = r0 + a.band < a.Ho1 ? r0 + a.band : a.Ho1;
+      {
+        const int per_unit = (r1 - r0) * a.ns1, nitems = nu * per_unit;
+        const u32x4* wl = reinterpret_cast<const u32x4*>(lds + kImgOff) + lane;
+        const float* bl = reinterpret_cast<const float*>(lds + kImgOff + 3 * 2 * 3 * 64 * 16);
+        for (int base = wave; base < nitems; base += kWaves * CH) {
+          Raw R[CH][3];
+#pragma unroll
+          for (int q = 0; q < CH; ++q) {
+            const int it = base + q * kWaves;
+            if (it < nitems) {
+              const int s = it / per_unit, rem = it - s * per_unit, lr = rem / a.ns1, k1 = rem - lr * a.ns1;
+              const int x = 16 * k1 + li, mis = s ? crop[1].mis : crop[0].mis;
+              const __amdgpu_buffer_rsrc_t rin = rw::uniform_rsrc(s ? crop[1].base : crop[0].base, s ? crop[1].range : crop[0].range);
+              const unsigned run = (unsigned)((2 * (r0 + lr) * a.Ws + 2 * x) * C + 8 * kq + mis);
+              const unsigned vin = x < a.Wo1 ? (AL ? run & ~3u : run) : 0x80000000u;
+#pragma unroll
+              for (int rr = 0; rr < 3; ++rr)
+                rw::load_raw<NL>(R[q][rr], rin, vin, __builtin_amdgcn_readfirstlane((unsigned)(rr * in_row)));
+            }
+          }
+#pragma unroll
+          for (int q = 0; q < CH; ++q) {
+            const int it = base + q * kWaves;
+            if (it < nitems) {
+              const int s = it / per_unit, rem = it - s * per_unit, lr = rem / a.ns1, k1 = rem - lr * a.ns1;
+              const int x = 16 * k1 + li, mis = s ? crop[1].mis : crop[0].mis;
+              const unsigned sh = (unsigned)((2 * (r0 + lr) * a.Ws + 2 * x) * C + 8 * kq + mis) & 3u;
+              f32x4 acc[2];
+#pragma unroll
+              for (int mt = 0; mt < 2; ++mt) acc[mt] = *reinterpret_cast<const f32x4*>(bl + mt * 16 + 4 * kq);
+#pragma unroll
+              for (int dy = 0; dy < 3; ++dy) {
+                u32x4 wf[2][3];
+#pragma unroll
+                for (int mt = 0; mt < 2; ++mt)
+#pragma unroll
+                  for (int p = 0; p < 3; ++p) wf[mt][p] = wl[((dy * 2 + mt) * 3 + p) * 64];
+                unsigned f[4];
+                rw::u8b_convert<AL>(f, R[q][dy], sh);
+                rw::u8b_mma_row(acc, u32x4{f[0], f[1], f[2], f[3]}, wf);
+              }
+              if (x < a.Wo1) {
+                unsigned char* px = lds + (kBandOff + s * unit_bytes + lr * row_bytes + x * kPixBytes);
+#pragma unroll
+                for (int mt = 0; mt < 2; ++mt) {
+                  f32x4 v = acc[mt];
+#pragma unroll
+                  for (int r = 0; r < 4; ++r) v[r] = rw::relu_bits(v[r]);
+                  *reinterpret_cast<f32x4*>(px + chan4_off(4 * mt + kq)) = v;
+                }
+              }
+            }
+          }
+        }
+      }
+      __syncthreads();
+      if (walks) {
+#pragma unroll
+        for (int c = 0; c < 4; ++c) W.src.a[c] = row0[c];
+        W.src.load(W.raw);
+        W.Wa = W.wread(0);
+        for (int t = r0;;) {
+          W.step(S1, S2, S0, t, t + 1 < r1);
+          if (++t >= r1) break;
+          W.step(S2, S0, S1, t, t + 1 < r1);
+          if (++t >= r1) break;
+          W.step(S0, S1, S2, t, t + 1 < r1);
+          if (++t >= r1) break;
+        }
+      }
+      __syncthreads();
+    }
+  }
+}
+
+}
diff --git a/curla_amd/csrc/conv1_u8_rw.h b/curla_amd/csrc/conv1_u8_rw.h
--- a/curla_amd/csrc/conv1_u8_rw.h
+++ b/curla_amd/csrc/conv1_u8_rw.h
@@ -276,13 +276,35 @@
   if (tid < 32) reinterpret_cast<float*>(img + 3 * 2 * 3 * 64 * 16)[tid] = bias[tid];
 }
 
+template <bool AL>
+__device__ __forceinline__ void u8b_convert(unsigned (&F)[4], const RawBytes<(AL ? 3 : 2)>& R, const unsigned sh) {
+  RawBytes<2> Wd;
+#pragma unroll
+  for (int j = 0; j < 2; ++j) Wd.d[j] = AL ? __builtin_amdgcn_alignbyte(R.d[AL ? j + 1 : j], R.d[j], sh) : R.d[j];
+#pragma unroll
+  for (int q = 0; q < 4; ++q) {
+    const float f0 = byte_f32<2>(Wd, 2 * q), f1 = byte_f32<2>(Wd, 2 * q + 1);
+    F[q] = (__builtin_bit_cast(unsigned, f0) >> 16) | (__builtin_bit_cast(unsigned, f1) & 0xFFFF0000u);
+  }
+}
+
+typedef unsigned u8b_u4 __attribute__((ext_vector_type(4)));
+__device__ __forceinline__ void u8b_mma_row(f32x4 (&acc)[2], const u8b_u4& F, const u8b_u4 (&wf)[2][3]) {
+  typedef short bf16x8 __attribute__((ext_vector_type(8)));
+  const bf16x8 xb = __builtin_bit_cast(bf16x8, F);
+#pragma unroll
+  for (int p = 2; p >= 0; --p)
+#pragma unroll
+    for (int mt = 0; mt < 2; ++mt)
+      acc[mt] = __builtin_amdgcn_mfma_f32_16x16x32_bf16(__builtin_bit_cast(bf16x8, wf[mt][p]), xb, acc[mt], 0, 0, 0);
+}
+
 template <int C, int NW, bool AL>
 __device__ __forceinline__ void conv1_u8b_body(const Conv1U8Args& a, const unsigned char* lds_img, const int bid,
                                                const int nblk) {
   constexpr int E = 8;
   constexpr int NW_ = 2;
   constexpr int NL = AL ? 3 : NW_;
-  typedef short bf16x8 __attribute__((ext_vector_type(8)));
   typedef unsigned u4 __attribute__((ext_vector_type(4)));
   const int lane = threadIdx.x & 63;
   const int wave = __builtin_amdgcn_readfirstlane(threadIdx.x >> 6);
@@ -358,24 +380,11 @@
         load_raw<NL>(R, rin, vin, __builtin_amdgcn_readfirstlane((unsigned)(rr * in_row)));
       };
       auto convert = [&](u4& F, const Raw& R) {
-        RawBytes<NW_> Wd;
-#pragma unroll
-        for (int j = 0; j < NW_; ++j)
-          Wd.d[j] = AL ? __builtin_amdgcn_alignbyte(R.d[j + 1], R.d[j], sh) : R.d[j];
-#pragma unroll
-        for (int q = 0; q < 4; ++q) {
-          const float f0 = byte_f32<NW_>(Wd, 2 * q), f1 = byte_f32<NW_>(Wd, 2 * q + 1);
-          F[q] = (__builtin_bit_cast(unsigned, f0) >> 16) | (__builtin_bit_cast(unsigned, f1) & 0xFFFF0000u);
-        }
-      };
-      auto mma_row = [&](f32x4 (&acc)[2], const u4& F, const int dy) {
-        const bf16x8 xb = __builtin_bit_cast(bf16x8, F);
-#pragma unroll
-        for (int p = 2; p >= 0; --p)
-#pragma unroll
-          for (int mt = 0; mt < 2; ++mt)
-            acc[mt] = __builtin_amdgcn_mfma_f32_16x16x32_bf16(__builtin_bit_cast(bf16x8, wf[dy][mt][p]), xb, acc[mt], 0, 0, 0);
-      };
+        unsigned f[4];
+        u8b_convert<AL>(f, R, sh);
+        F = u4{f[0], f[1], f[2], f[3]};
+      };
+      auto mma_row = [&](f32x4 (&acc)[2], const u4& F, const int dy) { u8b_mma_row(acc, F, wf[dy]); };
       struct Pair {
         Raw a, b;
       };
diff --git a/curla_amd/csrc/conv_rwb.h b/curla_amd/csrc/conv_rwb.h
--- a/curla_amd/csrc/conv_rwb.h
+++ b/curla_amd/csrc/conv_rwb.h
@@ -86,6 +86,147 @@
 
 struct Acc {
   f32x4 m[2][4];
+};
+
+struct W3 {
+  u32x4 h, m, l;
+};
+
+struct GlobalRows {
+  __amdgpu_buffer_rsrc_t rin;
+  unsigned voff[4];
+  int in_row;
+  __device__ __forceinline__ void load(f32x4 (&raw)[4][2]) const {
+#pragma unroll
+    for (int c = 0; c < 4; ++c) {
+      raw[c][0] = __builtin_bit_cast(f32x4, __builtin_amdgcn_raw_buffer_load_b128(rin, voff[c], 0, 0));
+      raw[c][1] = __builtin_bit_cast(f32x4, __builtin_amdgcn_raw_buffer_load_b128(rin, voff[c] + 16u, 0, 0));
+    }
+  }
+  __device__ __forceinline__ void advance() {
+#pragma unroll
+    for (int c = 0; c < 4; ++c) voff[c] += in_row;
+  }
+};
+
+template <int MODE, class Src>
+struct Walk {
+  Src src;
+  const u32x4* lw;
+  __amdgpu_buffer_rsrc_t rout, raux;
+  unsigned oa, ob;
+  int out_row;
+  int n;
+  f32x4 bias[2];
+  f32x4 raw[4][2];
+  f32x4 mk[2][2];
+  W3 Wa, Wb;
+
+  __device__ __forceinline__ W3 wread(const int g) const {
+    const int pos = g / 6, dy = 2 - (g / 2) % 3, mt = g & 1;
+    const u32x4* p = lw + ((((dy * 4 + pos) * 2 + mt) * 3)) * 64;
+    W3 w;
+#if defined(RWB_ABL) && (RWB_ABL & 2)
+    w.h = p[0], w.m = w.h, w.l = w.h;
+    return w;
+#endif
+    w.h = p[0], w.m = p[64], w.l = p[128];
+    return w;
+  }
+
+  static __device__ __forceinline__ f32x4 mul6(f32x4 acc, const W3& w, const B3& x) {
+#if !(defined(RWB_ABL) && (RWB_ABL & 4))
+    acc = mfma_bf16(w.l, x.h, acc);
+    acc = mfma_bf16(w.h, x.l, acc);
+    acc = mfma_bf16(w.m, x.m, acc);
+#endif
+    acc = mfma_bf16(w.m, x.h, acc);
+    acc = mfma_bf16(w.h, x.m, acc);
+    acc = mfma_bf16(w.h, x.h, acc);
+    return acc;
+  }
+
+  __device__ __forceinline__ void finish(const Acc& S) {
+#pragma unroll
+    for (int mt = 0; mt < 2; ++mt) {
+      f32x4 ya = S.m[mt][0] + S.m[mt][1] + S.m[mt][2];
+      f32x4 yb = S.m[mt][1] - S.m[mt][2] - S.m[mt][3];
+      if (MODE == MODE_FWD) {
+#pragma unroll
+        for (int r = 0; r < 4; ++r) ya[r] = fmaxf(ya[r], 0.f), yb[r] = fmaxf(yb[r], 0.f);
+      } else {
+#pragma unroll
+        for (int r = 0; r < 4; ++r) ya[r] = mk[0][mt][r] > 0.f ? ya[r] : 0.f, yb[r] = mk[1][mt][r] > 0.f ? yb[r] : 0.f;
+      }
+      __builtin_amdgcn_raw_buffer_store_b128(__builtin_bit_cast(u32x4, ya), rout, oa + mt * 64u, 0, CURLA_ACT_STORE_POLICY);
+      __builtin_amdgcn_raw_buffer_store_b128(__builtin_bit_cast(u32x4, yb), rout, ob + mt * 64u, 0, CURLA_ACT_STORE_POLICY);
+    }
+    oa += out_row, ob += out_row;
+  }
+
+  __device__ __forceinline__ void step(Acc& Sdy2, Acc& Sdy1, Acc& Sdy0, const int t, const bool more) {
+#ifdef RWB_STAMP
+    const unsigned long long c0 = __builtin_readcyclecounter();
+#endif
+    B3 X[4];
+    {
+      float v[4][8];
+#pragma unroll
+      for (int c8 = 0; c8 < 8; ++c8) {
+        const float d0 = raw[0][c8 >> 2][c8 & 3], d1 = raw[1][c8 >> 2][c8 & 3], d2 = raw[2][c8 >> 2][c8 & 3],
+                    d3 = raw[3][c8 >> 2][c8 & 3];
+        v[0][c8] = d0 - d2, v[1][c8] = d1 + d2, v[2][c8] = d2 - d1, v[3][c8] = d1 - d3;
+      }
+#pragma unroll
+      for (int pos = 0; pos < 4; ++pos) X[pos] = split8(v[pos]);
+    }
+    if (more) {
+      src.advance();
+      src.load(raw);
+    }
+    const bool do2 = t >= 2, do1 = t >= 1 && t <= n, do0 = t < n;
+    if (MODE == MODE_DGRAD && do2) {
+#pragma unroll
+      for (int mt = 0; mt < 2; ++mt) {
+        mk[0][mt] = __builtin_bit_cast(f32x4, __builtin_amdgcn_raw_buffer_load_b128(raux, oa + mt * 64u, 0, 0));
+        mk[1][mt] = __builtin_bit_cast(f32x4, __builtin_amdgcn_raw_buffer_load_b128(raux, ob + mt * 64u, 0, 0));
+      }
+    }
+#ifdef RWB_STAMP
+    const unsigned long long c1 = __builtin_readcyclecounter();
+#endif
+#pragma unroll
+    for (int g = 0; g < 24; ++g) {
+      const int pos = g / 6, which = (g / 2) % 3, mt = g & 1;
+      W3& cur = (g & 1) ? Wb : Wa;
+      W3& nxt = (g & 1) ? Wa : Wb;
+      nxt = wread(g == 23 ? 0 : g + 1);
+      __builtin_amdgcn_sched_barrier(0);
+      if (which == 0) {
+        if (do2) Sdy2.m[mt][pos] = mul6(Sdy2.m[mt][pos], cur, X[pos]);
+      } else if (which == 1) {
+        if (do1) Sdy1.m[mt][pos] = mul6(Sdy1.m[mt][pos], cur, X[pos]);
+      } else {
+        const f32x4 z = {0, 0, 0, 0};
+        if (do0) Sdy0.m[mt][pos] = mul6(pos == 1 ? bias[mt] : z, cur, X[pos]);
+      }
+      __builtin_amdgcn_sched_barrier(0);
+    }
+#ifdef RWB_STAMP
+    const unsigned long long c2 = __builtin_readcyclecounter();
+#endif
+    if (do2) finish(Sdy2);
+#ifdef RWB_STAMP
+    const unsigned long long c3 = __builtin_readcyclecounter();
+    if (threadIdx.x == 0 && blockIdx.x == 7 && t >= 2 && t < n) {
+      g_rwb_stamp[0] += c1 - c0, g_rwb_stamp[1] += c2 - c1, g_rwb_stamp[2] += c3 - c2, g_rwb_stamp[3] += 1;
+    }
+    if (threadIdx.x == 0 && blockIdx.x == 7 && !(t >= 2 && t < n)) {
+      const int e = t < 2 ? t : (t == n ? 2 : 3);
+      g_rwb_stamp[11 + e] += c3 - c0;
+    }
+#endif
+  }
 };
 
 template <int MODE, int NW>
@@ -107,7 +248,6 @@
     const bool second = si >= cnt0;
     const Problem& P = second ? P1 : P0;
     const int b = bid + (second ? si - cnt0 : si) * nblk;
-    const u32x4* lw = reinterpret_cast<const u32x4*>(lds_w + (second ? kWBytes / 2 : 0)) + lane;
     for (int k = 0; k < nstrips; ++k) {
       const int n_strip = k < G.nfull ? G.Ho : G.nr;
       const int a0 = lo > before ? lo : before;
@@ -128,158 +268,41 @@
       }
       const int Y = y0 + sb;
       const int x0 = 2 * j;
-      const __amdgpu_buffer_rsrc_t rin = uniform_rsrc(P.in + (size_t)b * G.Hi * G.Wi * 32, G.Hi * in_row);
-      const __amdgpu_buffer_rsrc_t rout = uniform_rsrc(P.out + (size_t)b * G.Ho * G.Wo * 32, G.Ho * out_row);
-      const __amdgpu_buffer_rsrc_t raux = uniform_rsrc(MODE == MODE_DGRAD ? P.aux + (size_t)b * G.Ho * G.Wo * 32 : P.aux,
-                                                       MODE == MODE_DGRAD ? G.Ho * out_row : 128);
-      unsigned voff[4];
+      Walk<MODE, GlobalRows> W;
+      W.lw = reinterpret_cast<const u32x4*>(lds_w + (second ? kWBytes / 2 : 0)) + lane;
+      W.n = n, W.out_row = out_row;
+      W.src.rin = uniform_rsrc(P.in + (size_t)b * G.Hi * G.Wi * 32, G.Hi * in_row);
+      W.src.in_row = in_row;
+      W.rout = uniform_rsrc(P.out + (size_t)b * G.Ho * G.Wo * 32, G.Ho * out_row);
+      W.raux = uniform_rsrc(MODE == MODE_DGRAD ? P.aux + (size_t)b * G.Ho * G.Wo * 32 : P.aux,
+                            MODE == MODE_DGRAD ? G.Ho * out_row : 128);
 #pragma unroll
       for (int c = 0; c < 4; ++c) {
         const int col = x0 + c - pad;
         const bool ok = lane_on && (unsigned)col < (unsigned)G.Wi;
-        voff[c] = ok ? (unsigned)(((Y - pad) * G.Wi + col) * 128 + kq * 32) : 0x80000000u;
-      }
-      unsigned oa = lane_on ? (unsigned)((Y * G.Wo + x0) * 128 + kq * 16) : 0x80000000u;
-      unsigned ob = (lane_on && x0 + 1 < G.Wo) ? oa + 128u : 0x80000000u;
-
-      f32x4 bias[2] = {{0, 0, 0, 0}, {0, 0, 0, 0}};
+        W.src.voff[c] = ok ? (unsigned)(((Y - pad) * G.Wi + col) * 128 + kq * 32) : 0x80000000u;
+      }
+      W.oa = lane_on ? (unsigned)((Y * G.Wo + x0) * 128 + kq * 16) : 0x80000000u;
+      W.ob = (lane_on && x0 + 1 < G.Wo) ? W.oa + 128u : 0x80000000u;
+
+      W.bias[0] = W.bias[1] = f32x4{0, 0, 0, 0};
       if (MODE == MODE_FWD) {
-        bias[0] = *reinterpret_cast<const f32x4*>(P.aux + 4 * kq);
-        bias[1] = *reinterpret_cast<const f32x4*>(P.aux + 16 + 4 * kq);
-      }
-
-      f32x4 raw[4][2];
-      auto load_row = [&]() {
-#pragma unroll
-        for (int c = 0; c < 4; ++c) {
-          raw[c][0] = __builtin_bit_cast(f32x4, __builtin_amdgcn_raw_buffer_load_b128(rin, voff[c], 0, 0));
-          raw[c][1] = __builtin_bit_cast(f32x4, __builtin_amdgcn_raw_buffer_load_b128(rin, voff[c] + 16u, 0, 0));
-        }
-      };
-      struct W3 {
-        u32x4 h, m, l;
-      };
-      auto wread = [&](const int g) {
-        const int pos = g / 6, dy = 2 - (g / 2) % 3, mt = g & 1;
-        const u32x4* p = lw + ((((dy * 4 + pos) * 2 + mt) * 3)) * 64;
-        W3 w;
-#if defined(RWB_ABL) && (RWB_ABL & 2)
-        w.h = p[0], w.m = w.h, w.l = w.h;
-        return w;
-#endif
-        w.h = p[0], w.m = p[64], w.l = p[128];
-        return w;
-      };
+        W.bias[0] = *reinterpret_cast<const f32x4*>(P.aux + 4 * kq);
+        W.bias[1] = *reinterpret_cast<const f32x4*>(P.aux + 16 + 4 * kq);
+      }
 
       Acc S0, S1, S2;
-      f32x4 mk[2][2];
-
-      auto mul6 = [&](f32x4 acc, const W3& w, const B3& x) {
-#if !(defined(RWB_ABL) && (RWB_ABL & 4))
-        acc = mfma_bf16(w.l, x.h, acc);
-        acc = mfma_bf16(w.h, x.l, acc);
-        acc = mfma_bf16(w.m, x.m, acc);
-#endif
-        acc = mfma_bf16(w.m, x.h, acc);
-        acc = mfma_bf16(w.h, x.m, acc);
-        acc = mfma_bf16(w.h, x.h, acc);
-        return acc;
-      };
-      auto finish = [&](const Acc& S) {
-#pragma unroll
-        for (int mt = 0; mt < 2; ++mt) {
-          f32x4 ya = S.m[mt][0] + S.m[mt][1] + S.m[mt][2];
-          f32x4 yb = S.m[mt][1] - S.m[mt][2] - S.m[mt][3];
-          if (MODE == MODE_FWD) {
-#pragma unroll
-            for (int r = 0; r < 4; ++r) ya[r] = fmaxf(ya[r], 0.f), yb[r] = fmaxf(yb[r], 0.f);
-          } else {
-#pragma unroll
-            for (int r = 0; r < 4; ++r) ya[r] = mk[0][mt][r] > 0.f ? ya[r] : 0.f, yb[r] = mk[1][mt][r] > 0.f ? yb[r] : 0.f;
-          }
-          __builtin_amdgcn_raw_buffer_store_b128(__builtin_bit_cast(u32x4, ya), rout, oa + mt * 64u, 0, CURLA_ACT_STORE_POLICY);
-          __builtin_amdgcn_raw_buffer_store_b128(__builtin_bit_cast(u32x4, yb), rout, ob + mt * 64u, 0, CURLA_ACT_STORE_POLICY);
-        }
-        oa += out_row, ob += out_row;
-      };
-
-      W3 Wa, Wb;
-      auto step = [&](Acc& Sdy2, Acc& Sdy1, Acc& Sdy0, const int t) {
-#ifdef RWB_STAMP
-        const unsigned long long c0 = __builtin_readcyclecounter();
-#endif
-        B3 X[4];
-        {
-          float v[4][8];
-#pragma unroll
-          for (int c8 = 0; c8 < 8; ++c8) {
-            const float d0 = raw[0][c8 >> 2][c8 & 3], d1 = raw[1][c8 >> 2][c8 & 3], d2 = raw[2][c8 >> 2][c8 & 3],
-                        d3 = raw[3][c8 >> 2][c8 & 3];
-            v[0][c8] = d0 - d2, v[1][c8] = d1 + d2, v[2][c8] = d2 - d1, v[3][c8] = d1 - d3;
-          }
-#pragma unroll
-          for (int pos = 0; pos < 4; ++pos) X[pos] = split8(v[pos]);
-        }
-        if (t < n + 1) {
-#pragma unroll
-          for (int c = 0; c < 4; ++c) voff[c] += in_row;
-          load_row();
-        }
-        const bool do2 = t >= 2, do1 = t >= 1 && t <= n, do0 = t < n;
-        if (MODE == MODE_DGRAD && do2) {
-#pragma unroll
-          for (int mt = 0; mt < 2; ++mt) {
-            mk[0][mt] = __builtin_bit_cast(f32x4, __builtin_amdgcn_raw_buffer_load_b128(raux, oa + mt * 64u, 0, 0));
-            mk[1][mt] = __builtin_bit_cast(f32x4, __builtin_amdgcn_raw_buffer_load_b128(raux, ob + mt * 64u, 0, 0));
-          }
-        }
-#ifdef RWB_STAMP
-        const unsigned long long c1 = __builtin_readcyclecounter();
-#endif
-#pragma unroll
-        for (int g = 0; g < 24; ++g) {
-          const int pos = g / 6, which = (g / 2) % 3, mt = g & 1;
-          W3& cur = (g & 1) ? Wb : Wa;
-          W3& nxt = (g & 1) ? Wa : Wb;
-          nxt = wread(g == 23 ? 0 : g + 1);
-          __builtin_amdgcn_sched_barrier(0);
-          if (which == 0) {
-            if (do2) Sdy2.m[mt][pos] = mul6(Sdy2.m[mt][pos], cur, X[pos]);
-          } else if (which == 1) {
-            if (do1) Sdy1.m[mt][pos] = mul6(Sdy1.m[mt][pos], cur, X[pos]);
-          } else {
-            const f32x4 z = {0, 0, 0, 0};
-            if (do0) Sdy0.m[mt][pos] = mul6(pos == 1 ? bias[mt] : z, cur, X[pos]);
-          }
-          __builtin_amdgcn_sched_barrier(0);
-        }
-#ifdef RWB_STAMP
-        const unsigned long long c2 = __builtin_readcyclecounter();
-#endif
-        if (do2) finish(Sdy2);
-#ifdef RWB_STAMP
-        const unsigned long long c3 = __builtin_readcyclecounter();
-        if (threadIdx.x == 0 && blockIdx.x == 7 && t >= 2 && t < n) {
-          g_rwb_stamp[0] += c1 - c0, g_rwb_stamp[1] += c2 - c1, g_rwb_stamp[2] += c3 - c2, g_rwb_stamp[3] += 1;
-        }
-        if (threadIdx.x == 0 && blockIdx.x == 7 && !(t >= 2 && t < n)) {
-          const int e = t < 2 ? t : (t == n ? 2 : 3);
-          g_rwb_stamp[11 + e] += c3 - c0;
-        }
-#endif
-      };
-
 #ifdef RWB_STAMP
       const unsigned long long p1 = __builtin_readcyclecounter();
 #endif
-      load_row();
-      Wa = wread(0);
+      W.src.load(W.raw);
+      W.Wa = W.wread(0);
       for (int t = 0;;) {
-        step(S1, S2, S0, t);
+        W.step(S1, S2, S0, t, t < n + 1);
         if (++t > n + 1) break;
-        step(S2, S0, S1, t);
+        W.step(S2, S0, S1, t, t < n + 1);
         if (++t > n + 1) break;
-        step(S0, S1, S2, t);
+        W.step(S0, S1, S2, t, t < n + 1);
         if (++t > n + 1) break;
       }
 #ifdef RWB_STAMP
@@ -287,9 +310,8 @@
         g_rwb_stamp[8] += __builtin_readcyclecounter() - p1, g_rwb_stamp[9] += 1, g_rwb_stamp[10] += n;
       }
 #endif
-
-    }
-  }
-}
-
-}
+    }
+  }
+}
+
+}
diff --git a/curla_amd/csrc/options.h b/curla_amd/csrc/options.h
--- a/curla_amd/csrc/options.h
+++ b/curla_amd/csrc/options.h
@@ -10,6 +10,7 @@
   kOptGemmMfma,
   kOptS1Wgrad,
   kOptWgrad1U8,
+  kOptNogradFuse,
   kOptCount
 };
 
@@ -22,5 +23,6 @@
 enum GemmMfmaOpt { kGemmMfmaAuto, kGemmMfmaF32, kGemmMfmaB3, kGemmMfmaValues };
 enum S1WgradOpt { kS1WgradAuto, kS1WgradX, kS1WgradXY, kS1WgradValues };
 enum Wgrad1U8Opt { kWgrad1U8Auto, kWgrad1U8F32, kWgrad1U8B16, kWgrad1U8Values };
+enum NogradFuseOpt { kNogradFuseOff, kNogradFuseAuto, kNogradFuseValues };
 
 int curla_opt(int id);
diff --git a/curla_amd/csrc/options.hip b/curla_amd/csrc/options.hip
--- a/curla_amd/csrc/options.hip
+++ b/curla_amd/csrc/options.hip
@@ -26,10 +26,12 @@
     {"gemm_mfma", {"auto", "f32", "b3", nullptr}, {nullptr, nullptr, "bf16x3", nullptr}},
     {"s1_wgrad", {"auto", "x", "xy", nullptr}, {nullptr, "1d", "2d", nullptr}},
     {"wgrad1_u8", {"auto", "f32", "b16", nullptr}, {nullptr, nullptr, "bf16", nullptr}},
+    {"nograd_fuse", {"off", "auto", nullptr}, {"0", "1", nullptr}},
 };
 
 constexpr int kValueCount[kOptCount] = {kConv1U8Values, kConv1F32Values, kS1FwdValues, kBwdSplitValues, kGemmTileValues,
-                                        kLinearBwdValues, kGemmMfmaValues, kS1WgradValues, kWgrad1U8Values};
+                                        kLinearBwdValues, kGemmMfmaValues, kS1WgradValues, kWgrad1U8Values,
+                                        kNogradFuseValues};
 constexpr bool value_counts_match() {
   for (int id = 0; id < kOptCount; ++id)
     if (!kDefs[id].values[kValueCount[id] - 1] || kDefs[id].values[kValueCount[id]]) return false;
diff --git a/curla_amd/curl_sac.py b/curla_amd/curl_sac.py
--- a/curla_amd/curl_sac.py
+++ b/curla_amd/curl_sac.py
@@ -799,10 +799,10 @@
         merged = pair is not None and pair[1] is no and pair[0].B == 2 * B
         tenc = self.critic_target.encoder
         if merged:
-            enc.conv_forward2(pair[0], ws.acts_pair, tenc, no, ws.acts_tmp)
+            enc.conv_forward2(pair[0], ws.acts_pair, tenc, no, ws.acts_tmp, other_nograd=True)
             h_next = ws.acts_pair[-1][B:]
         else:
-            enc.conv_forward(no, ws.acts_tmp)
+            enc.conv_forward(no, ws.acts_tmp, nograd=True)
             h_next = ws.acts_tmp[-1]
         if merged:
             CNNEncoder.fc_partial_multi([(self.actor.encoder, h_next), (tenc, ws.acts_tmp[-1]), (enc, ws.acts_main[-1])])
@@ -826,7 +826,7 @@
                      outer=(2, self._twin_outer))
         else:
             if not merged:
-                tenc.conv_forward(no, ws.acts_tmp)
+                tenc.conv_forward(no, ws.acts_tmp, nograd=True)
                 tenc.fc_partial(ws.acts_tmp[-1])
             tenc.ln_from_partial(B, ws.z_t, xa=ws.xa, act=ws.pi)
             _mlp_fwd(ws.xa, 0, self.critic_target.twin(), 2, B, F + A, H, 1, ws.q_h1, ws.q_h2, ws.tq)
@@ -890,7 +890,7 @@
         pos = self._pos_hint
         self._pos_hint = None
         if pos is not None:
-            enc.conv_forward2(o, ws.acts_main, self.critic_target.encoder, pos, ws.acts_tmp)
+            enc.conv_forward2(o, ws.acts_main, self.critic_target.encoder, pos, ws.acts_tmp, other_nograd=True)
             self._pos_cache = pos
         else:
             enc.conv_forward(o, ws.acts_main)
@@ -984,11 +984,11 @@
         self._anchor_cache = self._pos_cache = None
         self._pos_fc_done = False
         if need_anchor and need_pos:
-            enc.conv_forward2(oa, ws.acts_main, tenc, op_, ws.acts_tmp)
+            enc.conv_forward2(oa, ws.acts_main, tenc, op_, ws.acts_tmp, other_nograd=True)
         elif need_anchor:
             enc.conv_forward(oa, ws.acts_main)
         elif need_pos:
-            tenc.conv_forward(op_, ws.acts_tmp)
+            tenc.conv_forward(op_, ws.acts_tmp, nograd=True)
         if need_anchor:
             CNNEncoder.fc_partial_multi([(enc, ws.acts_main[-1]), (tenc, ws.acts_tmp[-1])])
             CNNEncoder.ln_from_partial_multi(B, [(enc, ws.z_c, dict(xhat=ws.xhat_c, rstd=ws.rstd_c)),
diff --git a/curla_amd/encoder.py b/curla_amd/encoder.py
--- a/curla_amd/encoder.py
+++ b/curla_amd/encoder.py
@@ -113,9 +113,24 @@
     def nsplit(self, B):
         return self._nsplit.get(B, self.ksplit(B))
 
-    def conv_forward(self, obs_ref, acts, conv_params=None):
+    def _s1_forward(self, acts, first, cp):
+        L = self.num_layers
+        if L - first > 1 and ops.conv_s1_fwd_stack(acts[first - 1], [cp[i][0] for i in range(first, L)],
+                                                   [cp[i][1] for i in range(first, L)], acts[first:L]):
+            return
+        for i in range(first, L):
+            ops.conv_s1_fwd(acts[i - 1], cp[i][0], cp[i][1], acts[i])
+
+    def _fused12(self, obs_ref, acts, cp):
+        return (self.num_layers >= 2 and self.num_filters == 32
+                and ops.conv12_nograd_fwd(obs_ref, cp[0][0], cp[0][1], cp[1][0], cp[1][1], acts[1]))
+
+    def conv_forward(self, obs_ref, acts, conv_params=None, nograd=False):
         cp = conv_params or self.conv_params()
         L = self.num_layers
+        if nograd and self._fused12(obs_ref, acts, cp):
+            self._s1_forward(acts, 2, cp)
+            return acts[-1]
         ops.conv1_fwd(obs_ref, cp[0][0], cp[0][1], acts[0])
         if L > 2 and ops.conv_s1_fwd_stack(acts[0], [cp[i][0] for i in range(1, L)], [cp[i][1] for i in range(1, L)],
                                            acts[1:L]):
@@ -124,11 +139,15 @@
             ops.conv_s1_fwd(acts[i - 1], cp[i][0], cp[i][1], acts[i])
         return acts[-1]
 
-    def conv_forward2(self, obs_ref, acts, other, other_ref, other_acts):
+    def conv_forward2(self, obs_ref, acts, other, other_ref, other_acts, other_nograd=False):
         cp, cp2 = self.conv_params(), other.conv_params()
         if self.num_layers != other.num_layers or acts[0].shape[1:] != other_acts[0].shape[1:]:
             self.conv_forward(obs_ref, acts)
-            other.conv_forward(other_ref, other_acts)
+            other.conv_forward(other_ref, other_acts, nograd=other_nograd)
+            return
+        if other_nograd and other._fused12(other_ref, other_acts, cp2):
+            other._s1_forward(other_acts, 2, cp2)
+            self.conv_forward(obs_ref, acts)
             return
         if ops.conv1_pairable(obs_ref, other_ref):
             ops.conv1_fwd2(obs_ref, cp[0][0], cp[0][1], acts[0], other_ref, cp2[0][0], cp2[0][1], other_acts[0])
diff --git a/curla_amd/ops.py b/curla_amd/ops.py
--- a/curla_amd/ops.py
+++ b/curla_amd/ops.py
@@ -70,6 +70,20 @@
     obs.check()
     call("curla_conv1_wgrad", ptr(obs.src), obs.is_u8, ptr(obs.idx), ptr(obs.h1), ptr(obs.w1), ptr(g), ptr(dw), ptr(db),
          ptr(ws), obs.B, obs.C, obs.Hs, obs.Ws, obs.Hc, obs.Wc, dw.shape[0], scale, stream())
+
+
+def conv12_nograd_fwd(obs: ObsRef, wa, ba, wb, bb, out2, scale=1.0 / 255.0):
+    if _lib._trace_hook is not None or obs.is_u8 != 1:
+        return False
+    obs.check()
+    rc = _lib.load().curla_conv12_nograd_fwd(ptr(obs.src), ptr(obs.idx), ptr(obs.h1), ptr(obs.w1), ptr(wa), ptr(ba), ptr(wb),
+                                             ptr(bb), ptr(out2), obs.B, obs.C, obs.Hs, obs.Ws, obs.Hc, obs.Wc, wa.shape[0],
+                                             scale, stream())
+    if rc == -3:
+        return False
+    if rc != 0:
+        raise _lib.CurlaHipError(f"curla_conv12_nograd_fwd failed: {_lib._ERRORS.get(rc, rc)}")
+    return True
 
 
 def conv_s1_fwd(x, w, b, out):
diff --git a/include/curla_hip.h b/include/curla_hip.h
--- a/include/curla_hip.h
+++ b/include/curla_hip.h
@@ -29,6 +29,10 @@
                      const float* bias, float* out, int B, const int64_t* idx2, const int32_t* h1_2,
                      const int32_t* w1_2, const float* w2, const float* bias2, float* out2, int B2, int C, int Hs, int Ws,
                      int Hc, int Wc, int channels, float scale, void* stream);
+
+int curla_conv12_nograd_fwd(const uint8_t* ring, const int64_t* idx, const int32_t* h1, const int32_t* w1, const float* wa,
+                            const float* ba, const float* wb, const float* bb, float* out2, int B, int C, int Hs, int Ws,
+                            int Hc, int Wc, int channels, float scale, void* stream);
 
 int curla_conv3x3_s1_fwd(const float* in, const float* w, const float* bias, float* out, int B, int Hi, int Wi,
                          int channels, void* stream);
```

Result: no change. 512.1 (median of 6 runs) (+0.1%).
